# psychopa4/PFNL

Hardware: AMD Instinct MI355X
Metric: HR frames/sec at 4xSR, 7-frame 128x128->512x512 (higher is better)
Workload: dtype f32

## Files before the change

### pfnl_amd/csrc/capi.hip

```cpp
#include <dlfcn.h>

#include <atomic>
#include <cmath>
#include <condition_variable>
#include <cstdio>
#include <cstdlib>
#include <cstring>
#include <functional>
#include <map>
#include <memory>
#include <mutex>
#include <string>
#include <thread>
#include <vector>

#include "../../include/pfnl_hip.h"
#include "capi_internal.h"
#include "common.h"
#include "conv_bf16.h"
#include "conv_split16.h"
#include "conv_small.h"

namespace {

thread_local std::string g_err;

int fail(int code, const std::string& msg) {
    g_err = msg;
    return code;
}
}

int pfnl_internal_fail(int code, const std::string& msg) { return fail(code, msg); }

namespace {

static unsigned long long g_alloc_gen = 0;

struct DevBuf {
    float* p = nullptr;
    size_t n = 0;
    int ensure(size_t count) {
        if (count <= n) return 0;
        ++g_alloc_gen;
        if (p) hipFree(p);
        p = nullptr;
        n = 0;
        if (hipMalloc(&p, count * sizeof(float)) != hipSuccess) return -1;
        n = count;
        return 0;
    }
    void release() {
        if (p) hipFree(p);
        p = nullptr;
        n = 0;
    }
};

struct HostTensor {
    std::vector<int64_t> shape;
    std::vector<float> data;
};

struct PinBuf {
    unsigned char* p = nullptr;
    size_t n = 0;
    int ensure(size_t bytes) {
        if (bytes <= n) return 0;
        release();
        if (hipHostMalloc(reinterpret_cast<void**>(&p), bytes, hipHostMallocDefault) != hipSuccess) {
            p = nullptr;
            return -1;
        }
        n = bytes;
        return 0;
    }
    void release() {
        if (p) hipHostFree(p);
        p = nullptr;
        n = 0;
    }
};

struct HostPool {
    std::vector<std::thread> th;
    std::mutex m;
    std::condition_variable cv_work, cv_done;
    std::function<void(int)> fn;
    std::unique_ptr<std::atomic<int>[]> flag;
    int cap = 0, n = 0, next = 0, finished = 0, device = 0;
    bool stop = false;
    void start(int k, int dev) {
        if (!th.empty()) return;
        device = dev;
        for (int i = 0; i < k; ++i) th.emplace_back([this] { loop(); });
    }
    void loop() {
        hipSetDevice(device);
        for (;;) {
            int i;
            {
                std::unique_lock<std::mutex> lk(m);
                cv_work.wait(lk, [&] { return stop || next < n; });
                if (stop) return;
                i = next++;
            }
            fn(i);
            flag[i].store(1, std::memory_order_release);
            {
                std::lock_guard<std::mutex> lk(m);
                ++finished;
            }
            cv_done.notify_all();
        }
    }
    void run(int count, std::function<void(int)> f) {
        std::lock_guard<std::mutex> lk(m);
        if (count > cap) {
            flag.reset(new std::atomic<int>[count]);
            cap = count;
        }
        for (int i = 0; i < count; ++i) flag[i].store(0, std::memory_order_relaxed);
        fn = std::move(f);
        n = count;
        next = 0;
        finished = 0;
        cv_work.notify_all();
    }
    void wait_chunk(int i) {
        while (!flag[i].load(std::memory_order_acquire)) std::this_thread::yield();
    }
    void wait() {
        std::unique_lock<std::mutex> lk(m);
        cv_done.wait(lk, [&] { return finished >= n; });
    }
    void shutdown() {
        {
            std::lock_guard<std::mutex> lk(m);
            stop = true;
        }
        cv_work.notify_all();
        for (auto& t : th) t.join();
        th.clear();
    }
};

}

static constexpr int kSmallTiles256 = 200;
static constexpr int kMidChains256 = 136;
static int scaled_by_cus(int v256, int ncu) {
    return ncu > 0 && ncu != 256 ? std::max(1, (int)((long long)v256 * ncu / 256)) : v256;
}

struct BlockPacks {
    size_t c1_w = 0, c1_b = 0, c10_w = 0, c10_b = 0, c10_s = 0, c2a_w = 0, c2b_w = 0, c2_b = 0;
    size_t c1_u = 0, c2a_u = 0, c2b_u = 0;
    size_t bf_c1 = 0, bf_c10 = 0, bf_c2a = 0, bf_c2b = 0, bf_c1_m16 = 0, bf_c2b_m16 = 0;
    size_t s_c1 = 0, s_c2a = 0, s_c2b = 0, s_c10 = 0, s_c10f = 0, s_c2a_sf = 0, s_c2b_sf = 0, s_c2a_m16 = 0, s_c2b_m16 = 0, s_c1_m16 = 0;
    size_t sm_c1 = 0, sm_c10 = 0, sm_c2 = 0;
};

struct pfnl_handle {
    pfnl_config cfg;
    int ncu = 0;
    hipStream_t stream = nullptr;
    std::map<std::string, std::vector<int64_t>> expected;
    std::map<std::string, HostTensor> host;
    bool finalized = false;
    bool weights_external = false;
    size_t wdev_used = 0, wdev16_used = 0, wdev16s_used = 0;
    struct GraphEntry {
        int B, H, W, seen;
        hipGraph_t graph;
        hipGraphExec_t exec;
        unsigned long long alloc_gen, cfg_gen;
        unsigned long long seen_cfg_gen;
        int slot;
    };
    std::vector<GraphEntry> graphs;
    unsigned long long cfg_gen = 0;
    hipEvent_t gev = nullptr;
    int graph_mode = 0;
    bool conv2_grouped = true;
    int merge_cstride = 48;
    int conv1x1_algo = 2;
    bool bf16_fuse10 = true;
    bool bf16_m16 = true;
    bool bf16 = false;
    DevBuf wdev16;
    size_t off16_m1 = 0;
    size_t off16s_m1 = 0;
    int m1_algo = 0;
    int conv_algo = 5;
    int nl_algo = 2;
    DevBuf wdev16s;
    bool s16_m16 = true;
    size_t off16m_m1 = 0;
    unsigned* rflag_host = nullptr;
    unsigned* rflag_dev = nullptr;
    PinBuf pin_in, pin_out;
    HostPool pool;
    std::vector<hipEvent_t> d2h_ev;
    bool strict = false, strict_once = false, weights_f16_ok = true;
    long long range_reruns = 0;
    int small_mode = 0;
    bool small_c10 = true;
    DevBuf p10;
    bool sf_chain = true;
    bool sf_c10 = true;
    bool sf_mid = true;
    int sf_mid_chains = 0;
    bool sf0 = false;
    DevBuf inp0sf;
    bool split_chains = true;
    DevBuf c10part;
    bool sf_path = true;

    DevBuf wdev;
    size_t off_conv0_w = 0, off_conv0_b = 0;
    std::vector<BlockPacks> blocks;
    std::vector<size_t> off_m1_u;
    size_t off_m1_w = 0, off_m1_b = 0, off_m2_w = 0, off_m2_b = 0, off_nl_w = 0, off_nl_b = 0, off_zero = 0;

    std::map<std::string, std::vector<int64_t>> optional;
    bool nl_theta = false;
    size_t off_nl_m = 0, off_nl_c = 0;
    DevBuf Q;
    DevBuf Xs;
    int nl_type = -1;
    int nl_sub = 1;

    DevBuf nl16;
    DevBuf X, Xo, nlp, inp0, inp1, base, pb, merge, stage_in, stage_out, scratch;
    int lastB = 0, lastH = 0, lastW = 0;

    bool prof = false;
    int prof_mode = 0;
    bool prof_gate = true;
    bool chain_open = false;
    std::vector<hipEvent_t> evs;
    std::vector<int> ev_cls;
    std::vector<int> ev_cnt;
    int run_cls = -1, run_n = 0;
    size_t evs_used = 0;
    double prof_ms[PFNL_K_COUNT] = {0};
    int64_t prof_n[PFNL_K_COUNT] = {0};

    pfnl_stream* session = nullptr;
};

pfnl_handle_view pfnl_internal_view(pfnl_handle* h) {
    return {h->cfg.num_frames, h->cfg.scale, h->cfg.device_id, h->finalized, h->stream, &h->session};
}

namespace {

using namespace pfnl;

inline bool prof_sampled(int nb, int i) { return nb >= 10 ? (i % 10) == 3 : (i & 3) == 0; }

int prof_mark(pfnl_handle* h, hipStream_t s, int cls, int count = 1) {
    if (h->evs_used == h->evs.size()) {
        hipEvent_t e;
        if (hipEventCreate(&e) != hipSuccess) return -1;
        h->evs.push_back(e);
        h->ev_cls.push_back(-1);
        h->ev_cnt.push_back(1);
    }
    h->ev_cls[h->evs_used] = cls;
    h->ev_cnt[h->evs_used] = count;
    return hipEventRecord(h->evs[h->evs_used++], s) == hipSuccess ? 0 : -1;
}

void prof_flush_run(pfnl_handle* h, hipStream_t s) {
    if (h->prof && h->prof_mode == 4 && h->run_n > 0) prof_mark(h, s, h->run_cls, h->run_n);
    h->run_n = 0;
    h->run_cls = -1;
}

struct Roctx {
    int (*push)(const char*) = nullptr;
    int (*pop)() = nullptr;
};
const Roctx* roctx() {
    static const Roctx r = [] {
        Roctx x;
        const char* e = std::getenv("PFNL_ROCTX");
        if (!e || !*e || *e == '0') return x;
        for (const char* n : {"librocprofiler-sdk-roctx.so", "librocprofiler-sdk-roctx.so.1", "libroctx64.so", "libroctx64.so.4",
                              "/opt/rocm/lib/librocprofiler-sdk-roctx.so", "/opt/rocm/lib/libroctx64.so"}) {
            if (void* lib = dlopen(n, RTLD_NOW | RTLD_GLOBAL)) {
                x.push = reinterpret_cast<int (*)(const char*)>(dlsym(lib, "roctxRangePushA"));
                x.pop = reinterpret_cast<int (*)()>(dlsym(lib, "roctxRangePop"));
                if (x.push && x.pop) break;
                x.push = nullptr;
                x.pop = nullptr;
            }
        }
        return x;
    }();
    return &r;
}
const char* const kClassNames[PFNL_K_COUNT] = {"pfnl:nl_pack", "pfnl:nl_attn", "pfnl:conv0", "pfnl:conv3x3", "pfnl:conv1x1", "pfnl:merge1", "pfnl:tail"};

struct ProfScope {
    pfnl_handle* h;
    hipStream_t s;
    int cls;
    bool ranged = false;
    ProfScope(pfnl_handle* h_, hipStream_t s_, int cls_) : h(h_), s(s_), cls(cls_) {
        if (roctx()->push && cls >= 0 && cls < PFNL_K_COUNT) {
            roctx()->push(kClassNames[cls]);
            ranged = true;
        }
        if (h && h->prof && h->prof_mode == 4 && h->run_n > 0 && h->run_cls != cls) prof_flush_run(h, s);
        if (h && h->prof && h->prof_gate && !h->chain_open) {
            prof_mark(h, s, -1);
            h->chain_open = true;
        }
    }
    ~ProfScope() {
        if (h && h->prof && h->prof_mode == 4) {
            h->run_cls = cls;
            ++h->run_n;
        } else if (h && h->prof && h->prof_gate) {
            prof_mark(h, s, cls);
        }
        if (ranged) roctx()->pop();
    }
};

int prof_collect(pfnl_handle* h) {
    for (size_t i = 0; i < h->evs_used; ++i) {
        const int cls = h->ev_cls[i];
        if (cls < 0 || i == 0) continue;
        if (hipEventSynchronize(h->evs[i]) != hipSuccess) return -1;
        float ms = 0.f;
        if (hipEventElapsedTime(&ms, h->evs[i - 1], h->evs[i]) != hipSuccess) return -1;
        h->prof_ms[cls] += ms;
        h->prof_n[cls] += h->ev_cnt[i];
    }
    h->evs_used = 0;
    h->chain_open = false;
    return 0;
}

int check_geometry(const pfnl_config& c) {
    if (c.num_frames != 3 && c.num_frames != 5 && c.num_frames != 7)
        return fail(PFNL_ERR_INVALID, "num_frames must be 3, 5 or 7");
    if (c.scale != 2 && c.scale != 4) return fail(PFNL_ERR_INVALID, "scale must be 2 or 4");
    if (c.mf != 64) return fail(PFNL_ERR_INVALID, "mf must be 64");
    if (c.num_block < 0 || c.num_block > 1024) return fail(PFNL_ERR_INVALID, "bad num_block");
    for (int r : c.reserved)
        if (r != 0) return fail(PFNL_ERR_INVALID, "reserved config fields must be 0");
    return 0;
}

void add_expected(pfnl_handle* h, const std::string& layer, int k, int cin, int cout) {
    h->expected["nlvsr/" + layer + "/kernel"] = {k, k, cin, cout};
    h->expected["nlvsr/" + layer + "/bias"] = {cout};
}

size_t numel(const std::vector<int64_t>& s) {
    size_t n = 1;
    for (auto d : s) n *= (size_t)d;
    return n;
}

enum Merge1Kind {
    M1_SMALL,
    M1_BF16,
    M1_SPLIT16,
    M1_SPLIT16_CUT,
    M1_WINOGRAD,
    M1_DIRECT,
};
const char* const kMerge1Names[] = {"small", "bf16", "split16", "split16_cut", "winograd", "direct"};

struct TrunkPlan {
    bool bf16 = false;
    bool strict = false;
    int nltype = 1;
    int nl_family = 0;
    bool nl_fused_pack = false;
    bool bmid = false, fuse10 = false;
    int algo = 0, conv1x1_algo = 0;
    bool sf = false;
    bool small = false, small_c10 = false;
    bool mid = false;
    bool c10_fused = false;
    bool chain = false;
    bool sf0 = false;
    bool conv2_grouped = false;
    int n_full = 0, split_s = 0, split_q = 0;
    int c1x1_launches = 0;
    int launches_per_block = 0;
    int tiles8x32 = 0, chains = 0;
    int mfma = 32;
    int c1_mfma = 32;
    int merge1 = M1_DIRECT;
    int merge_stride = 48;
    size_t p10_floats = 0, inp0sf_floats = 0, c10part_floats = 0;
    const char* name = "";
};

void plan_bf16_trunk(const pfnl_handle* h, TrunkPlan& pl, int T, int grid, int mid_chains, bool fits32) {
    pl.bmid = h->sf_mid && h->bf16_fuse10 && pl.chains < mid_chains;
    pl.fuse10 = h->bf16_fuse10 && !pl.bmid;
    pl.launches_per_block = pl.fuse10 ? 3 : 4;
    pl.c1x1_launches = pl.fuse10 ? 0 : 1;
    if (pl.fuse10 && h->split_chains && fits32 && split_rule(pl.chains, T, grid, pl.n_full, pl.split_s, pl.split_q)) {
        pl.launches_per_block += 1;
        pl.c1x1_launches = 1;
    }
    pl.name = pl.bmid ? "bf16_mid4" : (pl.fuse10 ? (pl.split_s ? "bf16_3_split" : "bf16_3") : "bf16_4");
    pl.mfma = h->bf16_m16 ? 16 : 32;
    pl.merge1 = M1_BF16;
    pl.merge_stride = 64;
}

void plan_fp32_trunk(const pfnl_handle* h, TrunkPlan& pl, int B, int H, int W, int T, int grid, int mid_chains, bool fits32) {
    const int small_tiles = scaled_by_cus(kSmallTiles256, h->ncu);
    const int algo0 = h->conv_algo == 5 ? ((pl.tiles8x32 >= small_tiles && fits32) ? 4 : 3) : h->conv_algo;
    pl.algo = (pl.strict && algo0 == 4) ? 3 : algo0;
    pl.conv1x1_algo = (pl.strict && h->conv1x1_algo == 2) ? 1 : h->conv1x1_algo;
    pl.sf = pl.algo == 4 && pl.conv1x1_algo == 2 && h->sf_path;
    pl.small = !pl.strict && fits32 &&
               (h->small_mode == 1 || (h->small_mode == 0 && h->conv_algo == 5 && h->conv1x1_algo == 2 && pl.tiles8x32 < small_tiles));
    pl.small_c10 = pl.small && h->small_c10;
    if (pl.small) {
        pl.launches_per_block = pl.small_c10 ? 2 : 3;
        pl.c1x1_launches = pl.small_c10 ? 0 : 1;
        pl.name = pl.small_c10 ? "small2" : "small3";
        pl.merge1 = M1_SMALL;
        pl.merge_stride = 64;
        return;
    }
    pl.mid = pl.sf && h->sf_mid && h->conv_algo == 5 && h->sf_c10 && h->sf_chain && pl.chains < mid_chains;
    pl.c10_fused = pl.sf && h->sf_c10 && !pl.mid;
    pl.chain = pl.sf && h->sf_chain && !pl.mid;
    pl.sf0 = pl.c10_fused && pl.chain && h->sf0;
    const int wino_groups = B * ((W + 31) / 32) * ((H + 3) / 4);
    pl.conv2_grouped = pl.algo == 3 && h->conv2_grouped && wino_groups >= 224 && fits32;
    pl.launches_per_block = (pl.c10_fused ? 1 : 2) + ((pl.chain || pl.conv2_grouped) ? 1 : 2);
    pl.c1x1_launches = pl.c10_fused ? 0 : 1;
    if (pl.c10_fused && pl.chain && h->split_chains && split_rule(pl.chains, T, grid, pl.n_full, pl.split_s, pl.split_q)) {
        pl.launches_per_block += 1;
        pl.c1x1_launches = 1;
    }
    pl.mfma = (h->s16_m16 && pl.c10_fused && pl.chain && !pl.sf0 && !pl.split_s && pl.chains >= grid) ? 16 : 32;
    pl.c1_mfma = pl.mfma;
    pl.name = pl.mid ? "mid4" : (pl.c10_fused && pl.chain) ? (pl.sf0 ? "chain2_sf0" : (pl.split_s ? "chain2_split" : "chain2"))
            : pl.algo == 4 ? (pl.launches_per_block == 3 ? "split16_3" : "split16_4")
            : pl.algo == 3 ? (pl.conv2_grouped ? "winograd_ws3" : "winograd_ws4")
            : pl.algo == 1 ? "winograd_tile4" : "direct4";
    if (pl.algo == 4 && h->m1_algo != 2 && fits32) pl.merge1 = pl.split_s ? M1_SPLIT16_CUT : M1_SPLIT16;
    else if ((pl.algo == 3 || pl.algo == 4) && wino_groups >= 224 && fits32) pl.merge1 = M1_WINOGRAD;
    pl.merge_stride = pl.merge1 == M1_DIRECT ? 48 : 64;
}

TrunkPlan trunk_plan(const pfnl_handle* h, int B, int H, int W, int Hfull) {
    TrunkPlan pl;
    const int T = h->cfg.num_frames;
    pl.bf16 = h->bf16;
    pl.strict = !h->bf16 && (h->strict || h->strict_once || !h->weights_f16_ok);
    pl.tiles8x32 = B * T * ((W + 31) / 32) * ((H + 7) / 8);
    pl.chains = pl.tiles8x32 / T;
    const int grid = persistent_grid(h->ncu);
    const int mid_chains = h->sf_mid_chains > 0 ? h->sf_mid_chains : scaled_by_cus(kMidChains256, h->ncu);
    const bool fits32 = (long long)H * W * 256 < 0x7fffffffLL;
    if (h->bf16) plan_bf16_trunk(h, pl, T, grid, mid_chains, fits32);
    else plan_fp32_trunk(h, pl, B, H, W, T, grid, mid_chains, fits32);

    const int N = (Hfull / 2) * (W / 2);
    pl.nltype = h->nl_type < 0 ? (h->nl_theta ? 0 : 1) : h->nl_type;
    pl.nl_family = (pl.nltype != 1 || h->nl_sub > 1) ? 0
                 : h->bf16 ? 2
                 : (!pl.strict && (h->nl_algo == 1 || (h->nl_algo == 2 && N >= 1024))) ? 1 : 3;
    pl.nl_fused_pack = (pl.nl_family == 1 || pl.nl_family == 2) && nl_f16_fits_one_launch(B, N);

    const size_t frame_floats = (size_t)B * T * H * W * 64;
    pl.p10_floats = pl.small_c10 ? frame_floats : 0;
    pl.inp0sf_floats = pl.sf0 ? frame_floats : 0;
    pl.c10part_floats = pl.split_s ? (size_t)(pl.chains - pl.n_full) * pl.split_s * 8 * 32 * 64 : 0;
    return pl;
}

struct Fwd {
    pfnl_handle* h;
    const TrunkPlan& pl;
    hipStream_t s;
    int B, T, F, H, W;
    const float* wd;
    const uint16_t* w16;
    const uint16_t* w16s;
};

template <class P>
void set_split_chains(P& q, const TrunkPlan& pl, float* partial) {
    q.n_full = pl.n_full;
    q.split_s = pl.split_s;
    q.split_q = pl.split_q;
    q.partial = pl.split_s ? partial : nullptr;
}

template <class P>
P split_finalize_params(const Fwd& f) {
    P q{};
    q.H = f.H;
    q.W = f.W;
    q.items = f.F;
    q.add_div = f.T;
    set_split_chains(q, f.pl, f.h->c10part.p);
    return q;
}

ConvParams direct_params(const Fwd& f, const float* in, const float* wpack, const float* bias, float* out, int cout, int frames, int act) {
    ConvParams p{};
    p.in = in;
    p.wpack = wpack;
    p.bias = bias;
    p.out = out;
    p.H = f.H;
    p.W = f.W;
    p.in_cstride = 64;
    p.out_cstride = cout;
    p.cout = cout;
    p.chunks_per_frame = 64 / CONV_CK;
    p.frames_per_item = frames;
    p.nchunks = frames * p.chunks_per_frame;
    p.add_div = 1;
    p.act = act;
    return p;
}

int ensure_workspace(pfnl_handle* h, const TrunkPlan& pl, int B, int H, int W, int N) {
    const int T = h->cfg.num_frames, C = 12 * T, CP = nl_padded_ch(C);
    const size_t P = (size_t)H * W;
    if (h->X.ensure((size_t)B * N * CP) || h->Xo.ensure((size_t)B * N * CP) ||
        h->nlp.ensure(nl_partial_floats(B, N, C)) ||
        h->inp0.ensure((size_t)B * T * P * 64) || h->inp1.ensure((size_t)B * T * P * 64) ||
        h->base.ensure((size_t)B * P * 64) || h->pb.ensure((size_t)B * P * 64) ||
        h->merge.ensure((size_t)B * P * 64))
        return fail(PFNL_ERR_NOMEM, "workspace allocation failed");
    h->lastB = B;
    h->lastH = H;
    h->lastW = W;
    if (h->p10.ensure(h->cfg.num_block > 0 ? pl.p10_floats : 0) || h->inp0sf.ensure(pl.inp0sf_floats) || h->c10part.ensure(pl.c10part_floats))
        return fail(PFNL_ERR_NOMEM, "workspace allocation failed");
    return 0;
}

int nonlocal_block(const Fwd& f, const float* in, int Hfull, int q0, int q1) {
    pfnl_handle* const h = f.h;
    const TrunkPlan& pl = f.pl;
    const int B = f.B, T = f.T, W = f.W, N = (Hfull / 2) * (W / 2), C = 12 * T, CP = nl_padded_ch(C), nlt = pl.nltype;
    const float* const wd = f.wd;
    const hipStream_t s = f.s;
    if ((pl.nl_family == 1 || pl.nl_family == 2) && h->nl16.ensure((nl_f16_scratch_halfs(B, N) + 1) / 2))
        return fail(PFNL_ERR_NOMEM, "workspace allocation failed");
    {
        ProfScope ps(h, s, PFNL_K_NL_PACK);
        if (pl.nl_fused_pack) HIPCHK(launch_nl_pack_fused(in, h->X.p, reinterpret_cast<uint16_t*>(h->nl16.p), B, T, Hfull, W, s));
        else HIPCHK(launch_nl_pack(in, h->X.p, B, T, Hfull, W, s));
    }
    ProfScope ps(h, s, PFNL_K_NL_ATTN);
    if ((nlt == 0 || nlt == 2) && !h->nl_theta)
        return fail(PFNL_ERR_STATE, "nl_type 0 / 2 need the nlblock_0 theta / phi variables (reference utils.py:31-42)");
    if (pl.nl_family == 0) {
        const float* Kx = h->X.p;
        int Nk = N;
        if (h->nl_sub > 1) {
            const int h2 = Hfull / 2, w2 = W / 2;
            if (h2 / h->nl_sub < 1 || w2 / h->nl_sub < 1) return fail(PFNL_ERR_INVALID, "nl_sub_sample larger than the space_to_depth grid");
            Nk = (h2 / h->nl_sub) * (w2 / h->nl_sub);
            if (h->Xs.ensure((size_t)B * Nk * CP)) return fail(PFNL_ERR_NOMEM, "workspace allocation failed");
            HIPCHK(launch_nl_pool(h->X.p, h->Xs.p, B, h2, w2, h->nl_sub, C, s));
            Kx = h->Xs.p;
        }
        const float* Qp = nullptr;
        if (nlt != 1) {
            if (h->Q.ensure((size_t)B * N * CP)) return fail(PFNL_ERR_NOMEM, "workspace allocation failed");
            HIPCHK(launch_nl_qproj(h->X.p, wd + h->off_nl_m, wd + h->off_nl_c, h->Q.p, B, N, C, s, nlt == 2));
            Qp = h->Q.p;
        }
        HIPCHK(launch_nl_attn_general(h->X.p, Kx, Nk, h->Xo.p, wd + h->off_nl_w, wd + h->off_nl_b, h->nlp.p, B, N, C, s, Qp, q0, q1, nlt == 2));
    } else if (pl.nl_family == 1 || pl.nl_family == 2) {
        HIPCHK(launch_nl_attn_f16(h->X.p, h->Xo.p, wd + h->off_nl_w, wd + h->off_nl_b, h->nlp.p, reinterpret_cast<uint16_t*>(h->nl16.p), B, N, C, s,
                                  q0, q1, pl.nl_family == 1, pl.nl_fused_pack));
    } else {
        HIPCHK(launch_nl_attn(h->X.p, h->Xo.p, wd + h->off_nl_w, wd + h->off_nl_b, h->nlp.p, B, N, C, s, nullptr, q0, q1));
    }
    return 0;
}


int block_bf16(const Fwd& f, const BlockPacks& k) {
    pfnl_handle* const h = f.h;
    const TrunkPlan& pl = f.pl;
    const hipStream_t s = f.s;
    const float* const wd = f.wd;
    uint16_t* const a0 = reinterpret_cast<uint16_t*>(h->inp0.p);
    uint16_t* const a1 = reinterpret_cast<uint16_t*>(h->inp1.p);
    uint16_t* const ab = reinterpret_cast<uint16_t*>(h->base.p);
    uint16_t* const ap = reinterpret_cast<uint16_t*>(h->pb.p);
    {
        ProfScope ps(h, s, PFNL_K_CONV3X3);
        ConvBf16Params q{a0, f.w16 + k.bf_c1, wd + k.c1_b, nullptr, nullptr, a1, f.H, f.W, f.F, 1, 1};
        if (pl.fuse10) {
            q.add_div = f.T;
            q.x_w = f.w16 + k.bf_c10;
            q.x_bias = wd + k.c10_b;
            q.x_out = ab;
            set_split_chains(q, pl, h->c10part.p);
        }
        if (pl.mfma == 16) q.wpack16 = f.w16 + k.bf_c1_m16;
        HIPCHK(launch_conv3x3_bf16(q, s));
    }
    if (pl.fuse10 && pl.split_s) {
        ProfScope ps(h, s, PFNL_K_CONV1X1);
        ConvBf16Params q = split_finalize_params<ConvBf16Params>(f);
        q.x_bias = wd + k.c10_b;
        q.x_out = ab;
        HIPCHK(launch_c10_finalize_bf16(q, s));
    }
    if (!pl.fuse10) {
        ProfScope ps(h, s, PFNL_K_CONV1X1);
        HIPCHK(launch_conv1x1_bf16(a1, f.w16 + k.bf_c10, wd + k.c10_b, ab, f.B, f.T, f.H * f.W, 1, s));
    }
    {
        ProfScope ps(h, s, PFNL_K_CONV3X3);
        ConvBf16Params q{ab, f.w16 + k.bf_c2a, wd + h->off_zero, nullptr, nullptr, ap, f.H, f.W, f.B, 1, 0};
        HIPCHK(launch_conv3x3_bf16(q, s));
    }
    {
        ProfScope ps(h, s, PFNL_K_CONV3X3);
        ConvBf16Params q{a1, f.w16 + k.bf_c2b, wd + k.c2_b, ap, a0, a0, f.H, f.W, f.F, f.T, 1};
        q.flat = pl.bmid ? 1 : 0;
        set_split_chains(q, pl, nullptr);
        if (pl.mfma == 16) q.wpack16 = f.w16 + k.bf_c2b_m16;
        HIPCHK(launch_conv3x3_bf16(q, s));
    }
    return 0;
}

int block_small(const Fwd& f, const BlockPacks& k) {
    pfnl_handle* const h = f.h;
    const hipStream_t s = f.s;
    const float* const wd = f.wd;
    const int H = f.H, W = f.W, F = f.F, T = f.T;
    {
        ProfScope ps(h, s, PFNL_K_CONV3X3);
        ConvSmallParams q{nullptr, h->inp0.p, 0, 1, 1, 1, f.w16s + k.sm_c1, wd + k.c1_b, nullptr, h->inp1.p, H, W, F, 1, 3};
        if (f.pl.small_c10) {
            q.x_wpack = f.w16s + k.sm_c10;
            q.x_out = h->p10.p;
            q.x_T = T;
        }
        HIPCHK(launch_conv_small(q, s));
    }
    if (!f.pl.small_c10) {
        ProfScope ps(h, s, PFNL_K_CONV1X1);
        ConvSmallParams q{nullptr, h->inp1.p, 0, 1, T, T, f.w16s + k.sm_c10, wd + k.c10_b, nullptr, h->base.p, H, W, f.B, 1, 1};
        HIPCHK(launch_conv_small(q, s));
    }
    {
        ProfScope ps(h, s, PFNL_K_CONV3X3);
        ConvSmallParams q{f.pl.small_c10 ? h->p10.p : h->base.p, h->inp1.p, 1, T, 1, 2, f.w16s + k.sm_c2, wd + k.c2_b, h->inp0.p, h->inp0.p, H, W, F, 1, 3};
        if (f.pl.small_c10) {
            q.a_nsum = T;
            q.a_bias = wd + k.c10_b;
        }
        HIPCHK(launch_conv_small(q, s));
    }
    return 0;
}

int block_fp32(const Fwd& f, const BlockPacks& k, bool first, bool last) {
    pfnl_handle* const h = f.h;
    const TrunkPlan& pl = f.pl;
    const hipStream_t s = f.s;
    const float* const wd = f.wd;
    const int H = f.H, W = f.W, F = f.F, T = f.T, B = f.B, algo = pl.algo;
    const bool sf = pl.sf;
    const bool in_sf0 = pl.sf0 && !first, out_sf0 = pl.sf0 && !last;
    if (pl.c10_fused) {
        {
            ProfScope ps(h, s, PFNL_K_CONV3X3);
            ConvSplitParams q{in_sf0 ? h->inp0sf.p : h->inp0.p, f.w16s + k.s_c1, wd + k.c1_b, nullptr, nullptr, h->inp1.p, H, W, F, T, 1};
            q.in_sf = in_sf0 ? 1 : 0;
            q.wpack2 = f.w16s + k.s_c10f;
            q.bias2 = wd + k.c10_b;
            q.out2 = h->base.p;
            set_split_chains(q, pl, h->c10part.p);
            if (pl.c1_mfma == 16) q.wpack_m16 = f.w16s + k.s_c1_m16;
            HIPCHK(launch_conv3x3_c1c10(q, s));
        }
        if (pl.split_s) {
            ProfScope ps(h, s, PFNL_K_CONV1X1);
            ConvSplitParams q = split_finalize_params<ConvSplitParams>(f);
            q.act = 1;
            q.out2 = h->base.p;
            HIPCHK(launch_c10_finalize(q, s));
        }
    } else {
        {
            ProfScope ps(h, s, PFNL_K_CONV3X3);
            if (algo == 4) {
                ConvSplitParams q{h->inp0.p, f.w16s + k.s_c1, wd + k.c1_b, nullptr, nullptr, h->inp1.p, H, W, F, 1, 1};
                q.out_sf = sf ? 1 : 0;
                HIPCHK(launch_conv3x3_split16(q, s));
            } else if (algo == 1 || algo == 3) {
                WinoParams wp{h->inp0.p, wd + k.c1_u, wd + k.c1_b, nullptr, nullptr, h->inp1.p, H, W, 1, 1, F};
                HIPCHK(algo == 3 ? launch_conv_wino_ws(wp, s) : launch_conv_wino(wp, s));
            } else {
                HIPCHK(launch_conv_mfma(direct_params(f, h->inp0.p, wd + k.c1_w, wd + k.c1_b, h->inp1.p, 64, 1, 1), 3, F, s));
            }
        }
        {
            ProfScope ps(h, s, PFNL_K_CONV1X1);
            if (pl.conv1x1_algo == 2)
                HIPCHK(launch_conv1x1_split16(h->inp1.p, f.w16s + k.s_c10, wd + k.c10_b, h->base.p, B, T, H * W, 1, s, sf, sf));
            else if (pl.conv1x1_algo == 1)
                HIPCHK(launch_conv1x1_stream(h->inp1.p, wd + k.c10_s, wd + k.c10_b, h->base.p, B, T, H * W, 1, s));
            else
                HIPCHK(launch_conv_mfma(direct_params(f, h->inp1.p, wd + k.c10_w, wd + k.c10_b, h->base.p, 64, T, 1), 1, B, s));
        }
    }
    if (pl.conv2_grouped) {
        ProfScope ps(h, s, PFNL_K_CONV3X3);
        WinoParams wp{h->inp1.p, wd + k.c2b_u, wd + k.c2_b, nullptr, h->inp0.p, h->inp0.p, H, W, T, 1, F};
        wp.in2 = h->base.p;
        wp.upack2 = wd + k.c2a_u;
        HIPCHK(launch_conv_wino_ws(wp, s));
        return 0;
    }
    if (pl.chain) {
        ProfScope ps(h, s, PFNL_K_CONV3X3);
        ConvSplitParams q{h->inp1.p, f.w16s + k.s_c2b_sf, wd + k.c2_b, nullptr, h->inp0.p, h->inp0.p, H, W, F, T, 1};
        q.in2 = h->base.p;
        q.wpack2 = f.w16s + k.s_c2a_sf;
        q.out2 = out_sf0 ? h->inp0sf.p : nullptr;
        set_split_chains(q, pl, nullptr);
        if (pl.mfma == 16) {
            q.wpack_m16 = f.w16s + k.s_c2b_m16;
            q.wpack2_m16 = f.w16s + k.s_c2a_m16;
        }
        HIPCHK(launch_conv3x3_sf_chain(q, s));
        return 0;
    }
    {
        ProfScope ps(h, s, PFNL_K_CONV3X3);
        if (algo == 4) {
            ConvSplitParams q{h->base.p, f.w16s + (sf ? k.s_c2a_sf : k.s_c2a), wd + h->off_zero, nullptr, nullptr, h->pb.p, H, W, B, 1, 0};
            HIPCHK(sf ? launch_conv3x3_sf(q, s) : launch_conv3x3_split16(q, s));
        } else if (algo == 1 || algo == 3) {
            WinoParams wp{h->base.p, wd + k.c2a_u, wd + h->off_zero, nullptr, nullptr, h->pb.p, H, W, 1, 0, B};
            HIPCHK(algo == 3 ? launch_conv_wino_ws(wp, s) : launch_conv_wino(wp, s));
        } else {
            HIPCHK(launch_conv_mfma(direct_params(f, h->base.p, wd + k.c2a_w, wd + h->off_zero, h->pb.p, 64, 1, 0), 3, B, s));
        }
    }
    {
        ProfScope ps(h, s, PFNL_K_CONV3X3);
        if (algo == 4) {
            ConvSplitParams q{h->inp1.p, f.w16s + (sf ? k.s_c2b_sf : k.s_c2b), wd + k.c2_b, h->pb.p, h->inp0.p, h->inp0.p, H, W, F, T, 1};
            q.flat = pl.mid ? 1 : 0;
            HIPCHK(sf ? launch_conv3x3_sf(q, s) : launch_conv3x3_split16(q, s));
        } else if (algo == 1 || algo == 3) {
            WinoParams wp{h->inp1.p, wd + k.c2b_u, wd + k.c2_b, h->pb.p, h->inp0.p, h->inp0.p, H, W, T, 1, F};
            HIPCHK(algo == 3 ? launch_conv_wino_ws(wp, s) : launch_conv_wino(wp, s));
        } else {
            ConvParams p = direct_params(f, h->inp1.p, wd + k.c2b_w, wd + k.c2_b, h->inp0.p, 64, 1, 1);
            p.addend = h->pb.p;
            p.add_div = T;
            p.resid = h->inp0.p;
            HIPCHK(launch_conv_mfma(p, 3, F, s));
        }
    }
    return 0;
}

int convmerge1(const Fwd& f) {
    pfnl_handle* const h = f.h;
    const TrunkPlan& pl = f.pl;
    const hipStream_t s = f.s;
    const float* const wd = f.wd;
    const int H = f.H, W = f.W, F = f.F, T = f.T;
    h->merge_cstride = pl.merge_stride;
    if (pl.merge1 == M1_SPLIT16 || pl.merge1 == M1_SPLIT16_CUT) {
        {
            ProfScope ps(h, s, PFNL_K_MERGE1);
            ConvSplitParams q{h->inp0.p, f.w16s + h->off16s_m1, wd + h->off_m1_b, nullptr, nullptr, h->merge.p, H, W, F, T, 1, 1};
            set_split_chains(q, pl, h->c10part.p);
            HIPCHK(launch_conv3x3_split16(q, s));
        }
        if (pl.merge1 == M1_SPLIT16_CUT) {
            ProfScope ps(h, s, PFNL_K_MERGE1);
            ConvSplitParams q = split_finalize_params<ConvSplitParams>(f);
            q.act = 1;
            q.bias = wd + h->off_m1_b;
            q.out = h->merge.p;
            HIPCHK(launch_c10_finalize(q, s));
        }
        return 0;
    }
    ProfScope ps(h, s, PFNL_K_MERGE1);
    switch (pl.merge1) {
    case M1_SMALL: {
        ConvSmallParams q{nullptr, h->inp0.p, 0, 1, T, T, f.w16s + h->off16m_m1, wd + h->off_m1_b, nullptr, h->merge.p, H, W, f.B, 1, 3};
        HIPCHK(launch_conv_small(q, s));
        return 0;
    }
    case M1_BF16: {
        ConvBf16Params q{reinterpret_cast<const uint16_t*>(h->inp0.p), f.w16 + h->off16_m1, wd + h->off_m1_b, nullptr, nullptr, nullptr, H, W, F, T, 1};
        q.out_f32 = h->merge.p;
        HIPCHK(launch_conv3x3_bf16(q, s));
        return 0;
    }
    case M1_WINOGRAD: {
        WinoParams wp{h->inp0.p, wd + h->off_m1_u[0], wd + h->off_m1_b, nullptr, nullptr, h->merge.p, H, W, T, 1, F};
        wp.upack_stride = T > 1 ? (long long)(h->off_m1_u[1] - h->off_m1_u[0]) : 0;
        wp.accum = 1;
        HIPCHK(launch_conv_wino_ws(wp, s));
        return 0;
    }
    default:
        HIPCHK(launch_conv_mfma(direct_params(f, h->inp0.p, wd + h->off_m1_w, wd + h->off_m1_b, h->merge.p, 48, T, 1), 3, f.B, s));
        return 0;
    }
}

int forward_device(pfnl_handle* h, const float* in, float* out, int B, int Hfull, int W, hipStream_t s,
                   const StripGeom* strip = nullptr, int q0 = 0, int q1 = -1, int flag_slot = 1 ) {
    const pfnl_config& c = h->cfg;
    const int T = c.num_frames;
    const int H = strip ? strip->Hs : Hfull;
    const TrunkPlan pl = trunk_plan(h, B, H, W, Hfull);
    if (pl.bf16 && (long long)T * H * W * 128 >= 0x7fffffffLL) return fail(PFNL_ERR_INVALID, "frame too large for the bf16 trunk");
    if (int e = ensure_workspace(h, pl, B, H, W, (Hfull / 2) * (W / 2))) return e;
    const Fwd f{h, pl, s, B, T, B * T, H, W, h->wdev.p, reinterpret_cast<const uint16_t*>(h->wdev16.p), reinterpret_cast<const uint16_t*>(h->wdev16s.p)};
    const float* const wd = h->wdev.p;

    if (int e = nonlocal_block(f, in, Hfull, q0, q1)) return e;
    {
        ProfScope ps(h, s, PFNL_K_CONV0);
        if (pl.bf16)
            HIPCHK(launch_conv0_bf16(h->Xo.p, wd + h->off_conv0_w, wd + h->off_conv0_b, reinterpret_cast<uint16_t*>(h->inp0.p), B, T, Hfull, W, s, strip));
        else
            HIPCHK(launch_conv0(h->Xo.p, wd + h->off_conv0_w, wd + h->off_conv0_b, h->inp0.p, B, T, Hfull, W, s, strip, pl.strict));
    }
    for (int i = 0; i < c.num_block; ++i) {
        if (h->prof_mode == 2) {
            h->prof_gate = prof_sampled(c.num_block, i);
            h->chain_open = false;
        } else if (h->prof_mode == 3) {
            h->prof_gate = i == c.num_block / 2;
            h->chain_open = false;
        }
        const BlockPacks& k = h->blocks[i];
        const int e = pl.bf16 ? block_bf16(f, k) : pl.small ? block_small(f, k) : block_fp32(f, k, i == 0, i + 1 == c.num_block);
        if (e) return e;
    }
    h->prof_gate = h->prof_mode != 3;
    if (h->prof_mode == 2 || h->prof_mode == 3) h->chain_open = false;
    if (int e = convmerge1(f)) return e;
    {
        unsigned* const rflag = (pl.strict || pl.nltype == 2) ? nullptr : h->rflag_dev + flag_slot;
        ProfScope ps(h, s, PFNL_K_TAIL);
        HIPCHK(launch_tail(h->merge.p, in, wd + h->off_m2_w, wd + h->off_m2_b, out, B, T, Hfull, W, c.scale, pl.merge_stride, s, strip, rflag));
    }
    prof_flush_run(h, s);
    h->chain_open = false;
    return 0;
}

struct OptionField {
    int pfnl_handle::*i = nullptr;
    bool pfnl_handle::*b = nullptr;
    constexpr OptionField(int pfnl_handle::*f) : i(f) {}
    constexpr OptionField(bool pfnl_handle::*f) : b(f) {}
    int get(const pfnl_handle* h) const { return i ? h->*i : (int)(h->*b); }
    void set(pfnl_handle* h, int v) const {
        if (i) h->*i = v;
        else h->*b = v != 0;
    }
};

struct OptionName {
    const char* name;
    int value;
};

struct OptionSpec {
    const char* key;
    OptionField field;
    OptionName names[8];
    const char* refusal;
};

const OptionSpec kOptions[] = {
    {"graph", &pfnl_handle::graph_mode, {{"auto", 1}, {"on", 2}, {"off", 0}}, "graph must be auto, on or off"},
    {"conv3x3", &pfnl_handle::conv_algo, {{"winograd", 3}, {"winograd_ws", 3}, {"winograd_tile", 1}, {"direct", 0}, {"split16", 4}, {"auto", 5}},
     "conv3x3 must be auto, split16, winograd, winograd_tile or direct"},
    {"strict_fp32", &pfnl_handle::strict, {{"on", 1}, {"off", 0}}, "strict_fp32 must be on or off"},
    {"small", &pfnl_handle::small_mode, {{"auto", 0}, {"on", 1}, {"off", 2}}, "small must be auto, on or off"},
    {"split16_chain", &pfnl_handle::sf_chain, {{"on", 1}, {"off", 0}}, "split16_chain must be on or off"},
    {"split16_c10", &pfnl_handle::sf_c10, {{"on", 1}, {"off", 0}}, "split16_c10 must be on or off"},
    {"split16_mid", &pfnl_handle::sf_mid, {{"auto", 1}, {"off", 0}}, "split16_mid must be auto or off"},
    {"split16_sf0", &pfnl_handle::sf0, {{"on", 1}, {"off", 0}}, "split16_sf0 must be on or off"},
    {"split16_splitchains", &pfnl_handle::split_chains, {{"auto", 1}, {"off", 0}}, "split16_splitchains must be auto or off"},
    {"split16_sf", &pfnl_handle::sf_path, {{"on", 1}, {"off", 0}}, "split16_sf must be on or off"},
    {"conv2", &pfnl_handle::conv2_grouped, {{"grouped", 1}, {"split", 0}}, "conv2 must be grouped or split"},
    {"split16_mfma", &pfnl_handle::s16_m16, {{"16", 1}, {"32", 0}}, "split16_mfma must be 16 or 32"},
    {"bf16_mfma", &pfnl_handle::bf16_m16, {{"16", 1}, {"32", 0}}, "bf16_mfma must be 16 or 32"},
    {"bf16_conv10", &pfnl_handle::bf16_fuse10, {{"fused", 1}, {"separate", 0}}, "bf16_conv10 must be fused or separate"},
    {"precision", &pfnl_handle::bf16, {{"bf16", 1}, {"fp32", 0}}, "precision must be fp32 or bf16"},
    {"merge1", &pfnl_handle::m1_algo, {{"auto", 0}, {"split16", 1}, {"winograd", 2}}, "merge1 must be auto, split16 or winograd"},
    {"nl_type", &pfnl_handle::nl_type,
     {{"auto", -1}, {"0", 0}, {"embedded_gaussian", 0}, {"1", 1}, {"gaussian", 1}, {"2", 2}, {"dot_product", 2}},
     "nl_type: auto | 0 | 1 | 2 (nltype 3, 'concat', builds no graph in the reference either: utils.py:23)"},
    {"small_c10", &pfnl_handle::small_c10, {{"on", 1}, {"off", 0}}, "small_c10 must be on or off"},
    {"nonlocal", &pfnl_handle::nl_algo, {{"f32", 0}, {"split16", 1}, {"auto", 2}}, "nonlocal must be auto, f32 or split16"},
    {"conv1x1", &pfnl_handle::conv1x1_algo, {{"stream", 1}, {"tiled", 0}, {"split16", 2}}, "conv1x1 must be split16, stream or tiled"},
};

const OptionSpec* find_option(const std::string& key) {
    for (const OptionSpec& o : kOptions)
        if (key == o.key) return &o;
    return nullptr;
}

}

void pfnl_nl_fold_gw(const float* wg, const float* bg, const float* ww, const float* bw, int C, int CP, float* Wf, float* bf) {
    for (int ci = 0; ci < C; ++ci)
        for (int co = 0; co < C; ++co) {
            double acc = 0.0;
            for (int cm = 0; cm < C; ++cm) acc += (double)wg[(size_t)ci * C + cm] * (double)ww[(size_t)cm * C + co];
            Wf[(size_t)ci * CP + co] = (float)acc;
        }
    for (int co = 0; co < C; ++co) {
        double acc = bw[co];
        for (int cm = 0; cm < C; ++cm) acc += (double)bg[cm] * (double)ww[(size_t)cm * C + co];
        bf[co] = (float)acc;
    }
}

void pfnl_nl_fold_theta_phi(const float* wt, const float* bt, const float* wp, const float* bp, int C, int CP, float* Mf, float* cf) {
    for (int ci = 0; ci < C; ++ci)
        for (int cj = 0; cj < C; ++cj) {
            double acc = 0.0;
            for (int cm = 0; cm < C; ++cm) acc += (double)wt[(size_t)ci * C + cm] * (double)wp[(size_t)cj * C + cm];
            Mf[(size_t)ci * CP + cj] = (float)acc;
        }
    for (int cj = 0; cj < C; ++cj) {
        double acc = 0.0;
        for (int cm = 0; cm < C; ++cm) acc += (double)bt[cm] * (double)wp[(size_t)cj * C + cm];
        cf[cj] = (float)acc;
    }
    if (!bp) return;
    double d0 = 0.0;
    for (int cm = 0; cm < C; ++cm) d0 += (double)bt[cm] * (double)bp[cm];
    cf[C] = (float)d0;
    for (int ci = 0; ci < C; ++ci) {
        double acc = 0.0;
        for (int cm = 0; cm < C; ++cm) acc += (double)wt[(size_t)ci * C + cm] * (double)bp[cm];
        Mf[(size_t)ci * CP + C] = (float)acc;
    }
}

extern "C" {

const char* pfnl_last_error(void) { return g_err.c_str(); }
int pfnl_version(void) { return 4; }

int pfnl_device_count(int* count) {
    if (!count) return fail(PFNL_ERR_INVALID, "count is NULL");
    int n = 0;
    if (hipGetDeviceCount(&n) != hipSuccess) n = 0;
    *count = n;
    return 0;
}

int pfnl_create(const pfnl_config* cfg, pfnl_handle** out) {
    if (!cfg || !out) return fail(PFNL_ERR_INVALID, "NULL argument");
    if (int e = check_geometry(*cfg)) return e;
    int ndev = 0;
    if (hipGetDeviceCount(&ndev) != hipSuccess || ndev == 0)
        return fail(PFNL_ERR_NODEVICE, "no HIP device visible: libpfnl_hip has no CPU fallback");
    if (cfg->device_id < 0 || cfg->device_id >= ndev) return fail(PFNL_ERR_INVALID, "bad device_id");
    HIPCHK(hipSetDevice(cfg->device_id));
    pfnl_handle* h = new pfnl_handle();
    h->cfg = *cfg;
    h->ncu = pfnl::device_cu_count();
    if (const char* e = std::getenv("PFNL_SF_MID_CHAINS")) h->sf_mid_chains = std::atoi(e);
    if (const char* e = std::getenv("PFNL_CONV3X3")) {
        const std::string v(e);
        h->conv_algo = v == "direct" ? 0 : (v == "winograd_tile" ? 1 : (v == "split16" ? 4 : (v == "winograd" ? 3 : 5)));
    }
    if (hipStreamCreateWithFlags(&h->stream, hipStreamDefault) != hipSuccess) {
        delete h;
        return fail(PFNL_ERR_HIP, "hipStreamCreate failed");
    }
    if (hipHostMalloc(reinterpret_cast<void**>(&h->rflag_host), 64, hipHostMallocMapped) != hipSuccess ||
        hipHostGetDevicePointer(reinterpret_cast<void**>(&h->rflag_dev), h->rflag_host, 0) != hipSuccess) {
        if (h->rflag_host) hipHostFree(h->rflag_host);
        hipStreamDestroy(h->stream);
        delete h;
        return fail(PFNL_ERR_NOMEM, "allocation failed");
    }
    std::memset(h->rflag_host, 0, 64);
    if (const char* e = std::getenv("PFNL_STRICT_FP32")) h->strict = std::string(e) != "0" && std::string(e) != "off";
    const int T = cfg->num_frames, C = 12 * T;
    add_expected(h, "conv0", 5, 3, 64);
    for (int i = 0; i < cfg->num_block; ++i) {
        add_expected(h, "conv1_" + std::to_string(i), 3, 64, 64);
        add_expected(h, "conv10_" + std::to_string(i), 1, 64 * T, 64);
        add_expected(h, "conv2_" + std::to_string(i), 3, 128, 64);
    }
    add_expected(h, "convmerge1", 3, 64 * T, 48);
    add_expected(h, "convmerge2", 3, 12, cfg->scale == 4 ? 12 : 3);
    add_expected(h, "nlblock_0/g/g", 1, C, C);
    add_expected(h, "nlblock_0/w/w", 1, C, C);
    for (const char* n : {"theta/theta", "phi/phi"}) {
        h->optional[std::string("nlvsr/nlblock_0/") + n + "/kernel"] = {1, 1, C, C};
        h->optional[std::string("nlvsr/nlblock_0/") + n + "/bias"] = {C};
    }
    *out = h;
    return 0;
}

int pfnl_destroy(pfnl_handle* h) {
    if (!h) return 0;
    if (h->session) pfnl_stream_close(h->session);
    hipSetDevice(h->cfg.device_id);
    if (h->stream) {
        hipStreamSynchronize(h->stream);
        hipStreamDestroy(h->stream);
    }
    for (auto& e : h->evs) hipEventDestroy(e);
    if (h->gev) hipEventDestroy(h->gev);
    for (auto& g : h->graphs) {
        if (g.exec) hipGraphExecDestroy(g.exec);
        if (g.graph) hipGraphDestroy(g.graph);
    }
    h->pool.shutdown();
    for (auto& e : h->d2h_ev) hipEventDestroy(e);
    h->pin_in.release();
    h->pin_out.release();
    if (h->rflag_host) hipHostFree(h->rflag_host);
    for (DevBuf* b : {&h->p10, &h->Xs, &h->Q, &h->wdev16s, &h->wdev, &h->wdev16, &h->nl16, &h->X, &h->Xo, &h->nlp, &h->inp0, &h->inp0sf, &h->c10part, &h->inp1, &h->base, &h->pb, &h->merge,
                      &h->stage_in, &h->stage_out, &h->scratch})
        b->release();
    delete h;
    return 0;
}

int pfnl_set_weight(pfnl_handle* h, const char* tf_name, const float* host, const int64_t* shape,
                    int rank) {
    if (!h || !tf_name || !host || !shape) return fail(PFNL_ERR_INVALID, "NULL argument");
    std::string name(tf_name);
    if (name.size() > 2 && name.compare(name.size() - 2, 2, ":0") == 0) name.resize(name.size() - 2);
    auto it = h->expected.find(name);
    if (it == h->expected.end()) it = h->expected.find("nlvsr/" + name);
    if (it == h->expected.end()) {
        it = h->optional.find(name);
        if (it == h->optional.end()) it = h->optional.find("nlvsr/" + name);
        if (it == h->optional.end()) return fail(PFNL_ERR_INVALID, "unknown tensor name: " + name);
    }
    if ((int)it->second.size() != rank) return fail(PFNL_ERR_INVALID, "rank mismatch for " + name);
    for (int i = 0; i < rank; ++i)
        if (shape[i] != it->second[i]) return fail(PFNL_ERR_INVALID, "shape mismatch for " + name);
    if (h->weights_external) {
        h->host.clear();
        h->weights_external = false;
    }
    HostTensor t;
    t.shape = it->second;
    t.data.assign(host, host + numel(t.shape));
    h->host[it->first] = std::move(t);
    h->finalized = false;
    return 0;
}

int pfnl_set_option(pfnl_handle* h, const char* key, const char* value) {
    if (!h || !key || !value) return fail(PFNL_ERR_INVALID, "NULL argument");
    const std::string k(key), v(value);
    ++h->cfg_gen;
    if (k == "nl_sub_sample") {
        const int n = atoi(v.c_str());
        if (n < 1 || n > 64) return fail(PFNL_ERR_INVALID, "nl_sub_sample: an integer >= 1");
        h->nl_sub = n;
        return 0;
    }
    if (k == "bf16_nonlocal") {
        if (v != "f16") return fail(PFNL_ERR_INVALID, "bf16_nonlocal must be f16");
        return 0;
    }
    const OptionSpec* o = find_option(k);
    if (!o) return fail(PFNL_ERR_INVALID, "unknown option " + k);
    for (const OptionName& n : o->names)
        if (n.name && v == n.name) {
            o->field.set(h, n.value);
            return 0;
        }
    return fail(PFNL_ERR_INVALID, o->refusal);
}

int pfnl_get_option(pfnl_handle* h, const char* key, char* buf, size_t buflen) {
    if (!h || !key || !buf || buflen < 1) return fail(PFNL_ERR_INVALID, "NULL argument");
    const std::string k(key);
    std::string v;
    if (k == "nl_sub_sample") v = std::to_string(h->nl_sub);
    else if (k == "bf16_nonlocal") v = "f16";
    else if (const OptionSpec* o = find_option(k)) {
        const int cur = o->field.get(h);
        for (const OptionName& n : o->names)
            if (n.name && n.value == cur) {
                v = n.name;
                break;
            }
    } else return fail(PFNL_ERR_INVALID, "unknown option " + k);
    if (v.size() + 1 > buflen) return fail(PFNL_ERR_INVALID, "buffer too small");
    std::memcpy(buf, v.c_str(), v.size() + 1);
    return 0;
}

int pfnl_missing_weights(pfnl_handle* h, int* count) {
    if (!h || !count) return fail(PFNL_ERR_INVALID, "NULL argument");
    int n = 0;
    for (auto& kv : h->expected)
        if (!h->host.count(kv.first)) ++n;
    *count = n;
    return 0;
}

int pfnl_finalize_weights(pfnl_handle* h) {
    if (!h) return fail(PFNL_ERR_INVALID, "NULL handle");
    for (auto& kv : h->expected)
        if (!h->host.count(kv.first)) return fail(PFNL_ERR_STATE, "missing tensor " + kv.first);
    HIPCHK(hipSetDevice(h->cfg.device_id));
    const int T = h->cfg.num_frames, nb = h->cfg.num_block, C = 12 * T, CP = pfnl::nl_padded_ch(C);
    std::vector<float> blob;
    auto W = [&](const std::string& l) -> const std::vector<float>& { return h->host["nlvsr/" + l + "/kernel"].data; };
    auto Bv = [&](const std::string& l) -> const std::vector<float>& { return h->host["nlvsr/" + l + "/bias"].data; };
    auto reserve = [&](size_t n) {
        size_t off = (blob.size() + 63) / 64 * 64;
        blob.resize(off + n, 0.f);
        return off;
    };
    auto put_bias = [&](const std::vector<float>& b) {
        size_t off = reserve(64);
        std::memcpy(&blob[off], b.data(), b.size() * sizeof(float));
        return off;
    };
    auto put_wino = [&](const std::vector<float>& k, int cin_total, int cin_begin) {
        size_t off = reserve(pfnl::wino_pack_floats());
        pfnl::wino_pack_weights(k.data(), cin_total, cin_begin, &blob[off]);
        return off;
    };
    auto put_pack = [&](const std::vector<float>& k, int ks, int cin_total, int cin_begin, int cin, int cout) {
        size_t off = reserve(pfnl::conv_pack_floats(ks, cin));
        pfnl::conv_pack_weights(k.data(), ks, cin_total, cin_begin, cin, cout, &blob[off]);
        return off;
    };

    h->off_zero = reserve(64);
    h->off_conv0_w = reserve(75 * 64);
    std::memcpy(&blob[h->off_conv0_w], W("conv0").data(), 75 * 64 * sizeof(float));
    h->off_conv0_b = put_bias(Bv("conv0"));
    h->blocks.assign(nb, BlockPacks{});
    for (int i = 0; i < nb; ++i) {
        const std::string s = std::to_string(i);
        BlockPacks& k = h->blocks[i];
        k.c1_w = put_pack(W("conv1_" + s), 3, 64, 0, 64, 64);
        k.c1_b = put_bias(Bv("conv1_" + s));
        k.c10_w = put_pack(W("conv10_" + s), 1, 64 * T, 0, 64 * T, 64);
        k.c10_b = put_bias(Bv("conv10_" + s));
        k.c10_s = reserve(pfnl::conv1x1_pack_floats(T));
        pfnl::conv1x1_pack_weights(W("conv10_" + s).data(), T, &blob[k.c10_s]);
        k.c2a_w = put_pack(W("conv2_" + s), 3, 128, 0, 64, 64);
        k.c2b_w = put_pack(W("conv2_" + s), 3, 128, 64, 64, 64);
        k.c2_b = put_bias(Bv("conv2_" + s));
        k.c1_u = put_wino(W("conv1_" + s), 64, 0);
        k.c2a_u = put_wino(W("conv2_" + s), 128, 0);
        k.c2b_u = put_wino(W("conv2_" + s), 128, 64);
    }
    h->off_m1_w = put_pack(W("convmerge1"), 3, 64 * T, 0, 64 * T, 48);
    h->off_m1_b = put_bias(Bv("convmerge1"));
    h->off_m1_u.assign(T, 0);
    for (int f = 0; f < T; ++f) {
        h->off_m1_u[f] = reserve(pfnl::wino_pack_floats());
        pfnl::wino_pack_weights(W("convmerge1").data(), 64 * T, 64 * f, &blob[h->off_m1_u[f]], 48);
    }
    {
        const auto& k = W("convmerge2");
        h->off_m2_w = reserve(k.size());
        std::memcpy(&blob[h->off_m2_w], k.data(), k.size() * sizeof(float));
        h->off_m2_b = put_bias(Bv("convmerge2"));
    }
    {
        h->off_nl_w = reserve((size_t)CP * CP);
        h->off_nl_b = reserve(CP);
        pfnl_nl_fold_gw(W("nlblock_0/g/g").data(), Bv("nlblock_0/g/g").data(), W("nlblock_0/w/w").data(), Bv("nlblock_0/w/w").data(), C, CP,
                        &blob[h->off_nl_w], &blob[h->off_nl_b]);
    }
    {
        int have = 0;
        for (auto& kv : h->optional) have += (int)h->host.count(kv.first);
        if (have != 0 && have != (int)h->optional.size())
            return fail(PFNL_ERR_STATE, "nlblock_0 theta/phi: all four tensors (two kernels, two biases) or none");
        h->nl_theta = have != 0;
        if (h->nl_theta) {
            h->off_nl_m = reserve((size_t)CP * CP);
            h->off_nl_c = reserve(CP);
            pfnl_nl_fold_theta_phi(W("nlblock_0/theta/theta").data(), Bv("nlblock_0/theta/theta").data(), W("nlblock_0/phi/phi").data(),
                                   Bv("nlblock_0/phi/phi").data(), C, CP, &blob[h->off_nl_m], &blob[h->off_nl_c]);
        }
    }
    {
        std::vector<uint16_t> b16;
        auto reserve16 = [&](size_t n) {
            size_t off = (b16.size() + 127) / 128 * 128;
            b16.resize(off + n, 0);
            return off;
        };
        for (int i = 0; i < nb; ++i) {
            const std::string s = std::to_string(i);
            BlockPacks& k = h->blocks[i];
            k.bf_c1 = reserve16(pfnl::conv3x3_bf16_pack_halfs());
            pfnl::conv3x3_bf16_pack_weights(W("conv1_" + s).data(), 64, 0, &b16[k.bf_c1]);
            k.bf_c10 = reserve16(pfnl::conv1x1_bf16_pack_halfs(T));
            pfnl::conv1x1_bf16_pack_weights(W("conv10_" + s).data(), T, &b16[k.bf_c10]);
            k.bf_c2a = reserve16(pfnl::conv3x3_bf16_pack_halfs());
            pfnl::conv3x3_bf16_pack_weights(W("conv2_" + s).data(), 128, 0, &b16[k.bf_c2a]);
            k.bf_c2b = reserve16(pfnl::conv3x3_bf16_pack_halfs());
            pfnl::conv3x3_bf16_pack_weights(W("conv2_" + s).data(), 128, 64, &b16[k.bf_c2b]);
            k.bf_c1_m16 = reserve16(pfnl::conv3x3_bf16_pack_halfs());
            pfnl::conv3x3_bf16_pack_weights16(W("conv1_" + s).data(), 64, 0, &b16[k.bf_c1_m16]);
            k.bf_c2b_m16 = reserve16(pfnl::conv3x3_bf16_pack_halfs());
            pfnl::conv3x3_bf16_pack_weights16(W("conv2_" + s).data(), 128, 64, &b16[k.bf_c2b_m16]);
        }
        h->off16_m1 = reserve16((size_t)T * pfnl::conv3x3_bf16_pack_halfs());
        for (int f = 0; f < T; ++f)
            pfnl::conv3x3_bf16_pack_weights(W("convmerge1").data(), 64 * T, 64 * f, &b16[h->off16_m1 + (size_t)f * pfnl::conv3x3_bf16_pack_halfs()], 48);
        b16.resize((b16.size() + 1) / 2 * 2 + 2, 0);
        h->wdev16_used = b16.size() / 2;
        if (h->wdev16.ensure(b16.size() / 2)) return fail(PFNL_ERR_NOMEM, "weight allocation failed");
        HIPCHK(hipMemcpy(h->wdev16.p, b16.data(), b16.size() * sizeof(uint16_t), hipMemcpyHostToDevice));
    }
    {
        std::vector<uint16_t> b16;
        const size_t n3 = pfnl::conv3x3_split16_pack_halfs(), n1 = pfnl::conv1x1_split16_pack_halfs(T);
        const size_t blk = 8 * n3 + n1 + pfnl::conv1x1_c10_pack_halfs(T);
        h->off16s_m1 = (size_t)nb * blk;
        const size_t m3 = pfnl::conv_small_pack_halfs(3, 1), m10 = pfnl::conv_small_pack_halfs(1, T);
        const size_t small_base = (size_t)nb * blk + (size_t)T * n3;
        h->off16m_m1 = small_base + (size_t)nb * (3 * m3 + m10);
        b16.resize(h->off16m_m1 + (size_t)T * m3 + 2, 0);
        pfnl::conv_small_pack_weights(W("convmerge1").data(), 3, T, 48, &b16[h->off16m_m1]);
        for (int f = 0; f < T; ++f)
            pfnl::conv3x3_split16_pack_weights(W("convmerge1").data(), 64 * T, 64 * f, &b16[h->off16s_m1 + (size_t)f * n3], 48);
        for (int i = 0; i < nb; ++i) {
            const std::string s = std::to_string(i);
            BlockPacks& k = h->blocks[i];
            k.s_c1 = (size_t)i * blk;
            k.s_c2a = k.s_c1 + n3;
            k.s_c2b = k.s_c1 + 2 * n3;
            k.s_c10 = k.s_c1 + 3 * n3;
            k.s_c2a_sf = k.s_c10 + n1;
            k.s_c2b_sf = k.s_c2a_sf + n3;
            k.s_c10f = k.s_c2b_sf + n3;
            k.s_c2a_m16 = k.s_c10f + pfnl::conv1x1_c10_pack_halfs(T);
            k.s_c2b_m16 = k.s_c2a_m16 + n3;
            k.s_c1_m16 = k.s_c2b_m16 + n3;
            pfnl::conv3x3_split16_pack_weights16(W("conv1_" + s).data(), 64, 0, &b16[k.s_c1_m16], true);
            pfnl::conv3x3_split16_pack_weights16(W("conv2_" + s).data(), 128, 0, &b16[k.s_c2a_m16]);
            pfnl::conv3x3_split16_pack_weights16(W("conv2_" + s).data(), 128, 64, &b16[k.s_c2b_m16]);
            pfnl::conv1x1_c10_pack_weights(W("conv10_" + s).data(), T, &b16[k.s_c10f]);
            pfnl::conv3x3_split16_pack_weights(W("conv2_" + s).data(), 128, 0, &b16[k.s_c2a_sf], 64, true);
            pfnl::conv3x3_split16_pack_weights(W("conv2_" + s).data(), 128, 64, &b16[k.s_c2b_sf], 64, true);
            k.sm_c1 = small_base + (size_t)i * (3 * m3 + m10);
            k.sm_c2 = k.sm_c1 + m3;
            k.sm_c10 = k.sm_c1 + 3 * m3;
            pfnl::conv_small_pack_weights(W("conv1_" + s).data(), 3, 1, 64, &b16[k.sm_c1]);
            pfnl::conv_small_pack_weights(W("conv2_" + s).data(), 3, 2, 64, &b16[k.sm_c2]);
            pfnl::conv_small_pack_weights(W("conv10_" + s).data(), 1, T, 64, &b16[k.sm_c10]);
            pfnl::conv1x1_split16_pack_weights(W("conv10_" + s).data(), T, &b16[k.s_c10]);
            pfnl::conv3x3_split16_pack_weights(W("conv1_" + s).data(), 64, 0, &b16[k.s_c1]);
            pfnl::conv3x3_split16_pack_weights(W("conv2_" + s).data(), 128, 0, &b16[k.s_c2a]);
            pfnl::conv3x3_split16_pack_weights(W("conv2_" + s).data(), 128, 64, &b16[k.s_c2b]);
        }
        h->wdev16s_used = b16.size() / 2;
        if (h->wdev16s.ensure(b16.size() / 2)) return fail(PFNL_ERR_NOMEM, "weight allocation failed");
        HIPCHK(hipMemcpy(h->wdev16s.p, b16.data(), b16.size() / 2 * 2 * sizeof(uint16_t), hipMemcpyHostToDevice));
    }
    {
        float wmax = 0.f;
        for (const auto& kv : h->host)
            for (float v : kv.second.data) wmax = std::fmax(wmax, std::fabs(v));
        h->weights_f16_ok = wmax < 65504.0f;
    }
    h->wdev_used = blob.size();
    if (h->wdev.ensure(blob.size())) return fail(PFNL_ERR_NOMEM, "weight allocation failed");
    HIPCHK(hipMemcpy(h->wdev.p, blob.data(), blob.size() * sizeof(float), hipMemcpyHostToDevice));
    h->finalized = true;
    ++h->cfg_gen;
    return 0;
}

int pfnl_workspace_bytes(pfnl_handle* h, int B, int H, int W, size_t* bytes) {
    if (!h || !bytes) return fail(PFNL_ERR_INVALID, "NULL argument");
    if (B <= 0 || H <= 0 || W <= 0 || (H & 1) || (W & 1)) return fail(PFNL_ERR_INVALID, "bad shape");
    const size_t T = h->cfg.num_frames, P = (size_t)H * W, N = P / 4, sc = h->cfg.scale;
    const int C = 12 * (int)T;
    const size_t CP = pfnl::nl_padded_ch(C);
    size_t f = 2 * B * N * CP
             + pfnl::nl_partial_floats(B, (int)N, C)
             + 2 * B * T * P * 64
             + 3 * B * P * 64
             + (size_t)B * T * P * 3 + (size_t)B * P * sc * sc * 3;
    if (h->bf16 || h->nl_algo != 0) f += (pfnl::nl_f16_scratch_halfs(B, (int)N) + 1) / 2;
    if (h->nl_theta) f += (size_t)B * N * CP;
    if (h->nl_sub > 1) f += (size_t)B * ((H / 2) / h->nl_sub) * ((W / 2) / h->nl_sub) * CP;
    const TrunkPlan pl = trunk_plan(h, B, H, W, H);
    f += pl.p10_floats + pl.inp0sf_floats + pl.c10part_floats;
    *bytes = f * sizeof(float);
    return 0;
}

int pfnl_plan(pfnl_handle* h, int B, int H, int W, char* buf, size_t buflen) {
    if (!h || !buf || buflen < 1) return fail(PFNL_ERR_INVALID, "NULL argument");
    if (B <= 0 || H <= 0 || W <= 0 || (H & 1) || (W & 1)) return fail(PFNL_ERR_INVALID, "bad shape");
    const TrunkPlan pl = trunk_plan(h, B, H, W, H);
    static const char* const nln[] = {"general_f32", "split16", "f16", "f32"};
    static const char* const a3[] = {"direct", "winograd_tile", "?", "winograd", "split16"};
    static const char* const a1[] = {"tiled", "stream", "split16"};
    char tmp[384];
    if (pl.bf16)
        std::snprintf(tmp, sizeof tmp, "%s launches_per_block=%d c1x1=%d precision=bf16 tiles=%d chains=%d whole_chains=%d split_parts=%d part_frames=%d nl=%s nl_pack_fused=%d mfma=%d merge1=%s",
                      pl.name, pl.launches_per_block, pl.c1x1_launches, pl.tiles8x32, pl.chains, pl.split_s ? pl.n_full : pl.chains, pl.split_s, pl.split_q,
                      nln[pl.nl_family], pl.nl_fused_pack ? 1 : 0, pl.mfma, kMerge1Names[pl.merge1]);
    else
        std::snprintf(tmp, sizeof tmp, "%s launches_per_block=%d c1x1=%d precision=fp32 conv3x3=%s conv1x1=%s c10_fused=%d chain=%d sf0=%d strict=%d tiles=%d chains=%d "
                      "whole_chains=%d split_parts=%d part_frames=%d nl=%s nl_pack_fused=%d mfma=%d c1_mfma=%d merge1=%s",
                      pl.name, pl.launches_per_block, pl.c1x1_launches, pl.small ? "small" : a3[pl.algo < 0 || pl.algo > 4 ? 2 : pl.algo],
                      a1[pl.conv1x1_algo < 0 || pl.conv1x1_algo > 2 ? 0 : pl.conv1x1_algo], pl.c10_fused ? 1 : 0, pl.chain ? 1 : 0, pl.sf0 ? 1 : 0,
                      pl.strict ? 1 : 0, pl.tiles8x32, pl.chains, pl.split_s ? pl.n_full : pl.chains, pl.split_s, pl.split_q, nln[pl.nl_family],
                      pl.nl_fused_pack ? 1 : 0, pl.mfma, pl.c1_mfma, kMerge1Names[pl.merge1]);
    if (std::strlen(tmp) + 1 > buflen) return fail(PFNL_ERR_INVALID, "buffer too small");
    std::strcpy(buf, tmp);
    return 0;
}

static int range_flag_take(pfnl_handle* h, int slot, int* flagged) {
    unsigned* const f = h->rflag_host + slot;
    *flagged = __atomic_exchange_n(f, 0u, __ATOMIC_ACQ_REL) != 0;
    return 0;
}

int pfnl_range_reruns(pfnl_handle* h, long long* count) {
    if (!h || !count) return fail(PFNL_ERR_INVALID, "NULL argument");
    *count = h->range_reruns;
    return 0;
}

namespace {
constexpr size_t STAGE_POOL_MIN = 512u << 10;
constexpr int STAGE_MAX_CHUNKS = 32;

bool host_is_pinned(const void* p) {
    hipPointerAttribute_t a;
    if (hipPointerGetAttributes(&a, p) != hipSuccess) {
        (void)hipGetLastError();
        return false;
    }
    return a.type == hipMemoryTypeHost;
}

void ensure_pool(pfnl_handle* h) {
    if (!h->pool.th.empty()) return;
    int k = 4;
    if (const char* e = std::getenv("PFNL_HOST_THREADS")) k = std::atoi(e);
    const int hw = (int)std::thread::hardware_concurrency();
    if (hw > 1 && k > hw - 1) k = hw - 1;
    k = k < 1 ? 1 : (k > 16 ? 16 : k);
    h->pool.start(k, h->cfg.device_id);
}

size_t stage_chunk_bytes(size_t bytes) {
    size_t c = (bytes + STAGE_MAX_CHUNKS - 1) / STAGE_MAX_CHUNKS;
    if (c < (1u << 20)) c = 1u << 20;
    return (c + 4095) & ~(size_t)4095;
}

int stage_h2d(pfnl_handle* h, float* dst, const void* src, size_t bytes, hipStream_t s) {
    if (host_is_pinned(src)) {
        HIPCHK(hipMemcpyAsync(dst, src, bytes, hipMemcpyHostToDevice, s));
        return 0;
    }
    if (h->pin_in.ensure(bytes)) return fail(PFNL_ERR_NOMEM, "pinned staging allocation failed");
    unsigned char* const pin = h->pin_in.p;
    if (bytes < STAGE_POOL_MIN) {
        std::memcpy(pin, src, bytes);
        HIPCHK(hipMemcpyAsync(dst, pin, bytes, hipMemcpyHostToDevice, s));
        return 0;
    }
    ensure_pool(h);
    const size_t csz = stage_chunk_bytes(bytes);
    const int n = (int)((bytes + csz - 1) / csz);
    const unsigned char* const sp = static_cast<const unsigned char*>(src);
    h->pool.run(n, [=](int i) {
        const size_t off = (size_t)i * csz;
        std::memcpy(pin + off, sp + off, std::min(csz, bytes - off));
    });
    hipError_t err = hipSuccess;
    for (int i = 0; i < n; ++i) {
        h->pool.wait_chunk(i);
        const size_t off = (size_t)i * csz;
        if (err == hipSuccess)
            err = hipMemcpyAsync(reinterpret_cast<unsigned char*>(dst) + off, pin + off, std::min(csz, bytes - off), hipMemcpyHostToDevice, s);
    }
    h->pool.wait();
    if (err != hipSuccess) return fail(PFNL_ERR_HIP, std::string("H2D staging: ") + hipGetErrorString(err));
    return 0;
}

int stage_d2h(pfnl_handle* h, void* dst, const float* src, size_t bytes, hipStream_t s) {
    if (host_is_pinned(dst)) {
        HIPCHK(hipMemcpyAsync(dst, src, bytes, hipMemcpyDeviceToHost, s));
        HIPCHK(hipStreamSynchronize(s));
        return 0;
    }
    if (h->pin_out.ensure(bytes)) return fail(PFNL_ERR_NOMEM, "pinned staging allocation failed");
    unsigned char* const pin = h->pin_out.p;
    if (bytes < STAGE_POOL_MIN) {
        HIPCHK(hipMemcpyAsync(pin, src, bytes, hipMemcpyDeviceToHost, s));
        HIPCHK(hipStreamSynchronize(s));
        std::memcpy(dst, pin, bytes);
        return 0;
    }
    ensure_pool(h);
    const size_t csz = stage_chunk_bytes(bytes);
    const int n = (int)((bytes + csz - 1) / csz);
    while ((int)h->d2h_ev.size() < n) {
        hipEvent_t e = nullptr;
        HIPCHK(hipEventCreateWithFlags(&e, hipEventDisableTiming));
        h->d2h_ev.push_back(e);
    }
    for (int i = 0; i < n; ++i) {
        const size_t off = (size_t)i * csz;
        HIPCHK(hipMemcpyAsync(pin + off, reinterpret_cast<const unsigned char*>(src) + off, std::min(csz, bytes - off), hipMemcpyDeviceToHost, s));
        HIPCHK(hipEventRecord(h->d2h_ev[i], s));
    }
    HIPCHK(hipEventSynchronize(h->d2h_ev[0]));
    unsigned char* const dp = static_cast<unsigned char*>(dst);
    hipEvent_t* const ev = h->d2h_ev.data();
    h->pool.run(n, [=](int i) {
        const size_t off = (size_t)i * csz;
        (void)hipEventSynchronize(ev[i]);
        std::memcpy(dp + off, pin + off, std::min(csz, bytes - off));
    });
    h->pool.wait();
    HIPCHK(hipStreamSynchronize(s));
    return 0;
}

const char* const RANGE_MSG_FP32 =
    "a device-pointer forward since the last check produced non-finite values: an operand left the range of the f16-pipe kernels "
    "(|x| < 65504; the non-local block: inputs on a [0,1] scale) or the input was not finite. Re-run with "
    "pfnl_set_option(h, \"strict_fp32\", \"on\") (f32-MFMA kernels: the reference's range), or use host pointers";
const char* const RANGE_MSG_BF16 =
    "a precision=bf16 forward produced non-finite values: the input was not finite, or it left the range of the binary16 operands of "
    "this precision's non-local block and conv0 (inputs on a [0,1] scale, |x| < ~350). precision=fp32 covers the whole fp32 range";
}

int pfnl_forward(pfnl_handle* h, const void* in, int in_is_device, void* out, int out_is_device, int B,
                 int H, int W, void* stream) {
    if (!h || !in || !out) return fail(PFNL_ERR_INVALID, "NULL argument");
    if (!h->finalized) return fail(PFNL_ERR_STATE, "pfnl_finalize_weights has not been called");
    if (B <= 0 || H <= 0 || W <= 0) return fail(PFNL_ERR_INVALID, "B, H, W must be positive");
    if ((H & 1) || (W & 1))
        return fail(PFNL_ERR_INVALID, "H and W must be even (space_to_depth(2), reference model/pfnl.py:57)");
    HIPCHK(hipSetDevice(h->cfg.device_id));
    const int T = h->cfg.num_frames, sc = h->cfg.scale;
    const size_t n_in = (size_t)B * T * H * W * 3, n_out = (size_t)B * H * W * sc * sc * 3;
    const float* din = (const float*)in;
    float* dout = (float*)out;
    const bool sync_call = !in_is_device || !out_is_device;
    const int slot = sync_call ? 0 : 1;
    const bool can_rerun = !h->bf16 && !(h->strict || !h->weights_f16_ok);
    const bool want_graph = !h->prof && (h->graph_mode == 2 || (h->graph_mode == 1 && (size_t)B * T * H * W <= 65536));
    hipStream_t s = stream ? (hipStream_t)stream : ((in_is_device && out_is_device && !want_graph) ? (hipStream_t) nullptr : h->stream);
    if (want_graph) {
        if (h->stage_in.ensure(n_in) || h->stage_out.ensure(n_out)) return fail(PFNL_ERR_NOMEM, "staging allocation failed");
        pfnl_handle::GraphEntry* ge = nullptr;
        for (auto& g : h->graphs)
            if (g.B == B && g.H == H && g.W == W && g.slot == slot) ge = &g;
        if (!ge) {
            h->graphs.push_back({B, H, W, 0, nullptr, nullptr, 0, 0, h->cfg_gen, slot});
            ge = &h->graphs.back();
        }
        if (ge->exec && (ge->alloc_gen != g_alloc_gen || ge->cfg_gen != h->cfg_gen)) {
            HIPCHK(hipStreamSynchronize(s));
            hipGraphExecDestroy(ge->exec);
            hipGraphDestroy(ge->graph);
            ge->exec = nullptr;
            ge->graph = nullptr;
            ge->seen = 0;
        }
        if (!ge->exec && ge->seen_cfg_gen != h->cfg_gen) {
            ge->seen = 0;
            ge->seen_cfg_gen = h->cfg_gen;
        }
        if (!ge->exec && ge->seen >= 1) {
            HIPCHK(hipStreamBeginCapture(s, hipStreamCaptureModeThreadLocal));
            const int fe = forward_device(h, h->stage_in.p, h->stage_out.p, B, H, W, s, nullptr, 0, -1, slot);
            hipGraph_t g = nullptr;
            const hipError_t ce = hipStreamEndCapture(s, &g);
            if (fe) return fe;
            if (ce != hipSuccess || !g) return fail(PFNL_ERR_HIP, std::string("graph capture: ") + hipGetErrorString(ce));
            hipGraphExec_t ex = nullptr;
            const hipError_t ie = hipGraphInstantiate(&ex, g, nullptr, nullptr, 0);
            if (ie != hipSuccess) {
                hipGraphDestroy(g);
                return fail(PFNL_ERR_HIP, std::string("graph instantiate: ") + hipGetErrorString(ie));
            }
            ge->graph = g;
            ge->exec = ex;
            ge->alloc_gen = g_alloc_gen;
            ge->cfg_gen = h->cfg_gen;
        }
        if (ge->exec) {
            if (!stream) {
                if (!h->gev && hipEventCreateWithFlags(&h->gev, hipEventDisableTiming) != hipSuccess)
                    return fail(PFNL_ERR_HIP, "event creation failed");
                HIPCHK(hipEventRecord(h->gev, nullptr));
                HIPCHK(hipStreamWaitEvent(s, h->gev, 0));
            }
            if (in_is_device)
                HIPCHK(hipMemcpyAsync(h->stage_in.p, in, n_in * sizeof(float), hipMemcpyDeviceToDevice, s));
            else if (int e = stage_h2d(h, h->stage_in.p, in, n_in * sizeof(float), s))
                return e;
            HIPCHK(hipGraphLaunch(ge->exec, s));
            if (out_is_device)
                HIPCHK(hipMemcpyAsync(out, h->stage_out.p, n_out * sizeof(float), hipMemcpyDeviceToDevice, s));
            if (sync_call) {
                if (!out_is_device) {
                    if (int e = stage_d2h(h, out, h->stage_out.p, n_out * sizeof(float), s)) return e;
                } else {
                    HIPCHK(hipStreamSynchronize(s));
                }
                int flagged = 0;
                if (int e = range_flag_take(h, 0, &flagged)) return e;
                if (flagged && can_rerun) {
                    h->strict_once = true;
                    const int e = forward_device(h, h->stage_in.p, h->stage_out.p, B, H, W, s, nullptr, 0, -1, 0);
                    h->strict_once = false;
                    if (e) return e;
                    ++h->range_reruns;
                    if (out_is_device) {
                        HIPCHK(hipMemcpyAsync(out, h->stage_out.p, n_out * sizeof(float), hipMemcpyDeviceToDevice, s));
                        HIPCHK(hipStreamSynchronize(s));
                    } else if (int e2 = stage_d2h(h, out, h->stage_out.p, n_out * sizeof(float), s)) {
                        return e2;
                    }
                } else if (flagged && h->bf16) {
                    return fail(PFNL_ERR_RANGE, RANGE_MSG_BF16);
                }
            } else if (!stream) {
                HIPCHK(hipEventRecord(h->gev, s));
                HIPCHK(hipStreamWaitEvent(nullptr, h->gev, 0));
            }
            h->lastB = B;
            h->lastH = H;
            h->lastW = W;
            return 0;
        }
        ge->seen++;
    }
    if (!in_is_device) {
        if (h->stage_in.ensure(n_in)) return fail(PFNL_ERR_NOMEM, "staging allocation failed");
        if (int e = stage_h2d(h, h->stage_in.p, in, n_in * sizeof(float), s)) return e;
        din = h->stage_in.p;
    }
    if (!out_is_device) {
        if (h->stage_out.ensure(n_out)) return fail(PFNL_ERR_NOMEM, "staging allocation failed");
        dout = h->stage_out.p;
    }
    if (int e = forward_device(h, din, dout, B, H, W, s, nullptr, 0, -1, slot)) return e;
    if (!out_is_device) {
        if (int e = stage_d2h(h, out, dout, n_out * sizeof(float), s)) return e;
    } else if (!in_is_device) {
        HIPCHK(hipStreamSynchronize(s));
    }
    if (sync_call) {
        int flagged = 0;
        if (int e = range_flag_take(h, 0, &flagged)) return e;
        if (flagged && can_rerun) {
            h->strict_once = true;
            const int e = forward_device(h, din, dout, B, H, W, s, nullptr, 0, -1, 0);
            h->strict_once = false;
            if (e) return e;
            ++h->range_reruns;
            if (!out_is_device) {
                if (int e2 = stage_d2h(h, out, dout, n_out * sizeof(float), s)) return e2;
            } else {
                HIPCHK(hipStreamSynchronize(s));
            }
        } else if (flagged && h->bf16) {
            return fail(PFNL_ERR_RANGE, RANGE_MSG_BF16);
        }
    }
    return 0;
}

int pfnl_forward_strip(pfnl_handle* h, const void* in, void* out, int B, int H, int W, int row0, int nrows, void* stream) {
    if (!h || !in || !out) return fail(PFNL_ERR_INVALID, "NULL argument");
    if (!h->finalized) return fail(PFNL_ERR_STATE, "pfnl_finalize_weights has not been called");
    if (B <= 0 || H <= 0 || W <= 0 || (H & 1) || (W & 1)) return fail(PFNL_ERR_INVALID, "B, H, W must be positive, H and W even");
    if (row0 < 0 || nrows < 1 || row0 + nrows > H) return fail(PFNL_ERR_INVALID, "strip rows out of range");
    HIPCHK(hipSetDevice(h->cfg.device_id));
    const int halo = 4 + 2 * h->cfg.num_block;
    int a = row0 - halo, b = row0 + nrows + halo;
    a = a < 0 ? 0 : (a & ~1);
    b = b > H ? H : ((b + 1) & ~1);
    const StripGeom g{a, b - a, row0 - a, row0 - a + nrows};
    const int W2 = W / 2, H2 = H / 2;
    int qa = (a - 2) >> 1, qb = (b + 2 + 1) >> 1;
    qa = qa < 0 ? 0 : qa;
    qb = qb > H2 ? H2 : qb;
    hipStream_t s = stream ? (hipStream_t)stream : (hipStream_t) nullptr;
    return forward_device(h, (const float*)in, (float*)out, B, H, W, s, &g, qa * W2, qb * W2);
}

int pfnl_sync(pfnl_handle* h) {
    if (!h) return fail(PFNL_ERR_INVALID, "NULL handle");
    HIPCHK(hipSetDevice(h->cfg.device_id));
    HIPCHK(hipStreamSynchronize(h->stream));
    HIPCHK(hipStreamSynchronize(nullptr));
    int flagged = 0;
    if (int e = range_flag_take(h, 1, &flagged)) return e;
    if (flagged) return fail(PFNL_ERR_RANGE, h->bf16 ? RANGE_MSG_BF16 : RANGE_MSG_FP32);
    return 0;
}

int pfnl_host_alloc(size_t bytes, void** out) {
    if (!out || !bytes) return fail(PFNL_ERR_INVALID, "bad host allocation");
    void* p = nullptr;
    if (hipHostMalloc(&p, bytes, hipHostMallocDefault) != hipSuccess || !p) {
        (void)hipGetLastError();
        return fail(PFNL_ERR_NOMEM, "hipHostMalloc failed");
    }
    *out = p;
    return 0;
}

int pfnl_host_free(void* p) {
    if (p && hipHostFree(p) != hipSuccess) {
        (void)hipGetLastError();
        return fail(PFNL_ERR_HIP, "hipHostFree failed");
    }
    return 0;
}

int pfnl_range_flag(pfnl_handle* h, int* flagged) {
    if (!h || !flagged) return fail(PFNL_ERR_INVALID, "NULL argument");
    return range_flag_take(h, 1, flagged);
}

static int prepare_to_receive_weights(pfnl_handle* h) {
    if (h->finalized) return 0;
    for (auto& kv : h->expected)
        if (!h->host.count(kv.first)) {
            HostTensor t;
            t.shape = kv.second;
            t.data.assign(numel(t.shape), 0.f);
            h->host[kv.first] = std::move(t);
        }
    const int e = pfnl_finalize_weights(h);
    if (!e) h->weights_external = true;
    return e;
}

int pfnl_copy_weights(pfnl_handle* dst, pfnl_handle* src) {
    if (!dst || !src) return fail(PFNL_ERR_INVALID, "NULL handle");
    if (dst == src) return 0;
    if (!src->finalized) return fail(PFNL_ERR_STATE, "the source handle has no finalized weights");
    if (src->nl_theta) return fail(PFNL_ERR_INVALID, "theta/phi handles carry host-side state: load them through pfnl_set_weight");
    if (int e = prepare_to_receive_weights(dst)) return e;
    if (dst->wdev_used != src->wdev_used || dst->wdev16_used != src->wdev16_used || dst->wdev16s_used != src->wdev16s_used)
        return fail(PFNL_ERR_STATE, "the handles differ in geometry (weight blob sizes)");
    HIPCHK(hipSetDevice(dst->cfg.device_id));
    HIPCHK(hipMemcpy(dst->wdev.p, src->wdev.p, src->wdev_used * sizeof(float), hipMemcpyDefault));
    HIPCHK(hipMemcpy(dst->wdev16.p, src->wdev16.p, src->wdev16_used * sizeof(float), hipMemcpyDefault));
    HIPCHK(hipMemcpy(dst->wdev16s.p, src->wdev16s.p, src->wdev16s_used * sizeof(float), hipMemcpyDefault));
    dst->weights_f16_ok = src->weights_f16_ok;
    dst->weights_external = true;
    ++dst->cfg_gen;
    return 0;
}

int pfnl_comm_bcast_weights(pfnl_comm* c, pfnl_handle* h, int root) {
    if (!c || !h) return fail(PFNL_ERR_INVALID, "NULL argument");
    int rank = 0, nranks = 0;
    if (int e = pfnl_comm_rank(c, &rank, &nranks)) return e;
    if (root < 0 || root >= nranks) return fail(PFNL_ERR_INVALID, "bad root");
    if (rank == root && !h->finalized) return fail(PFNL_ERR_STATE, "root has no finalized weights");
    const int prep = rank != root ? prepare_to_receive_weights(h) : 0;
    const std::string prep_msg = prep ? std::string(pfnl_last_error()) : std::string();
    double v[8] = {(double)h->wdev_used, -(double)h->wdev_used, (double)h->wdev16_used, -(double)h->wdev16_used,
                   (double)h->wdev16s_used, -(double)h->wdev16s_used, prep ? 1.0 : 0.0, (rank == root && !h->weights_f16_ok) ? 1.0 : 0.0};
    if (int e = pfnl_comm_allreduce_f64(c, v, 8, PFNL_COMM_MAX)) return e;
    if (v[6] != 0.0) return prep ? fail(prep, prep_msg) : fail(PFNL_ERR_STATE, "another rank could not prepare to receive the weights");
    if (v[0] != -v[1] || v[2] != -v[3] || v[4] != -v[5]) return fail(PFNL_ERR_STATE, "ranks disagree on the weight blob size (geometry / theta-phi option)");
    if (int e = pfnl_comm_bcast(c, h->wdev.p, h->wdev_used * sizeof(float), root)) return e;
    if (int e = pfnl_comm_bcast(c, h->wdev16.p, h->wdev16_used * sizeof(float), root)) return e;
    if (int e = pfnl_comm_bcast(c, h->wdev16s.p, h->wdev16s_used * sizeof(float), root)) return e;
    if (rank != root) {
        h->weights_f16_ok = v[7] == 0.0;
        h->weights_external = true;
    }
    ++h->cfg_gen;
    return 0;
}

int pfnl_profile_enable(pfnl_handle* h, int enable) {
    if (!h) return fail(PFNL_ERR_INVALID, "NULL handle");
    if (!enable && h->prof) {
        if (prof_collect(h)) return fail(PFNL_ERR_HIP, "event collection failed");
    }
    h->prof = enable != 0;
    h->prof_mode = enable == 2 ? 2 : enable == 3 ? 3 : enable == 4 ? 4 : (enable ? 1 : 0);
    h->prof_gate = h->prof_mode != 3;
    h->run_n = 0;
    h->run_cls = -1;
    return 0;
}

int pfnl_profile_reset(pfnl_handle* h) {
    if (!h) return fail(PFNL_ERR_INVALID, "NULL handle");
    if (prof_collect(h)) return fail(PFNL_ERR_HIP, "event collection failed");
    for (int i = 0; i < PFNL_K_COUNT; ++i) {
        h->prof_ms[i] = 0;
        h->prof_n[i] = 0;
    }
    return 0;
}

int pfnl_profile_read(pfnl_handle* h, double* ms, int64_t* launches) {
    if (!h || !ms || !launches) return fail(PFNL_ERR_INVALID, "NULL argument");
    if (prof_collect(h)) return fail(PFNL_ERR_HIP, "event collection failed");
    for (int i = 0; i < PFNL_K_COUNT; ++i) {
        ms[i] = h->prof_ms[i];
        launches[i] = h->prof_n[i];
    }
    return 0;
}

int pfnl_debug_tap(pfnl_handle* h, const char* name, float* host_dst, size_t count) {
    if (!h || !name || !host_dst) return fail(PFNL_ERR_INVALID, "NULL argument");
    if (!h->lastB) return fail(PFNL_ERR_STATE, "no forward has run");
    HIPCHK(hipSetDevice(h->cfg.device_id));
    HIPCHK(hipDeviceSynchronize());
    const int B = h->lastB, H = h->lastH, W = h->lastW, T = h->cfg.num_frames;
    const std::string n(name);
    const float* src = nullptr;
    size_t need = 0;
    if (n == "nl_out") {
        need = (size_t)B * H * W * 3 * T;
        if (h->scratch.ensure(need)) return fail(PFNL_ERR_NOMEM, "scratch allocation failed");
        HIPCHK(pfnl::launch_nl_unpack(h->Xo.p, h->scratch.p, B, T, H, W, h->stream));
        HIPCHK(hipStreamSynchronize(h->stream));
        src = h->scratch.p;
    } else if (n == "trunk") {
        need = (size_t)B * T * H * W * 64;
        src = h->inp0.p;
        if (h->bf16) {
            if (h->scratch.ensure(need)) return fail(PFNL_ERR_NOMEM, "scratch allocation failed");
            HIPCHK(pfnl::launch_cast_bf16_f32(reinterpret_cast<const uint16_t*>(h->inp0.p), h->scratch.p, need, h->stream));
            HIPCHK(hipStreamSynchronize(h->stream));
            src = h->scratch.p;
        }
    } else if (n == "merge1") {
        need = (size_t)B * H * W * 48;
        if (count != need) return fail(PFNL_ERR_INVALID, "tap size mismatch");
        HIPCHK(hipMemcpy2D(host_dst, 48 * sizeof(float), h->merge.p, h->merge_cstride * sizeof(float), 48 * sizeof(float),
                           (size_t)B * H * W, hipMemcpyDeviceToHost));
        return 0;
    } else {
        return fail(PFNL_ERR_INVALID, "unknown tap " + n);
    }
    if (count != need) return fail(PFNL_ERR_INVALID, "tap size mismatch");
    HIPCHK(hipMemcpy(host_dst, src, need * sizeof(float), hipMemcpyDeviceToHost));
    return 0;
}

}
```

### pfnl_amd/csrc/common.h

```cpp
#pragma once
#include <hip/hip_runtime.h>
#include <stddef.h>
#include <stdint.h>

#include <atomic>

namespace pfnl {

typedef float f32x16 __attribute__((ext_vector_type(16)));
typedef float f32x4 __attribute__((ext_vector_type(4)));

__device__ __forceinline__ f32x16 mfma32(float a, float b, f32x16 c) {
    return __builtin_amdgcn_mfma_f32_32x32x2f32(a, b, c, 0, 0, 0);
}
__device__ __forceinline__ int drow(int r, int lane) { return (r & 3) + 8 * (r >> 2) + 4 * (lane >> 5); }

typedef unsigned pfnl_u32x4 __attribute__((ext_vector_type(4)));
template <int AUX = 0>
__device__ __forceinline__ void buffer_store_b128_guarded(pfnl_u32x4 v, __amdgpu_buffer_rsrc_t rs, int voffset, int soffset) {
    __builtin_amdgcn_raw_buffer_store_b128(v, rs, voffset, soffset, AUX);
    asm volatile("s_nop 1" ::"v"(v));
}

inline int device_cu_count() {
    static std::atomic<int> ncu[64];
    int dev = 0;
    if (hipGetDevice(&dev) != hipSuccess || dev < 0 || dev >= 64) return 0;
    int n = ncu[dev].load(std::memory_order_relaxed);
    if (!n) {
        hipDeviceProp_t prop;
        if (hipGetDeviceProperties(&prop, dev) != hipSuccess) return 0;
        n = prop.multiProcessorCount > 0 ? prop.multiProcessorCount : 0;
        ncu[dev].store(n, std::memory_order_relaxed);
    }
    return n;
}

inline int persistent_grid(int ncu) { return ncu >= 8 ? ncu / 8 * 8 : 8; }

__device__ __forceinline__ float lrelu(float v) { return fmaxf(v, 0.2f * v); }

constexpr int CONV_TW = 32;
constexpr int CONV_TH = 8;
constexpr int CONV_CK = 16;
constexpr int CONV_NPAD = 64;

struct ConvParams {
    const float* in;
    const float* wpack;
    const float* bias;
    const float* addend;
    const float* resid;
    float* out;
    int H, W;
    int in_cstride;
    int out_cstride;
    int cout;
    int chunks_per_frame;
    int frames_per_item;
    int nchunks;
    int add_div;
    int act;
};

hipError_t launch_conv_mfma(const ConvParams& p, int ksize, int items, hipStream_t s);
int conv_ck(int ksize);
size_t conv_pack_floats(int ksize, int cin);
void conv_pack_weights(const float* hwio, int ksize, int cin_total, int cin_begin, int cin,
                       int cout, float* dst);

hipError_t launch_conv1x1_stream(const float* in, const float* wpack, const float* bias, float* out, int items, int T,
                                 int HW, int act, hipStream_t s);
hipError_t launch_conv1x1_split16(const float* in, const uint16_t* wpack, const float* bias, float* out, int items, int T,
                                  int HW, int act, hipStream_t s,
                                  bool in_sf = false, bool out_sf = false);
size_t conv1x1_split16_pack_halfs(int T);
void conv1x1_split16_pack_weights(const float* hwio, int T, uint16_t* dst);
size_t conv1x1_pack_floats(int T);
void conv1x1_pack_weights(const float* hwio, int T, float* dst);

struct WinoParams {
    const float* in;
    const float* upack;
    const float* bias;
    const float* addend;
    const float* resid;
    float* out;
    int H, W;
    int add_div;
    int act;
    int items;
    long long in_item_stride;
    const float* in2;
    const float* upack2;
    int accum;
    long long upack_stride;
};
hipError_t launch_conv_wino(const WinoParams& p, hipStream_t s);
hipError_t launch_conv_wino_ws(const WinoParams& p, hipStream_t s);
size_t wino_pack_floats();
void wino_pack_weights(const float* hwio, int cin_total, int cin_begin, float* dst, int cout = 64);

int nl_padded_ch(int C);
hipError_t launch_nl_pack(const float* x, float* X, int B, int T, int H, int W, hipStream_t s);
size_t nl_partial_floats(int B, int N, int C);
hipError_t launch_nl_attn(const float* X, float* Xo, const float* Wp, const float* bp, float* partial, int B,
                          int N, int C, hipStream_t s, const float* Q = nullptr,
                          int q0 = 0, int q1 = -1);
hipError_t launch_nl_qproj(const float* X, const float* M, const float* c, float* Q, int B, int N, int C, hipStream_t s,
                           bool dot_column = false);
hipError_t launch_nl_attn_general(const float* X, const float* Kx, int Nk, float* Xo, const float* Wp, const float* bp,
                                  float* partial, int B, int N, int C, hipStream_t s, const float* Q, int q0, int q1, bool dot);
hipError_t launch_nl_pool(const float* X, float* Xs, int B, int h2, int w2, int sub, int C, hipStream_t s);
int nl_key_splits(int B, int N);
hipError_t launch_nl_merge(const float* X, const float* Zp, const float* ML, const float* bp, float* Xo, int B, int N, int C, int ks,
                           hipStream_t s, int q0 = 0, int q1 = -1);
hipError_t launch_nl_unpack(const float* Xo, float* out, int B, int T, int H, int W, hipStream_t s);

struct StripGeom {
    int yoff, Hs, core0, core1;
};
hipError_t launch_conv0(const float* Xo, const float* w75x64, const float* bias, float* out, int B,
                        int T, int H, int W, hipStream_t s, const StripGeom* strip = nullptr, bool force_f32 = false);
hipError_t launch_tail(const float* merge, const float* x, const float* w2, const float* b2,
                       float* out, int B, int T, int H, int W, int scale, int merge_cstride, hipStream_t s,
                       const StripGeom* strip = nullptr, unsigned* nonfinite = nullptr);
hipError_t launch_blur_decimate(const float* hr, float* lr, int F, int H, int W, int scale, hipStream_t s);
hipError_t launch_bicubic(const float* x, float* out, int B, int H, int W, int scale, hipStream_t s);
hipError_t run_mfma_selftest(int* mismatches);
hipError_t launch_gather_windows(const float* frames, float* win, int F, int first, int count, int T, size_t frame_floats,
                                 hipStream_t s);
hipError_t launch_quantise_u8(const float* sr, uint8_t* out, size_t n, hipStream_t s);
hipError_t launch_gather_windows_u8(const uint8_t* ring, float* win, int cap, long long last, long long first, int count, int T,
                                    size_t frame_bytes, hipStream_t s);

size_t score_scratch_bytes(int F, int H, int W);
hipError_t launch_score_y(const uint8_t* pred, const uint8_t* truth, int F, int H, int W, int sp_border, double* out, double* partial,
                          hipStream_t s);

}
```

### pfnl_amd/csrc/conv_bf16.h

```cpp
#pragma once
#include <hip/hip_runtime.h>
#include <stddef.h>
#include <stdint.h>

namespace pfnl {

struct ConvBf16Params {
    const uint16_t* in;
    const uint16_t* wpack;
    const float* bias;
    const uint16_t* addend;
    const uint16_t* resid;
    uint16_t* out;
    int H, W, items, add_div, act;
    const uint16_t* x_w;
    const float* x_bias;
    uint16_t* x_out;
    float* out_f32;
    int n_full, split_s, split_q;
    float* partial;
    int flat;
    const uint16_t* wpack16;
};
hipError_t launch_conv3x3_bf16(const ConvBf16Params& p, hipStream_t s);
hipError_t launch_conv3x3_bf16_v2(const ConvBf16Params& p, int mode, hipStream_t s);
hipError_t launch_conv3x3_bf16_v3(const ConvBf16Params& p, int mode, hipStream_t s);
hipError_t launch_c10_finalize_bf16(const ConvBf16Params& p, hipStream_t s);
hipError_t launch_conv1x1_bf16(const uint16_t* in, const uint16_t* wpack, const float* bias, uint16_t* out, int items, int T,
                               int HW, int act, hipStream_t s);
hipError_t launch_cast_bf16_f32(const uint16_t* in, float* out, size_t n, hipStream_t s);
hipError_t launch_cast_f32_bf16(const float* in, uint16_t* out, size_t n, hipStream_t s);
uint16_t bf16_rne(float f);
size_t conv3x3_bf16_pack_halfs();
void conv3x3_bf16_pack_weights(const float* hwio, int cin_total, int cin_begin, uint16_t* dst, int cout = 64);
void conv3x3_bf16_pack_weights16(const float* hwio, int cin_total, int cin_begin, uint16_t* dst);
size_t conv1x1_bf16_pack_halfs(int T);
void conv1x1_bf16_pack_weights(const float* hwio, int T, uint16_t* dst);
struct StripGeom;
hipError_t launch_conv0_bf16(const float* Xo, const float* w75x64, const float* bias, uint16_t* out, int B, int T, int H,
                             int W, hipStream_t s, const StripGeom* strip = nullptr);

}
```

### pfnl_amd/csrc/conv_split16.h

```cpp
#pragma once
#include <hip/hip_runtime.h>
#include <stddef.h>
#include <stdint.h>

#include "chain_order.h"

namespace pfnl {

struct ConvSplitParams {
    const float* in;
    const uint16_t* wpack;
    const float* bias;
    const float* addend;
    const float* resid;
    float* out;
    int H, W, items, add_div, act;
    int accum;
    int out_sf;
    const float* in2;
    const uint16_t* wpack2;
    const float* bias2;
    float* out2;
    int n_full, split_s, split_q;
    float* partial;
    int in_sf;
    int flat;
    const uint16_t* wpack_m16;
    const uint16_t* wpack2_m16;
};

hipError_t launch_conv3x3_split16(const ConvSplitParams& p, hipStream_t s);
size_t conv3x3_split16_pack_halfs();
void conv3x3_split16_pack_weights16(const float* hwio, int cin_total, int cin_begin, uint16_t* dst,
                                    bool perm_rows = false);
void conv3x3_split16_pack_weights(const float* hwio, int cin_total, int cin_begin, uint16_t* dst, int cout = 64,
                                  bool identity_rows = false);

hipError_t launch_conv3x3_c1c10(const ConvSplitParams& p, hipStream_t s);
hipError_t launch_c10_finalize(const ConvSplitParams& p, hipStream_t s);
size_t conv1x1_c10_pack_halfs(int T);
void conv1x1_c10_pack_weights(const float* hwio, int T, uint16_t* dst);

hipError_t launch_conv3x3_sf(const ConvSplitParams& p, hipStream_t s);
hipError_t launch_conv3x3_sf_chain(const ConvSplitParams& p, hipStream_t s);
hipError_t launch_sf_from_f32(const float* in, uint16_t* out, size_t npix, hipStream_t s);
hipError_t launch_sf_to_f32(const uint16_t* in, float* out, size_t npix, hipStream_t s);

size_t nl_f16_scratch_halfs(int B, int N);
hipError_t launch_nl_attn_f16(const float* X, float* Xo, const float* Wp, const float* bp, float* partial, uint16_t* scratch16,
                              int B, int N, int C, hipStream_t s, int q0 = 0, int q1 = -1, bool split = true,
                              bool prepacked = false);
bool nl_f16_fits_one_launch(int B, int N);
hipError_t launch_nl_pack_fused(const float* x, float* X, uint16_t* scratch16, int B, int T, int H, int W, hipStream_t s);

}
```

### pfnl_amd/csrc/misc_kernels.hip

```cpp
#include <cstdlib>

#include "common.h"
#include "conv_bf16.h"

namespace pfnl {

constexpr int C0_T = 16;
constexpr int C0_IN = C0_T + 4;

template <bool BF16OUT>
__global__ __launch_bounds__(256) void conv0_kernel(const float* __restrict__ Xo,
                                                    const float* __restrict__ w,
                                                    const float* __restrict__ bias,
                                                    float* __restrict__ out, int T, int H, int W,
                                                    int CP, int yoff, int Hs) {
    __shared__ __attribute__((aligned(16))) float smem0[256 * 36];
    float* const sw = smem0;
    float* const s_in = smem0 + 75 * 64;
    const int tid = threadIdx.x;
    const int f = blockIdx.z;
    const int b = f / T, t = f % T;
    const int x0 = blockIdx.x * C0_T, y0 = blockIdx.y * C0_T;
    const int W2 = W / 2, C3 = 3 * T;
    const float* Xb = Xo + (size_t)b * (H / 2) * W2 * CP;

    for (int i = tid; i < 75 * 64; i += 256) sw[i] = w[i];
    for (int i = tid; i < C0_IN * C0_IN * 3; i += 256) {
        const int c = i % 3, pix = i / 3;
        const int py = pix / C0_IN, px = pix % C0_IN;
        const int gy = yoff + y0 + py - 2, gx = x0 + px - 2;
        float v = 0.f;
        if (gy >= 0 && gy < H && gx >= 0 && gx < W)
            v = Xb[((size_t)(gy >> 1) * W2 + (gx >> 1)) * CP + ((gy & 1) * 2 + (gx & 1)) * C3 + 3 * t + c];
        s_in[i] = v;
    }
    __syncthreads();

    const int ty = tid / C0_T, tx = tid % C0_T;
    typedef float f32x2 __attribute__((ext_vector_type(2)));
    f32x2 acc[32];
#pragma unroll
    for (int o = 0; o < 32; ++o) acc[o] = f32x2{bias[2 * o], bias[2 * o + 1]};
    for (int ky = 0; ky < 5; ++ky) {
        for (int kx = 0; kx < 5; ++kx) {
            const float* ip = s_in + ((ty + ky) * C0_IN + tx + kx) * 3;
            const float* wp = sw + (ky * 5 + kx) * 3 * 64;
#pragma unroll
            for (int c = 0; c < 3; ++c) {
                const float a = ip[c];
                const f32x2 a2 = {a, a};
#pragma unroll
                for (int o4 = 0; o4 < 16; ++o4) {
                    const f32x4 wv = *reinterpret_cast<const f32x4*>(wp + c * 64 + o4 * 4);
                    acc[o4 * 2 + 0] = __builtin_elementwise_fma(a2, f32x2{wv.x, wv.y}, acc[o4 * 2 + 0]);
                    acc[o4 * 2 + 1] = __builtin_elementwise_fma(a2, f32x2{wv.z, wv.w}, acc[o4 * 2 + 1]);
                }
            }
        }
    }
    constexpr int SS = 36;
    float* slab = smem0;
    static_assert(75 * 64 + C0_IN * C0_IN * 3 <= 256 * SS, "weights + input tile must fit the slab they share LDS with");
#pragma unroll
    for (int hp = 0; hp < 2; ++hp) {
        __syncthreads();
#pragma unroll
        for (int o4 = 0; o4 < 8; ++o4) {
            const int o = hp * 16 + o4 * 2;
            *reinterpret_cast<f32x4*>(slab + tid * SS + o4 * 4) =
                f32x4{lrelu(acc[o].x), lrelu(acc[o].y), lrelu(acc[o + 1].x), lrelu(acc[o + 1].y)};
        }
        __syncthreads();
#pragma unroll
        for (int it = 0; it < 8; ++it) {
            const int id = it * 256 + tid;
            const int pix = id >> 3, q = id & 7;
            const int y = y0 + pix / C0_T, x = x0 + pix % C0_T;
            if (y < Hs && x < W) {
                const f32x4 v = *reinterpret_cast<const f32x4*>(slab + pix * SS + q * 4);
                if (BF16OUT) {
                    typedef __bf16 bf16x4 __attribute__((ext_vector_type(4)));
                    *reinterpret_cast<bf16x4*>(reinterpret_cast<uint16_t*>(out) + (((size_t)f * Hs + y) * W + x) * 64 + hp * 32 + q * 4) =
                        __builtin_convertvector(v, bf16x4);
                } else {
                    *reinterpret_cast<f32x4*>(out + (((size_t)f * Hs + y) * W + x) * 64 + hp * 32 + q * 4) = v;
                }
            }
        }
    }
}

constexpr int C0M_TW = 32, C0M_TH = 16, C0M_IW = C0M_TW + 4, C0M_IH = C0M_TH + 4;
constexpr int C0M_IN_DW = C0M_IH * C0M_IW * 3 + 4;
constexpr int C0M_W_BYTES = 5 * 2 * 2 * 1024;

template <bool BF16OUT>
__global__ __launch_bounds__(256) void conv0_mfma_kernel(const float* __restrict__ Xo, const float* __restrict__ w,
                                                         const float* __restrict__ bias, float* __restrict__ out, int T, int H,
                                                         int W, int CP, int yoff, int Hs) {
    typedef _Float16 h8 __attribute__((ext_vector_type(8)));
    typedef unsigned u32x4 __attribute__((ext_vector_type(4)));
    __shared__ __attribute__((aligned(16))) unsigned char sw[C0M_W_BYTES];
    __shared__ __attribute__((aligned(16))) unsigned s_in[C0M_IN_DW];
    const int tid = threadIdx.x, lane = tid & 63, wave = tid >> 6;
    const int f = blockIdx.z;
    const int b = f / T, t = f % T;
    const int x0 = blockIdx.x * C0M_TW, y0 = blockIdx.y * C0M_TH;
    const int W2 = W / 2, C3 = 3 * T;
    const float* Xb = Xo + (size_t)b * (H / 2) * W2 * CP;

    auto split1 = [](float v, unsigned short& hb, unsigned short& lb) {
        const _Float16 hi = (_Float16)v;
        const _Float16 lo = (_Float16)((v - (float)hi) * 2048.0f);
        hb = __builtin_bit_cast(unsigned short, hi);
        lb = __builtin_bit_cast(unsigned short, lo);
    };
    constexpr int C0M_WIT = (5 * 2 * 64 + 255) / 256, C0M_XIT = (C0M_IN_DW + 255) / 256;
    float wreg[C0M_WIT][8], xreg[C0M_XIT];
#pragma unroll
    for (int k = 0; k < C0M_WIT; ++k) {
        const int ent = min(tid + k * 256, 5 * 2 * 64 - 1);
        const int l = ent & 63, g = (ent >> 6) & 1, ky = ent >> 7;
#pragma unroll
        for (int e = 0; e < 8; ++e) {
            const int kp = 8 * (l >> 5) + e;
            const float wv = w[(size_t)(ky * 15 + min(kp, 14)) * 64 + 32 * g + (l & 31)];
            wreg[k][e] = kp < 15 ? wv : 0.f;
        }
    }
#pragma unroll
    for (int k = 0; k < C0M_XIT; ++k) {
        const int i = min(tid + k * 256, C0M_IN_DW - 1);
        const int c = i % 3, pix = i / 3;
        const int py = pix / C0M_IW, px = pix - py * C0M_IW;
        const int gy = yoff + y0 + py - 2, gx = x0 + px - 2;
        const bool in = py < C0M_IH && gy >= 0 && gy < H && gx >= 0 && gx < W;
        const int cy = in ? gy : 0, cx = in ? gx : 0;
        const float v = Xb[((size_t)(cy >> 1) * W2 + (cx >> 1)) * CP + ((cy & 1) * 2 + (cx & 1)) * C3 + 3 * t + c];
        xreg[k] = in ? v : 0.f;
    }
#pragma unroll
    for (int k = 0; k < C0M_WIT; ++k) {
        const int ent = tid + k * 256;
        if (ent >= 5 * 2 * 64) break;
        const int l = ent & 63, g = (ent >> 6) & 1, ky = ent >> 7;
        unsigned short hv[8], lv[8];
#pragma unroll
        for (int e = 0; e < 8; ++e) split1(wreg[k][e], hv[e], lv[e]);
        u32x4 hq, lq;
#pragma unroll
        for (int e = 0; e < 4; ++e) {
            hq[e] = hv[2 * e] | ((unsigned)hv[2 * e + 1] << 16);
            lq[e] = lv[2 * e] | ((unsigned)lv[2 * e + 1] << 16);
        }
        *reinterpret_cast<u32x4*>(sw + ((ky * 2 + 0) * 2 + g) * 1024 + l * 16) = hq;
        *reinterpret_cast<u32x4*>(sw + ((ky * 2 + 1) * 2 + g) * 1024 + l * 16) = lq;
    }
#pragma unroll
    for (int k = 0; k < C0M_XIT; ++k) {
        const int i = tid + k * 256;
        if (i >= C0M_IN_DW) break;
        unsigned short hb, lb;
        split1(xreg[k], hb, lb);
        s_in[i] = hb | ((unsigned)lb << 16);
    }
    __syncthreads();

    const int xl = lane & 31, kh = lane >> 5;
    const float bias0 = bias[xl], bias1 = bias[32 + xl];
    const unsigned char* const wl = sw + lane * 16;
#pragma unroll 1
    for (int rr = 0; rr < 4; ++rr) {
        const int row = wave * 4 + rr;
        if (y0 + row >= Hs) break;
        f32x16 am0, am1, ac0, ac1;
#pragma unroll
        for (int r = 0; r < 16; ++r) {
            am0[r] = bias0;
            am1[r] = bias1;
            ac0[r] = 0.f;
            ac1[r] = 0.f;
        }
#pragma unroll
        for (int ky = 0; ky < 5; ++ky) {
            const unsigned* ap = s_in + ((row + ky) * C0M_IW + xl) * 3 + 8 * kh;
            unsigned d[8];
#pragma unroll
            for (int e = 0; e < 8; ++e) d[e] = ap[e];
            u32x4 ahq, alq;
#pragma unroll
            for (int e = 0; e < 4; ++e) {
                ahq[e] = __builtin_amdgcn_perm(d[2 * e + 1], d[2 * e], 0x05040100u);
                alq[e] = __builtin_amdgcn_perm(d[2 * e + 1], d[2 * e], 0x07060302u);
            }
            const h8 ah = __builtin_bit_cast(h8, ahq), al = __builtin_bit_cast(h8, alq);
            const h8 w0h = *reinterpret_cast<const h8*>(wl + ((ky * 2 + 0) * 2 + 0) * 1024);
            const h8 w1h = *reinterpret_cast<const h8*>(wl + ((ky * 2 + 0) * 2 + 1) * 1024);
            const h8 w0l = *reinterpret_cast<const h8*>(wl + ((ky * 2 + 1) * 2 + 0) * 1024);
            const h8 w1l = *reinterpret_cast<const h8*>(wl + ((ky * 2 + 1) * 2 + 1) * 1024);
            am0 = __builtin_amdgcn_mfma_f32_32x32x16_f16(ah, w0h, am0, 0, 0, 0);
            am1 = __builtin_amdgcn_mfma_f32_32x32x16_f16(ah, w1h, am1, 0, 0, 0);
            ac0 = __builtin_amdgcn_mfma_f32_32x32x16_f16(ah, w0l, ac0, 0, 0, 0);
            ac1 = __builtin_amdgcn_mfma_f32_32x32x16_f16(ah, w1l, ac1, 0, 0, 0);
            ac0 = __builtin_amdgcn_mfma_f32_32x32x16_f16(al, w0h, ac0, 0, 0, 0);
            ac1 = __builtin_amdgcn_mfma_f32_32x32x16_f16(al, w1h, ac1, 0, 0, 0);
        }
        const size_t rowbase = (((size_t)f * Hs + y0 + row) * W + x0) * 64;
#pragma unroll
        for (int r = 0; r < 16; ++r) {
            const int px = drow(r, lane);
            const float v0 = lrelu(am0[r] + ac0[r] * (1.0f / 2048.0f)), v1 = lrelu(am1[r] + ac1[r] * (1.0f / 2048.0f));
            if (x0 + px < W) {
                if (BF16OUT) {
                    uint16_t* o16 = reinterpret_cast<uint16_t*>(out) + rowbase + (size_t)px * 64 + xl;
                    o16[0] = __builtin_bit_cast(unsigned short, (__bf16)v0);
                    o16[32] = __builtin_bit_cast(unsigned short, (__bf16)v1);
                } else {
                    float* o = out + rowbase + (size_t)px * 64 + xl;
                    o[0] = v0;
                    o[32] = v1;
                }
            }
        }
    }
}

static bool conv0_use_valu() {
    static const int v = [] {
        const char* e = getenv("PFNL_CONV0");
        return (e && e[0] == 'v') ? 1 : 0;
    }();
    return v != 0;
}

hipError_t launch_conv0(const float* Xo, const float* w75x64, const float* bias, float* out, int B,
                        int T, int H, int W, hipStream_t s, const StripGeom* strip, bool force_f32) {
    const int yoff = strip ? strip->yoff : 0, Hs = strip ? strip->Hs : H;
    if (!conv0_use_valu() && !force_f32) {
        dim3 grid((W + C0M_TW - 1) / C0M_TW, (Hs + C0M_TH - 1) / C0M_TH, B * T);
        hipLaunchKernelGGL(conv0_mfma_kernel<false>, grid, dim3(256), 0, s, Xo, w75x64, bias, out, T, H, W, nl_padded_ch(12 * T), yoff, Hs);
        return hipGetLastError();
    }
    dim3 grid((W + C0_T - 1) / C0_T, (Hs + C0_T - 1) / C0_T, B * T);
    hipLaunchKernelGGL(conv0_kernel<false>, grid, dim3(256), 0, s, Xo, w75x64, bias, out, T, H, W,
                       nl_padded_ch(12 * T), yoff, Hs);
    return hipGetLastError();
}

hipError_t launch_conv0_bf16(const float* Xo, const float* w75x64, const float* bias, uint16_t* out, int B, int T, int H,
                             int W, hipStream_t s, const StripGeom* strip) {
    const int yoff = strip ? strip->yoff : 0, Hs = strip ? strip->Hs : H;
    if (!conv0_use_valu()) {
        dim3 grid((W + C0M_TW - 1) / C0M_TW, (Hs + C0M_TH - 1) / C0M_TH, B * T);
        hipLaunchKernelGGL(conv0_mfma_kernel<true>, grid, dim3(256), 0, s, Xo, w75x64, bias, reinterpret_cast<float*>(out), T, H, W,
                           nl_padded_ch(12 * T), yoff, Hs);
        return hipGetLastError();
    }
    dim3 grid((W + C0_T - 1) / C0_T, (Hs + C0_T - 1) / C0_T, B * T);
    hipLaunchKernelGGL(conv0_kernel<true>, grid, dim3(256), 0, s, Xo, w75x64, bias, reinterpret_cast<float*>(out), T, H, W,
                       nl_padded_ch(12 * T), yoff, Hs);
    return hipGetLastError();
}

__device__ __forceinline__ void cubic_taps(float t, float w[4]) {
    const float A = -0.75f;
    const float d0 = 1.f + t, d1 = t, d2 = 1.f - t, d3 = 2.f - t;
    w[0] = ((A * d0 - 5.f * A) * d0 + 8.f * A) * d0 - 4.f * A;
    w[1] = ((A + 2.f) * d1 - (A + 3.f)) * d1 * d1 + 1.f;
    w[2] = ((A + 2.f) * d2 - (A + 3.f)) * d2 * d2 + 1.f;
    w[3] = ((A * d3 - 5.f * A) * d3 + 8.f * A) * d3 - 4.f * A;
}

__device__ __forceinline__ void bicubic_px(const float* __restrict__ src, int H, int W, size_t pitch,
                                           int scale, int oy, int ox, float res[3]) {
    const int iy = oy / scale, ix = ox / scale;
    float wy[4], wx[4];
    cubic_taps((float)(oy % scale) / (float)scale, wy);
    cubic_taps((float)(ox % scale) / (float)scale, wx);
    res[0] = res[1] = res[2] = 0.f;
#pragma unroll
    for (int a = 0; a < 4; ++a) {
        const int yy = min(max(iy - 1 + a, 0), H - 1);
        float row[3] = {0.f, 0.f, 0.f};
#pragma unroll
        for (int bb = 0; bb < 4; ++bb) {
            const int xx = min(max(ix - 1 + bb, 0), W - 1);
            const float* p = src + (size_t)yy * pitch + (size_t)xx * 3;
            row[0] = fmaf(wx[bb], p[0], row[0]);
            row[1] = fmaf(wx[bb], p[1], row[1]);
            row[2] = fmaf(wx[bb], p[2], row[2]);
        }
        res[0] = fmaf(wy[a], row[0], res[0]);
        res[1] = fmaf(wy[a], row[1], res[1]);
        res[2] = fmaf(wy[a], row[2], res[2]);
    }
}

__global__ void bicubic_kernel(const float* __restrict__ x, float* __restrict__ out, int B, int H,
                               int W, int scale) {
    const int OH = H * scale, OW = W * scale;
    const size_t total = (size_t)B * OH * OW;
    for (size_t i = (size_t)blockIdx.x * blockDim.x + threadIdx.x; i < total;
         i += (size_t)gridDim.x * blockDim.x) {
        const int ox = (int)(i % OW);
        const int oy = (int)((i / OW) % OH);
        const int b = (int)(i / ((size_t)OW * OH));
        float r[3];
        bicubic_px(x + (size_t)b * H * W * 3, H, W, (size_t)W * 3, scale, oy, ox, r);
        out[i * 3 + 0] = r[0];
        out[i * 3 + 1] = r[1];
        out[i * 3 + 2] = r[2];
    }
}

hipError_t launch_bicubic(const float* x, float* out, int B, int H, int W, int scale, hipStream_t s) {
    const size_t total = (size_t)B * H * W * scale * scale;
    const int blocks = (int)((total + 255) / 256 < 8192 ? (total + 255) / 256 : 8192);
    hipLaunchKernelGGL(bicubic_kernel, dim3(blocks), dim3(256), 0, s, x, out, B, H, W, scale);
    return hipGetLastError();
}

template <int CO>
__global__ __launch_bounds__(256) void tail_kernel(const float* __restrict__ merge,
                                                   const float* __restrict__ x,
                                                   const float* __restrict__ w2,
                                                   const float* __restrict__ b2,
                                                   float* __restrict__ out, int B, int T, int H, int W, int MS,
                                                   int yoff, int Hs, int core0, int core1,
                                                   unsigned* __restrict__ nonfinite) {
    constexpr int SCALE = (CO == 12) ? 4 : 2;
    const int H2 = 2 * Hs, W2 = 2 * W;
    const int X = blockIdx.x * 32 + (threadIdx.x & 31);
    const int Y = blockIdx.y * 8 + (threadIdx.x >> 5);
    const int b = blockIdx.z;
    if (X >= W2 || Y >= H2 || (Y >> 1) < core0 || (Y >> 1) >= core1) return;
    const float* mb = merge + (size_t)b * Hs * W * MS;

    float acc[CO];
#pragma unroll
    for (int o = 0; o < CO; ++o) acc[o] = b2[o];
#pragma unroll
    for (int dy = 0; dy < 3; ++dy) {
        const int yy = Y + dy - 1;
        if (yy < 0 || yy >= H2) continue;
#pragma unroll
        for (int dx = 0; dx < 3; ++dx) {
            const int xx = X + dx - 1;
            if (xx < 0 || xx >= W2) continue;
            const float4* src = reinterpret_cast<const float4*>(
                mb + ((size_t)(yy >> 1) * W + (xx >> 1)) * MS + ((yy & 1) * 2 + (xx & 1)) * 12);
            const float4 v0 = src[0], v1 = src[1], v2 = src[2];
            const float v[12] = {v0.x, v0.y, v0.z, v0.w, v1.x, v1.y, v1.z, v1.w, v2.x, v2.y, v2.z, v2.w};
            const float* wp = w2 + (dy * 3 + dx) * 12 * CO;
#pragma unroll
            for (int k = 0; k < 12; ++k)
#pragma unroll
                for (int o = 0; o < CO; ++o) acc[o] = fmaf(v[k], wp[k * CO + o], acc[o]);
        }
    }

    const float* xc = x + (((size_t)b * T + T / 2) * H) * W * 3;
    const int OH = SCALE * H, OW = SCALE * W;
    float* ob = out + (size_t)b * OH * OW * 3;
    bool bad = false;
    if (CO == 12) {
        const int Yf = Y + 2 * yoff;
        const int iy = Yf >> 1, ix = X >> 1;
        float wy[2][4], wx[2][4];
#pragma unroll
        for (int i = 0; i < 2; ++i) {
            cubic_taps((float)(2 * (Yf & 1) + i) / 4.0f, wy[i]);
            cubic_taps((float)(2 * (X & 1) + i) / 4.0f, wx[i]);
        }
        float res[2][2][3];
#pragma unroll
        for (int i = 0; i < 2; ++i)
#pragma unroll
            for (int j = 0; j < 2; ++j) res[i][j][0] = res[i][j][1] = res[i][j][2] = 0.f;
#pragma unroll
        for (int a = 0; a < 4; ++a) {
            const int yy = min(max(iy - 1 + a, 0), H - 1);
            float px[4][3];
#pragma unroll
            for (int bb = 0; bb < 4; ++bb) {
                const int xx = min(max(ix - 1 + bb, 0), W - 1);
                const float* p = xc + ((size_t)yy * W + xx) * 3;
                px[bb][0] = p[0];
                px[bb][1] = p[1];
                px[bb][2] = p[2];
            }
#pragma unroll
            for (int j = 0; j < 2; ++j) {
                float row[3] = {0.f, 0.f, 0.f};
#pragma unroll
                for (int bb = 0; bb < 4; ++bb) {
                    row[0] = fmaf(wx[j][bb], px[bb][0], row[0]);
                    row[1] = fmaf(wx[j][bb], px[bb][1], row[1]);
                    row[2] = fmaf(wx[j][bb], px[bb][2], row[2]);
                }
#pragma unroll
                for (int i = 0; i < 2; ++i) {
                    res[i][j][0] = fmaf(wy[i][a], row[0], res[i][j][0]);
                    res[i][j][1] = fmaf(wy[i][a], row[1], res[i][j][1]);
                    res[i][j][2] = fmaf(wy[i][a], row[2], res[i][j][2]);
                }
            }
        }
#pragma unroll
        for (int i = 0; i < 2; ++i) {
            const int oy = 2 * Yf + i;
            float v[6];
#pragma unroll
            for (int j = 0; j < 2; ++j)
#pragma unroll
                for (int c = 0; c < 3; ++c) {
                    v[3 * j + c] = acc[(2 * i + j) * 3 + c] + res[i][j][c];
                    bad |= !(fabsf(v[3 * j + c]) <= 3.4028234e38f);
                }
            float* dstf = ob + ((size_t)oy * OW + 2 * X) * 3;
            if ((reinterpret_cast<uintptr_t>(out) & 7) == 0) {
                float2* dst = reinterpret_cast<float2*>(dstf);
                dst[0] = make_float2(v[0], v[1]);
                dst[1] = make_float2(v[2], v[3]);
                dst[2] = make_float2(v[4], v[5]);
            } else {
#pragma unroll
                for (int k = 0; k < 6; ++k) dstf[k] = v[k];
            }
        }
    } else {
        float bic[3];
        bicubic_px(xc, H, W, (size_t)W * 3, SCALE, Y + 2 * yoff, X, bic);
        float* dst = ob + ((size_t)(Y + 2 * yoff) * OW + X) * 3;
#pragma unroll
        for (int c = 0; c < 3; ++c) {
            const float v = acc[c] + bic[c];
            bad |= !(fabsf(v) <= 3.4028234e38f);
            dst[c] = v;
        }
    }
    if (bad && nonfinite) __hip_atomic_store(nonfinite, 1u, __ATOMIC_RELAXED, __HIP_MEMORY_SCOPE_SYSTEM);
}

hipError_t launch_tail(const float* merge, const float* x, const float* w2, const float* b2, float* out,
                       int B, int T, int H, int W, int scale, int merge_cstride, hipStream_t s, const StripGeom* strip, unsigned* nonfinite) {
    if (merge_cstride != 48 && merge_cstride != 64) return hipErrorInvalidValue;
    const StripGeom g = strip ? *strip : StripGeom{0, H, 0, H};
    dim3 grid((2 * W + 31) / 32, (2 * g.Hs + 7) / 8, B);
    if (scale == 4)
        hipLaunchKernelGGL(tail_kernel<12>, grid, dim3(256), 0, s, merge, x, w2, b2, out, B, T, H, W, merge_cstride, g.yoff, g.Hs, g.core0, g.core1, nonfinite);
    else if (scale == 2)
        hipLaunchKernelGGL(tail_kernel<3>, grid, dim3(256), 0, s, merge, x, w2, b2, out, B, T, H, W, merge_cstride, g.yoff, g.Hs, g.core0, g.core1, nonfinite);
    else
        return hipErrorInvalidValue;
    return hipGetLastError();
}

__constant__ float c_blur[13 * 13];

__global__ void blur_decimate_kernel(const float* __restrict__ hr, float* __restrict__ lr, int F, int H, int W,
                                     int oh, int ow, int scale) {
    const size_t total = (size_t)F * oh * ow;
    for (size_t i = (size_t)blockIdx.x * blockDim.x + threadIdx.x; i < total; i += (size_t)gridDim.x * blockDim.x) {
        const int ox = (int)(i % ow);
        const int oy = (int)((i / ow) % oh);
        const int f = (int)(i / ((size_t)ow * oh));
        const float* src = hr + (size_t)f * H * W * 3;
        float a0 = 0.f, a1 = 0.f, a2 = 0.f;
        for (int ky = 0; ky < 13; ++ky) {
            int y = oy * scale + ky - 6;
            y = y < 0 ? -y : (y >= H ? 2 * H - 2 - y : y);
            for (int kx = 0; kx < 13; ++kx) {
                int x = ox * scale + kx - 6;
                x = x < 0 ? -x : (x >= W ? 2 * W - 2 - x : x);
                const float w = c_blur[ky * 13 + kx];
                const float* p = src + ((size_t)y * W + x) * 3;
                a0 = fmaf(w, p[0], a0);
                a1 = fmaf(w, p[1], a1);
                a2 = fmaf(w, p[2], a2);
            }
        }
        lr[i * 3 + 0] = a0;
        lr[i * 3 + 1] = a1;
        lr[i * 3 + 2] = a2;
    }
}

hipError_t launch_blur_decimate(const float* hr, float* lr, int F, int H, int W, int scale, hipStream_t s) {
    static std::atomic<int> init[64];
    int dev = 0;
    hipError_t e = hipGetDevice(&dev);
    if (e != hipSuccess) return e;
    if (dev >= 0 && dev < 64 && !init[dev]) {
        double k[13], sum = 0.0;
        for (int i = 0; i < 13; ++i) {
            const double d = (i - 6) / 1.6;
            k[i] = exp(-0.5 * d * d);
            sum += k[i];
        }
        float w[169];
        for (int a = 0; a < 13; ++a)
            for (int b = 0; b < 13; ++b) w[a * 13 + b] = (float)((k[a] / sum) * (k[b] / sum));
        e = hipMemcpyToSymbol(HIP_SYMBOL(c_blur), w, sizeof(w));
        if (e != hipSuccess) return e;
        init[dev] = 1;
    }
    const int oh = (H + scale - 1) / scale, ow = (W + scale - 1) / scale;
    const size_t total = (size_t)F * oh * ow;
    const int blocks = (int)((total + 255) / 256 < 8192 ? (total + 255) / 256 : 8192);
    hipLaunchKernelGGL(blur_decimate_kernel, dim3(blocks), dim3(256), 0, s, hr, lr, F, H, W, oh, ow, scale);
    return hipGetLastError();
}

__global__ void mfma_selftest_kernel(int* mismatches) {
    const int lane = threadIdx.x & 63;
    const int i = lane & 31, k = lane >> 5;
    const float a = (float)(3 * i + 7 * k + 1);
    const float bv = (float)(5 * (lane & 31) - 11 * k + 2);
    f32x16 d;
    for (int r = 0; r < 16; ++r) d[r] = 0.f;
    d = mfma32(a, bv, d);
    int bad = 0;
    for (int r = 0; r < 16; ++r) {
        const int row = drow(r, lane), col = lane & 31;
        float ref = 0.f;
        for (int kk = 0; kk < 2; ++kk)
            ref += (float)(3 * row + 7 * kk + 1) * (float)(5 * col - 11 * kk + 2);
        if (d[r] != ref) ++bad;
    }
    if (bad) atomicAdd(mismatches, bad);
}

hipError_t run_mfma_selftest(int* mismatches) {
    int* d = nullptr;
    hipError_t e = hipMalloc(&d, sizeof(int));
    if (e != hipSuccess) return e;
    hipMemset(d, 0, sizeof(int));
    hipLaunchKernelGGL(mfma_selftest_kernel, dim3(1), dim3(64), 0, 0, d);
    e = hipMemcpy(mismatches, d, sizeof(int), hipMemcpyDeviceToHost);
    hipFree(d);
    return e;
}

}

namespace pfnl {

__global__ __launch_bounds__(256) void gather_windows_kernel(const f32x4* __restrict__ frames, f32x4* __restrict__ win, int F,
                                                             int first, int count, int T, size_t frame_f4) {
    const size_t total = (size_t)count * T * frame_f4;
    for (size_t i = (size_t)blockIdx.x * 256 + threadIdx.x; i < total; i += (size_t)gridDim.x * 256) {
        const size_t e = i % frame_f4;
        const int wt = (int)(i / frame_f4);
        const int w = wt / T, t = wt - w * T;
        int f = first + w + t - T / 2;
        f = f < 0 ? 0 : (f > F - 1 ? F - 1 : f);
        win[i] = frames[(size_t)f * frame_f4 + e];
    }
}

hipError_t launch_gather_windows(const float* frames, float* win, int F, int first, int count, int T, size_t frame_floats,
                                 hipStream_t s) {
    if (frame_floats % 4) return hipErrorInvalidValue;
    const size_t total = (size_t)count * T * (frame_floats / 4);
    const int blocks = (int)((total + 255) / 256 < 8192 ? (total + 255) / 256 : 8192);
    hipLaunchKernelGGL(gather_windows_kernel, dim3(blocks ? blocks : 1), dim3(256), 0, s, reinterpret_cast<const f32x4*>(frames),
                       reinterpret_cast<f32x4*>(win), F, first, count, T, frame_floats / 4);
    return hipGetLastError();
}

__global__ __launch_bounds__(256) void quantise_u8_kernel(const f32x4* __restrict__ sr, uint32_t* __restrict__ out, size_t n4) {
    for (size_t i = (size_t)blockIdx.x * 256 + threadIdx.x; i < n4; i += (size_t)gridDim.x * 256) {
        const f32x4 v = sr[i];
        const uint32_t a = (uint32_t)rintf(fminf(fmaxf(v.x * 255.0f, 0.f), 255.f));
        const uint32_t b = (uint32_t)rintf(fminf(fmaxf(v.y * 255.0f, 0.f), 255.f));
        const uint32_t c = (uint32_t)rintf(fminf(fmaxf(v.z * 255.0f, 0.f), 255.f));
        const uint32_t d = (uint32_t)rintf(fminf(fmaxf(v.w * 255.0f, 0.f), 255.f));
        out[i] = a | (b << 8) | (c << 16) | (d << 24);
    }
}

hipError_t launch_quantise_u8(const float* sr, uint8_t* out, size_t n, hipStream_t s) {
    if (n % 4) return hipErrorInvalidValue;
    const size_t n4 = n / 4;
    const int blocks = (int)((n4 + 255) / 256 < 8192 ? (n4 + 255) / 256 : 8192);
    hipLaunchKernelGGL(quantise_u8_kernel, dim3(blocks ? blocks : 1), dim3(256), 0, s, reinterpret_cast<const f32x4*>(sr),
                       reinterpret_cast<uint32_t*>(out), n4);
    return hipGetLastError();
}

}
```

### pfnl_amd/csrc/nonlocal_f16.hip

```cpp
#include <algorithm>
#include <cstdlib>
#include <type_traits>

#include "common.h"
#include "conv_bf16.h"
#include "conv_split16.h"

namespace pfnl {

typedef _Float16 bf16x8 __attribute__((ext_vector_type(8)));
typedef unsigned u32x4 __attribute__((ext_vector_type(4)));

constexpr int NF_KT = 64;
constexpr int NF_KROW = 208;
constexpr int NF_VROW = 144;
constexpr int NF_CP = 96;
constexpr int NF_THREADS = 512;
constexpr int NF_QB = NF_THREADS / 2;

constexpr float NF_XSCALE = 128.0f;
constexpr float NF_SINV = 1.0f / (128.0f * 128.0f);
constexpr float NF_PSHIFT = 14.0f;
__device__ __forceinline__ unsigned short bf16_bits(float f) {
    const _Float16 b = (_Float16)f;
    return __builtin_bit_cast(unsigned short, b);
}
__device__ __forceinline__ float bf16_float(unsigned short u) { return (float)__builtin_bit_cast(_Float16, u); }

template <bool FROMX>
__global__ __launch_bounds__(256) void nl_pack_f16_kernel(const float* __restrict__ X, uint16_t* __restrict__ Khi, uint16_t* __restrict__ Klo,
                                                          uint16_t* __restrict__ Vthi, uint16_t* __restrict__ Vtlo, int B, int N, int Npad, int C,
                                                          int CPin, const float* __restrict__ xraw, float* __restrict__ Xout, int H, int W) {
    __shared__ uint16_t vth[NF_CP][34], vtl[NF_CP][34];
    const int nblk = Npad / 32;
    const int b = blockIdx.x / nblk, n0 = (blockIdx.x - b * nblk) * 32;
    const int tid = threadIdx.x;
    [[maybe_unused]] const int C3 = C / 4, T = C / 12, W2 = W / 2;
#pragma unroll
    for (int j = 0; j < 32 * NF_CP / 256; ++j) {
        const int i = tid + 256 * j;
        const int kk = i / NF_CP, c = i - kk * NF_CP;
        const int n = n0 + kk;
        float raw = 0.f;
        if constexpr (FROMX) {
            if (n < N && c < C) {
                const int sub = c / C3, k = c - sub * C3;
                const int t = k / 3, cc = k - 3 * t;
                const int y = 2 * (n / W2) + (sub >> 1), xx = 2 * (n % W2) + (sub & 1);
                raw = xraw[((((size_t)b * T + t) * H + y) * W + xx) * 3 + cc];
            }
            if (n < N && c < CPin) Xout[((size_t)b * N + n) * CPin + c] = raw;
        } else {
            raw = (n < N && c < C) ? X[((size_t)b * N + n) * CPin + c] : 0.f;
        }
        const float v = raw * NF_XSCALE;
        const unsigned short hi = bf16_bits(v);
        const unsigned short lo = bf16_bits(v - bf16_float(hi));
        Khi[((size_t)b * Npad + n) * NF_CP + c] = (n >= N && c == C) ? (unsigned short)0xfbff : (c == C + 1 ? (unsigned short)0x3c00 : hi);
        Klo[((size_t)b * Npad + n) * NF_CP + c] = lo;
        const int e = (kk & 3) | (((kk >> 3) & 1) << 2), kh = (kk >> 2) & 1, t = kk >> 4;
        const int pos = 16 * t + 8 * kh + e;
        vth[c][pos] = c == C ? (unsigned short)0x3c00 : hi;
        vtl[c][pos] = c == C ? (unsigned short)0 : lo;
    }
    __syncthreads();
#pragma unroll
    for (int j = 0; j < 16 * NF_CP / 256; ++j) {
        const int i = tid + 256 * j;
        const int c = i >> 4, pp = (i & 15) * 2;
        const size_t vp = ((size_t)b * NF_CP + c) * Npad + n0 + pp;
        *reinterpret_cast<unsigned*>(Vthi + vp) = (unsigned)vth[c][pp] | ((unsigned)vth[c][pp + 1] << 16);
        *reinterpret_cast<unsigned*>(Vtlo + vp) = (unsigned)vtl[c][pp] | ((unsigned)vtl[c][pp + 1] << 16);
    }
}



template <bool SPLIT>
struct NfSW {
    static constexpr int KLO_OFF = NF_KT * NF_KROW;
    static constexpr int VHI_OFF = SPLIT ? 2 * NF_KT * NF_KROW : NF_KT * NF_KROW;
    static constexpr int VLO_OFF = VHI_OFF + NF_CP * NF_VROW;
    static constexpr int TILE_BYTES = SPLIT ? VLO_OFF + NF_CP * NF_VROW : VLO_OFF;
    static constexpr int NSLOT = SPLIT ? 3 : 5;
    static constexpr int PIECES = SPLIT ? 53 : 32;
    static constexpr int SLOT_BYTES = PIECES * 1024;
    static constexpr int PW = (PIECES + 7) / 8;
    static constexpr int LDS_BYTES = NSLOT * SLOT_BYTES;
    static_assert(TILE_BYTES <= SLOT_BYTES && LDS_BYTES <= 160 * 1024, "LDS budget");
    static_assert(SPLIT || PIECES % 8 == 0, "the vmcnt wait of a ring deeper than 3 counts on equal shares");
};

__device__ __forceinline__ void nf_dma16(__amdgpu_buffer_rsrc_t rs, unsigned lds_dst, int voff) {
    unsigned keep;
    asm volatile("s_mov_b32 %0, m0\n\ts_mov_b32 m0, %2\n\ts_nop 0\n\tbuffer_load_dwordx4 %1, %3, 0 offen lds\n\ts_mov_b32 m0, %0"
                 : "=&s"(keep) : "v"(voff), "s"(lds_dst), "s"(rs) : "memory");
}
#define NF_BARRIER() asm volatile("s_waitcnt lgkmcnt(0)\n\ts_barrier" ::: "memory")

template <int C, bool SPLIT>
__global__ __launch_bounds__(NF_THREADS, 2) void nl_attn_f16_sw_kernel(const float* __restrict__ X, const uint16_t* __restrict__ K16,
                                                                 unsigned rel_klo, unsigned rel_vhi, unsigned rel_vlo, unsigned scratch_bytes,
                                                                 float* __restrict__ Xo, const float* __restrict__ Wp,
                                                                 const float* __restrict__ bp, float* __restrict__ Zp,
                                                                 float* __restrict__ ML, int N, int Npad, int q0, int q1) {
    using G = NfSW<SPLIT>;
    constexpr int CT = 3;
    constexpr int CP = (C + 31) / 32 * 32;
    static_assert(C + 1 < NF_CP && C % 2 == 0, "needs two pad channels inside 96");
    extern __shared__ __attribute__((aligned(16))) unsigned char sm[];

    const int tid = threadIdx.x;
    const int lane = tid & 63;
    const int wave = __builtin_amdgcn_readfirstlane(tid >> 6);
    const int xl = lane & 31;
    const int kh = lane >> 5;
    const int b = blockIdx.y;
    const float* Xb = X + (size_t)b * N * CP;
    float* Xob = Xo + (size_t)b * N * CP;
    const int q = q0 + blockIdx.x * NF_QB + (tid >> 6) * 32 + xl;
    const int qc = q < q1 ? q : q1 - 1;

    constexpr float LOG2E = 1.4426950408889634f;
    bf16x8 qh[6];
    [[maybe_unused]] bf16x8 ql[6];
#pragma unroll
    for (int ks = 0; ks < 6; ++ks)
#pragma unroll
        for (int e = 0; e < 8; ++e) {
            const int c = 16 * ks + 8 * kh + e;
            const float v = c < C ? Xb[(size_t)qc * CP + c] * (LOG2E * NF_XSCALE) : (c == C ? 1024.f : 0.f);
            const _Float16 h = (_Float16)v;
            qh[ks][e] = h;
            if constexpr (SPLIT) ql[ks][e] = (_Float16)(v - (float)h);
        }
    constexpr int CS = C;
    constexpr int LCT = CS / 32, LI = CS % 32;
    constexpr int LKH = (LI % 8) >= 4 ? 1 : 0, LR = (LI / 8) * 4 + (LI % 8) % 4;

    f32x16 o[CT];
#pragma unroll
    for (int ct = 0; ct < CT; ++ct)
#pragma unroll
        for (int r = 0; r < 16; ++r) o[ct][r] = 0.f;
    float m = -INFINITY;

    int srel[G::PW];
#pragma unroll
    for (int k = 0; k < G::PW; ++k) {
        const int p = (wave + 8 * k) * 1024 + 16 * lane;
        int sr = 0x7fffffff;
        if (p < NF_KT * NF_KROW || (SPLIT && p < 2 * NF_KT * NF_KROW)) {
            const bool lo = p >= NF_KT * NF_KROW;
            const int r = p - (lo ? NF_KT * NF_KROW : 0);
            const int row = r / NF_KROW, col = r - row * NF_KROW;
            if (col < NF_CP * 2) {
                sr = (int)((lo ? rel_klo : 0u) + (unsigned)(((size_t)b * Npad + row) * (NF_CP * 2)) + col);
            }
        } else if (p < G::TILE_BYTES) {
            const bool lo = SPLIT && p >= G::VLO_OFF;
            const int r = p - (lo ? G::VLO_OFF : G::VHI_OFF);
            const int ch = r / NF_VROW, col = r - ch * NF_VROW;
            if (col < NF_KT * 2) {
                sr = (int)((lo ? rel_vlo : rel_vhi) + (unsigned)(((size_t)b * NF_CP + ch) * Npad * 2) + col);
            }
        }
        srel[k] = sr;
    }
    const unsigned lds0 = (unsigned)(uintptr_t)sm;
    auto tile_piece = [&](int k, int kt, int slot, bool live) __attribute__((always_inline)) {
        const int i = wave + 8 * k;
        if (G::PIECES % 8 == 0 || 8 * k + 7 < G::PIECES || i < G::PIECES) {
            const __amdgpu_buffer_rsrc_t rs = __builtin_amdgcn_make_buffer_rsrc(const_cast<uint16_t*>(K16), 0, live ? scratch_bytes : 0, 0x00020000);
            const int k0 = kt * NF_KT;
            const bool isk = i * 1024 < (SPLIT ? 2 : 1) * NF_KT * NF_KROW;
            const int off = (int)((unsigned)srel[k] + (unsigned)(k0 * (isk ? NF_CP * 2 : 2)));
            nf_dma16(rs, lds0 + slot * G::SLOT_BYTES + i * 1024, off);
        }
    };

    const int ntiles = (N + NF_KT - 1) / NF_KT;
    const int ksp = gridDim.z, sp = blockIdx.z;
    const int kt0 = (int)((long long)ntiles * sp / ksp), kt1 = (int)((long long)ntiles * (sp + 1) / ksp);
#pragma unroll
    for (int j = 0; j < G::NSLOT - 1; ++j)
#pragma unroll
        for (int k = 0; k < G::PW; ++k) tile_piece(k, kt0 + j, j, kt0 + j < kt1);
#pragma unroll
    for (int k = 0; k < G::PW; ++k) tile_piece(k, 0, G::NSLOT - 1, false);
    asm volatile("s_waitcnt vmcnt(0)" ::: "memory");
    __syncthreads();

    bf16x8 pt[2][2];
    [[maybe_unused]] bf16x8 pl[2][2];
#pragma unroll
    for (int i = 0; i < 2; ++i)
#pragma unroll
        for (int j = 0; j < 2; ++j)
#pragma unroll
            for (int e = 0; e < 8; ++e) {
                pt[i][j][e] = (_Float16)0.f;
                if constexpr (SPLIT) pl[i][j][e] = (_Float16)0.f;
            }
#define NP_MFMA(a_, b_, c_) __builtin_amdgcn_mfma_f32_32x32x16_f16(a_, b_, c_, 0, 0, 0)
    f32x16 st[2];
    constexpr int NQ = SPLIT ? 18 : 6, NR = SPLIT ? 24 : 12;
#define NP_PIN(v_) asm volatile("" : "+v"(v_))
    constexpr int AHEAD = 4;
    constexpr int RING = AHEAD + 2;
    bf16x8 rb[RING];
    auto half_body = [&](auto hc, const unsigned char* qbuf, const unsigned char* vbuf, int kt_fill, int s_fill) __attribute__((always_inline)) {
        constexpr int H = decltype(hc)::value;
        f32x16& stc = st[H];
        f32x16& stn = st[H ^ 1];
        const unsigned char* const kah = qbuf + ((1 - H) * 32 + xl) * NF_KROW + kh * 16;
        const unsigned char* const vah = vbuf + G::VHI_OFF + xl * NF_VROW + kh * 16 + (1 - H) * 64;
        auto read = [&](auto qc) __attribute__((always_inline)) {
            constexpr int q = decltype(qc)::value;
            if constexpr (q < NR) {
                constexpr int d = q % RING;
                if constexpr (!SPLIT) {
                    if constexpr (q < 6) rb[d] = *reinterpret_cast<const bf16x8*>(kah + q * 32);
                    else rb[d] = *reinterpret_cast<const bf16x8*>(vah + ((q - 6) % 3) * 32 * NF_VROW + ((q - 6) / 3) * 32);
                } else {
                    if constexpr (q < 12) rb[d] = *reinterpret_cast<const bf16x8*>(kah + (q & 1) * G::KLO_OFF + (q >> 1) * 32);
                    else {
                        constexpr int u = (q - 12) >> 1, lo = (q - 12) & 1;
                        rb[d] = *reinterpret_cast<const bf16x8*>(vah + lo * (G::VLO_OFF - G::VHI_OFF) + (u % 3) * 32 * NF_VROW + (u / 3) * 32);
                    }
                }
            }
        };
        auto mfma = [&](auto ic) __attribute__((always_inline)) {
            constexpr int i = decltype(ic)::value;
            constexpr int q = SPLIT ? 2 * (i / 3) + (i % 3 == 2) : i;
            const bf16x8 a = rb[q % RING];
            if constexpr (i < NQ) {
                constexpr int ks = SPLIT ? i / 3 : i;
                bf16x8 bq = qh[ks];
                if constexpr (SPLIT) {
                    if constexpr (i % 3 == 1) bq = ql[ks];
                }
                if constexpr (i == 0) {
                    f32x16 z;
#pragma unroll
                    for (int r = 0; r < 16; ++r) z[r] = 0.f;
                    stn = NP_MFMA(a, bq, z);
                } else {
                    stn = NP_MFMA(a, bq, stn);
                }
            } else {
                constexpr int j = i - NQ;
                constexpr int u = SPLIT ? j / 3 : j;
                constexpr int jj = u / 3, ct = u % 3;
                bf16x8 bp = pt[1 - H][jj];
                if constexpr (SPLIT) {
                    if constexpr (j % 3 == 1) bp = pl[1 - H][jj];
                }
                o[ct] = NP_MFMA(a, bp, o[ct]);
            }
        };
#pragma unroll
        for (int q0_ = 0; q0_ <= AHEAD; ++q0_) {
            if (q0_ == 0) read(std::integral_constant<int, 0>{});
            if (q0_ == 1) read(std::integral_constant<int, 1>{});
            if (q0_ == 2) read(std::integral_constant<int, 2>{});
            if (q0_ == 3) read(std::integral_constant<int, 3>{});
            if (q0_ == 4) read(std::integral_constant<int, 4>{});
            if (q0_ == 5) read(std::integral_constant<int, 5>{});
            if (q0_ == 6) read(std::integral_constant<int, 6>{});
        }
        __builtin_amdgcn_sched_barrier(0);
        float tmax = 0.f, tsw = 0.f, alpha = 1.f, shift = 0.f;
        [[maybe_unused]] float pv0 = 0.f, pv1 = 0.f;
        auto gap = [&](auto ic) __attribute__((always_inline)) {
            constexpr int i = decltype(ic)::value;
            mfma(ic);
            __builtin_amdgcn_sched_barrier(0);
            {
                constexpr int qn = (SPLIT ? 2 * (i / 3) + (i % 3 == 2) : i) + AHEAD + 1;
                constexpr int qp = i == 0 ? AHEAD + 1 : (SPLIT ? 2 * ((i - 1) / 3) + ((i - 1) % 3 == 2) : i - 1) + AHEAD + 1;
                if constexpr (qn > qp) read(std::integral_constant<int, qn - 1 < NR ? (qn - 1 >= qp ? qn - 1 : NR) : NR>{});
            }
            if constexpr (i == 0) {
                float ta, tb;
                asm("v_max3_f32 %0, %1, %2, %3" : "=v"(ta) : "v"(stc[0]), "v"(stc[1]), "v"(stc[2]));
                asm("v_max3_f32 %0, %1, %2, %3" : "=v"(tb) : "v"(stc[8]), "v"(stc[9]), "v"(stc[10]));
                asm("v_max3_f32 %0, %1, %2, %3" : "=v"(ta) : "v"(ta), "v"(stc[3]), "v"(stc[4]));
                asm("v_max3_f32 %0, %1, %2, %3" : "=v"(tb) : "v"(tb), "v"(stc[11]), "v"(stc[12]));
                asm("v_max3_f32 %0, %1, %2, %3" : "=v"(ta) : "v"(ta), "v"(stc[5]), "v"(stc[6]));
                asm("v_max3_f32 %0, %1, %2, %3" : "=v"(tb) : "v"(tb), "v"(stc[13]), "v"(stc[14]));
                asm("v_max3_f32 %0, %1, %2, %3" : "=v"(ta) : "v"(ta), "v"(stc[7]), "v"(stc[15]));
                asm("v_max_f32 %0, %1, %2" : "=v"(tmax) : "v"(ta), "v"(tb));
                NP_PIN(tmax);
            } else if constexpr (i == 1) {
                tsw = __shfl_xor(tmax, 32);
                NP_PIN(tsw);
            } else if constexpr (i == 3) {
                asm("v_max_f32 %0, %1, %2" : "=v"(tmax) : "v"(tmax), "v"(tsw));
                tmax *= NF_SINV;
                const float mn = fmaxf(m, tmax);
                alpha = __builtin_amdgcn_exp2f(m - mn);
                shift = NF_PSHIFT - mn;
                m = mn;
                NP_PIN(shift);
                NP_PIN(alpha);
            }
            if constexpr (!SPLIT) {
                if constexpr (i >= 4) {
                    constexpr int r = 2 * (i - 4);
                    const float a0 = __builtin_amdgcn_exp2f(__builtin_fmaf(stc[r], NF_SINV, shift));
                    const float a1 = __builtin_amdgcn_exp2f(__builtin_fmaf(stc[r + 1], NF_SINV, shift));
                    pt[H][r >> 3][r & 7] = (_Float16)a0;
                    pt[H][r >> 3][(r & 7) + 1] = (_Float16)a1;
                    NP_PIN(pt[H][r >> 3]);
                }
            } else {
                if constexpr (i >= 4 && i % 2 == 0) {
                    constexpr int r = 2 * ((i - 4) / 4);
                    if constexpr (((i - 4) / 2) % 2 == 0) {
                        pv0 = __builtin_amdgcn_exp2f(__builtin_fmaf(stc[r], NF_SINV, shift));
                        pv1 = __builtin_amdgcn_exp2f(__builtin_fmaf(stc[r + 1], NF_SINV, shift));
                        asm volatile("" : "+v"(pv0), "+v"(pv1));
                    } else {
                        const _Float16 h0 = (_Float16)pv0, h1 = (_Float16)pv1;
                        pt[H][r >> 3][r & 7] = h0;
                        pt[H][r >> 3][(r & 7) + 1] = h1;
                        pl[H][r >> 3][r & 7] = (_Float16)(pv0 - (float)h0);
                        pl[H][r >> 3][(r & 7) + 1] = (_Float16)(pv1 - (float)h1);
                        NP_PIN(pt[H][r >> 3]);
                        NP_PIN(pl[H][r >> 3]);
                    }
                }
            }
            if constexpr (H == 1) {
                constexpr int step = SPLIT ? 5 : 3;
                if constexpr (i % step == 2 && i / step < G::PW) tile_piece(i / step, kt_fill, s_fill, kt_fill < kt1);
            }
            __builtin_amdgcn_sched_barrier(0);
        };
        gap(std::integral_constant<int, 0>{});
        gap(std::integral_constant<int, 1>{});
        gap(std::integral_constant<int, 2>{});
        gap(std::integral_constant<int, 3>{});
        gap(std::integral_constant<int, 4>{});
        gap(std::integral_constant<int, 5>{});
        gap(std::integral_constant<int, 6>{});
        gap(std::integral_constant<int, 7>{});
        gap(std::integral_constant<int, 8>{});
        gap(std::integral_constant<int, 9>{});
        gap(std::integral_constant<int, 10>{});
        gap(std::integral_constant<int, 11>{});
        if constexpr (SPLIT) {
            gap(std::integral_constant<int, 12>{});
            gap(std::integral_constant<int, 13>{});
            gap(std::integral_constant<int, 14>{});
            gap(std::integral_constant<int, 15>{});
            gap(std::integral_constant<int, 16>{});
            gap(std::integral_constant<int, 17>{});
            gap(std::integral_constant<int, 18>{});
            gap(std::integral_constant<int, 19>{});
            gap(std::integral_constant<int, 20>{});
            gap(std::integral_constant<int, 21>{});
            gap(std::integral_constant<int, 22>{});
            gap(std::integral_constant<int, 23>{});
            gap(std::integral_constant<int, 24>{});
            gap(std::integral_constant<int, 25>{});
            gap(std::integral_constant<int, 26>{});
            gap(std::integral_constant<int, 27>{});
            gap(std::integral_constant<int, 28>{});
            gap(std::integral_constant<int, 29>{});
            gap(std::integral_constant<int, 30>{});
            gap(std::integral_constant<int, 31>{});
            gap(std::integral_constant<int, 32>{});
            gap(std::integral_constant<int, 33>{});
            gap(std::integral_constant<int, 34>{});
            gap(std::integral_constant<int, 35>{});
        }
        if (!__all(alpha == 1.0f)) {
#pragma unroll
            for (int ct = 0; ct < CT; ++ct)
#pragma unroll
                for (int r = 0; r < 16; ++r) o[ct][r] *= alpha;
        }
    };

    int s_cur = 0, s_prv = G::NSLOT - 1, s_nxt = 1;
    {
        const unsigned char* const kah = sm + xl * NF_KROW + kh * 16;
#pragma unroll
        for (int r = 0; r < 16; ++r) st[0][r] = 0.f;
#pragma unroll
        for (int ks = 0; ks < 6; ++ks) {
            const bf16x8 ah = *reinterpret_cast<const bf16x8*>(kah + ks * 32);
            st[0] = NP_MFMA(ah, qh[ks], st[0]);
            if constexpr (SPLIT) {
                const bf16x8 al = *reinterpret_cast<const bf16x8*>(kah + G::KLO_OFF + ks * 32);
                st[0] = NP_MFMA(ah, ql[ks], st[0]);
                st[0] = NP_MFMA(al, qh[ks], st[0]);
            }
        }
    }
    for (int kt = kt0; kt < kt1; ++kt) {
        const unsigned char* const cur = sm + s_cur * G::SLOT_BYTES;
        const unsigned char* const prv = sm + s_prv * G::SLOT_BYTES;
        const unsigned char* const nxt = sm + s_nxt * G::SLOT_BYTES;
        half_body(std::integral_constant<int, 0>{}, cur, prv, 0, 0);
        asm volatile("s_waitcnt vmcnt(%0)" ::"n"((G::NSLOT - 3) * G::PW) : "memory");
        NF_BARRIER();
        half_body(std::integral_constant<int, 1>{}, nxt, cur, kt + G::NSLOT - 1, s_prv);
        s_prv = s_cur;
        s_cur = s_nxt;
        s_nxt = s_nxt + 1 == G::NSLOT ? 0 : s_nxt + 1;
    }
    {
        const unsigned char* const vah = sm + s_prv * G::SLOT_BYTES + G::VHI_OFF + xl * NF_VROW + kh * 16 + 64;
#pragma unroll
        for (int jj = 0; jj < 2; ++jj)
#pragma unroll
            for (int ct = 0; ct < CT; ++ct) {
                const bf16x8 vh = *reinterpret_cast<const bf16x8*>(vah + ct * 32 * NF_VROW + jj * 32);
                o[ct] = NP_MFMA(vh, pt[1][jj], o[ct]);
                if constexpr (SPLIT) {
                    const bf16x8 vl = *reinterpret_cast<const bf16x8*>(vah + (G::VLO_OFF - G::VHI_OFF) + ct * 32 * NF_VROW + jj * 32);
                    o[ct] = NP_MFMA(vh, pl[1][jj], o[ct]);
                    o[ct] = NP_MFMA(vl, pt[1][jj], o[ct]);
                }
            }
    }

    float l = o[LCT][LR];
    {
        const float lo = __shfl_xor(l, 32);
        if (kh != LKH) l = lo;
    }
    const float inv = (1.0f / NF_XSCALE) / l;
#pragma unroll
    for (int ct = 0; ct < CT; ++ct)
#pragma unroll
        for (int r = 0; r < 16; ++r) o[ct][r] *= inv;

    constexpr int CTW = CP / 32;
    constexpr int NPAIR = CTW * CTW * 2;
    static_assert(NPAIR * 2048 <= G::SLOT_BYTES * G::NSLOT, "W' in operand form fits the ring");
    asm volatile("s_waitcnt vmcnt(0)" ::: "memory");
    __syncthreads();
    for (int pp = tid; pp < NPAIR * 64; pp += NF_THREADS) {
        const int ln = pp & 63, g = pp >> 6;
        const int t = g & 1, ctp = (g >> 1) % CTW, cotp = (g >> 1) / CTW;
        const float* w = Wp + (size_t)(ctp * 32 + 16 * t + 4 * (ln >> 5)) * CP + cotp * 32 + (ln & 31);
        bf16x8 h, l;
#pragma unroll
        for (int i = 0; i < 8; ++i) {
            const float v = w[((i & 3) + 8 * (i >> 2)) * CP];
            const _Float16 hh = (_Float16)v;
            h[i] = hh;
            l[i] = (_Float16)((v - (float)hh) * 2048.0f);
        }
        *reinterpret_cast<bf16x8*>(sm + g * 2048 + ln * 16) = h;
        *reinterpret_cast<bf16x8*>(sm + g * 2048 + 1024 + ln * 16) = l;
    }
    bf16x8 bh[CTW][2], bl[CTW][2];
#pragma unroll
    for (int ct = 0; ct < CTW; ++ct)
#pragma unroll
        for (int t = 0; t < 2; ++t)
#pragma unroll
            for (int i = 0; i < 8; ++i) {
                const float v = o[ct][8 * t + i];
                const _Float16 hh = (_Float16)v;
                bh[ct][t][i] = hh;
                bl[ct][t][i] = (_Float16)((v - (float)hh) * 2048.0f);
            }
    __syncthreads();
#pragma unroll
    for (int cot = 0; cot < CTW; ++cot) {
        f32x16 z, zc;
#pragma unroll
        for (int r = 0; r < 16; ++r) z[r] = zc[r] = 0.f;
#pragma unroll
        for (int ct = 0; ct < CTW; ++ct)
#pragma unroll
            for (int t = 0; t < 2; ++t) {
                const unsigned char* wa = sm + ((cot * CTW + ct) * 2 + t) * 2048 + lane * 16;
                const bf16x8 ah = *reinterpret_cast<const bf16x8*>(wa), al = *reinterpret_cast<const bf16x8*>(wa + 1024);
                z = NP_MFMA(ah, bh[ct][t], z);
                zc = NP_MFMA(ah, bl[ct][t], zc);
                zc = NP_MFMA(al, bh[ct][t], zc);
            }
#pragma unroll
        for (int r = 0; r < 16; ++r) z[r] = (z[r] + zc[r] * (1.0f / 2048.0f)) * (ksp == 1 ? 1.0f : l);
        if (q < q1) {
            if (ksp == 1) {
#pragma unroll
                for (int r = 0; r < 16; ++r) {
                    const int co = cot * 32 + drow(r, lane);
                    if (co < C) {
                        const size_t idx = (size_t)q * CP + co;
                        Xob[idx] = Xb[idx] + z[r] + bp[co];
                    }
                }
            } else {
                float* zp = Zp + (((size_t)b * ksp + sp) * N + q) * CP;
#pragma unroll
                for (int r = 0; r < 16; ++r) zp[cot * 32 + drow(r, lane)] = z[r];
            }
        }
    }
    if (ksp > 1 && q < q1 && kh == 0) {
        float* ml = ML + (((size_t)b * ksp + sp) * N + q) * 2;
        ml[0] = m;
        ml[1] = l;
    }
}

size_t nl_f16_scratch_halfs(int B, int N) {
    const size_t npad = (size_t)(N + 31) / 32 * 32 + 64;
    return 4 * (size_t)B * NF_CP * npad;
}

static size_t nl_f16_chunk_limit() {
    static const size_t lim = [] {
        const char* e = std::getenv("PFNL_NL_CHUNK_BYTES");
        const long long v = e ? std::atoll(e) : 0;
        return v > 0 ? (size_t)v : (size_t)0x7fff0000ull;
    }();
    return lim;
}

static hipError_t nl_attn_f16_run(const float* X, float* Xo, const float* Wp, const float* bp, float* partial, uint16_t* scratch16,
                                  int B, int N, int C, hipStream_t s, int q0, int q1, bool split, int ks_cap, bool prepacked = false);

bool nl_f16_fits_one_launch(int B, int N) { return 2 * nl_f16_scratch_halfs(1, N) * (size_t)B <= nl_f16_chunk_limit(); }

hipError_t launch_nl_pack_fused(const float* x, float* X, uint16_t* scratch16, int B, int T, int H, int W, hipStream_t s) {
    const int C = 12 * T, N = (H / 2) * (W / 2);
    if (!x || !X || !scratch16 || B < 1 || (C != 84 && C != 60 && C != 36) || (H & 1) || (W & 1) || !nl_f16_fits_one_launch(B, N)) return hipErrorInvalidValue;
    const int CP = nl_padded_ch(C);
    const int npad = (N + 31) / 32 * 32 + 64;
    uint16_t* Khi = scratch16;
    uint16_t* Klo = Khi + (size_t)B * npad * NF_CP;
    uint16_t* Vthi = Klo + (size_t)B * npad * NF_CP;
    uint16_t* Vtlo = Vthi + (size_t)B * NF_CP * npad;
    hipLaunchKernelGGL(nl_pack_f16_kernel<true>, dim3(B * (npad / 32)), dim3(256), 0, s, nullptr, Khi, Klo, Vthi, Vtlo, B, N, npad, C, CP, x, X, H, W);
    return hipGetLastError();
}

hipError_t launch_nl_attn_f16(const float* X, float* Xo, const float* Wp, const float* bp, float* partial, uint16_t* scratch16,
                               int B, int N, int C, hipStream_t s, int q0, int q1, bool split, bool prepacked) {
    if (B < 1 || N < 1) return hipErrorInvalidValue;
    if (prepacked) {
        if (!nl_f16_fits_one_launch(B, N)) return hipErrorInvalidValue;
        return nl_attn_f16_run(X, Xo, Wp, bp, partial, scratch16, B, N, C, s, q0, q1, split, nl_key_splits(B, N), true);
    }
    const size_t per_clip = 2 * nl_f16_scratch_halfs(1, N);
    const int ks_cap = nl_key_splits(B, N);
    int bc = (int)std::min<size_t>((size_t)B, std::max<size_t>(1, nl_f16_chunk_limit() / per_clip));
    const int CP = nl_padded_ch(C);
    for (int b0 = 0; b0 < B; b0 += bc) {
        const int nb = std::min(bc, B - b0);
        hipError_t e = nl_attn_f16_run(X + (size_t)b0 * N * CP, Xo + (size_t)b0 * N * CP, Wp, bp, partial, scratch16, nb, N, C, s, q0, q1, split, ks_cap);
        if (e != hipSuccess) return e;
    }
    return hipSuccess;
}

static hipError_t nl_attn_f16_run(const float* X, float* Xo, const float* Wp, const float* bp, float* partial, uint16_t* scratch16,
                                  int B, int N, int C, hipStream_t s, int q0, int q1, bool split, int ks_cap, bool prepacked) {
    if (C != 84 && C != 60 && C != 36) return hipErrorInvalidValue;
    if (q1 < 0) q1 = N;
    if (q0 < 0 || q0 >= q1 || q1 > N) return hipErrorInvalidValue;
    const int CP = nl_padded_ch(C);
    const int npad = (N + 31) / 32 * 32 + 64;
    uint16_t* Khi = scratch16;
    uint16_t* Klo = Khi + (size_t)B * npad * NF_CP;
    uint16_t* Vthi = Klo + (size_t)B * npad * NF_CP;
    uint16_t* Vtlo = Vthi + (size_t)B * NF_CP * npad;
    if (!prepacked) {
        hipLaunchKernelGGL(nl_pack_f16_kernel<false>, dim3(B * (npad / 32)), dim3(256), 0, s, X, Khi, Klo, Vthi, Vtlo, B, N, npad, C, CP, nullptr, nullptr, 0, 0);
        hipError_t e = hipGetLastError();
        if (e != hipSuccess) return e;
    }
    const int ks_max = std::min(nl_key_splits(B, N), ks_cap);
    int ks = 1;
    {
        const long long qb = (long long)((q1 - q0 + NF_QB - 1) / NF_QB) * B;
        double best = 1e30;
        for (int k = 1; k <= ks_max; ++k) {
            const double t = (double)((qb * k + 255) / 256) / k;
            if (t < best - 1e-9) {
                best = t;
                ks = k;
            }
        }
    }
    if (ks > 1 && !partial) return hipErrorInvalidValue;
    float* Zp = partial;
    float* ML = partial ? partial + (size_t)B * ks * N * CP : nullptr;
    dim3 grid((q1 - q0 + NF_QB - 1) / NF_QB, B, ks);
    dim3 block(NF_THREADS);
    int dev = 0;
    if (hipGetDevice(&dev) != hipSuccess || dev < 0 || dev >= 64) return hipErrorInvalidDevice;
    const size_t scratch_bytes = 2 * nl_f16_scratch_halfs(B, N);
    static std::atomic<int> attr_sw[64];
    if (!attr_sw[dev]) {
        const void* const fns[6] = {
            reinterpret_cast<const void*>(nl_attn_f16_sw_kernel<84, true>), reinterpret_cast<const void*>(nl_attn_f16_sw_kernel<60, true>),
            reinterpret_cast<const void*>(nl_attn_f16_sw_kernel<36, true>), reinterpret_cast<const void*>(nl_attn_f16_sw_kernel<84, false>),
            reinterpret_cast<const void*>(nl_attn_f16_sw_kernel<60, false>), reinterpret_cast<const void*>(nl_attn_f16_sw_kernel<36, false>),
        };
        const int lds[2] = {NfSW<true>::LDS_BYTES, NfSW<false>::LDS_BYTES};
        for (int i = 0; i < 6; ++i) {
            hipError_t e = hipFuncSetAttribute(fns[i], hipFuncAttributeMaxDynamicSharedMemorySize, lds[i / 3]);
            if (e != hipSuccess) return e;
        }
        attr_sw[dev] = 1;
    }
    const unsigned rel_klo = (unsigned)((Klo - Khi) * 2), rel_vhi = (unsigned)((Vthi - Khi) * 2), rel_vlo = (unsigned)((Vtlo - Khi) * 2);
#define NP_LAUNCH(C_, S_) hipLaunchKernelGGL((nl_attn_f16_sw_kernel<C_, S_>), grid, block, (NfSW<S_>::LDS_BYTES), s, X, Khi, rel_klo, rel_vhi, rel_vlo, \
                                             (unsigned)scratch_bytes, Xo, Wp, bp, Zp, ML, N, npad, q0, q1)
    switch (C) {
        case 84: if (split) NP_LAUNCH(84, true); else NP_LAUNCH(84, false); break;
        case 60: if (split) NP_LAUNCH(60, true); else NP_LAUNCH(60, false); break;
        case 36: if (split) NP_LAUNCH(36, true); else NP_LAUNCH(36, false); break;
    }
#undef NP_LAUNCH
    hipError_t e = hipGetLastError();
    if (e != hipSuccess || ks == 1) return e;
    return launch_nl_merge(X, Zp, ML, bp, Xo, B, N, C, ks, s, q0, q1);
}

}
```

### pfnl_amd/engine.py

```python
from __future__ import annotations

import ctypes as C
import os
from typing import Dict, Optional

import numpy as np

from . import _capi
from .spec import PFNLGeometry, check_weights


def _is_torch(x) -> bool:
    return type(x).__module__.startswith("torch")


class _PinnedPool:

    def __init__(self):
        import threading
        self._free = {}
        self._free_bytes = 0
        self._lock = threading.RLock()

    def _cap(self) -> int:
        return int(float(os.environ.get("PFNL_PINNED_POOL_MB", "256")) * (1 << 20))

    def array(self, shape, nbytes: int) -> Optional[np.ndarray]:
        import weakref
        lib = _capi.load_library()
        ptr = None
        with self._lock:
            lst = self._free.get(nbytes)
            if lst:
                ptr = lst.pop()
                self._free_bytes -= nbytes
        if ptr is None:
            p = C.c_void_p()
            if lib.pfnl_host_alloc(nbytes, C.byref(p)) != 0 or not p.value:
                return None
            ptr = p.value
        base = (C.c_float * (nbytes // 4)).from_address(ptr)
        fin = weakref.finalize(base, self._give, ptr, nbytes)
        fin.atexit = False
        return np.ctypeslib.as_array(base).reshape(shape)

    def _give(self, ptr: int, nbytes: int) -> None:
        keep = False
        with self._lock:
            if self._free_bytes + nbytes <= self._cap():
                self._free.setdefault(nbytes, []).append(ptr)
                self._free_bytes += nbytes
                keep = True
        if not keep:
            try:
                _capi.load_library().pfnl_host_free(C.c_void_p(ptr))
            except Exception:
                pass

    def free_bytes(self) -> int:
        return self._free_bytes


_pinned_pool = _PinnedPool()


class PFNLEngine:
    def __init__(self, geom: PFNLGeometry = PFNLGeometry(), device: int = 0):
        self.geom = geom
        self.device = int(device)
        self._lib = _capi.load_library()
        cfg = _capi.pfnl_config(geom.num_frames, geom.scale, geom.mf, geom.num_block, self.device,
                                (C.c_int32 * 3)(0, 0, 0))
        h = C.c_void_p()
        _capi.check(self._lib.pfnl_create(C.byref(cfg), C.byref(h)))
        self._h = h
        self._ready = False
        self._options: Dict[str, str] = {}

    def close(self) -> None:
        if getattr(self, "_h", None):
            self._lib.pfnl_destroy(self._h)
            self._h = None

    def __del__(self):
        try:
            self.close()
        except Exception:
            pass

    def load_weights(self, weights: Dict[str, np.ndarray]) -> None:
        check_weights(self.geom, weights)
        opt = [(n, s) for n, s in self.geom.optional_weight_shapes() if n in weights]
        for name, shape in list(self.geom.weight_shapes()) + opt:
            arr = np.ascontiguousarray(weights[name], dtype=np.float32)
            shp = (C.c_int64 * len(shape))(*shape)
            _capi.check(self._lib.pfnl_set_weight(self._h, name.encode(), arr.ctypes.data_as(C.c_void_p),
                                                  shp, len(shape)))
        _capi.check(self._lib.pfnl_finalize_weights(self._h))
        self._ready = True

    def copy_weights_from(self, other: "PFNLEngine") -> None:
        _capi.check(self._lib.pfnl_copy_weights(self._h, other._h))
        self._ready = True

    OPTION_KEYS = ("precision", "strict_fp32", "conv3x3", "conv1x1", "conv2", "merge1", "nonlocal", "nl_type", "nl_sub_sample", "small", "small_c10",
                   "split16_sf", "split16_chain", "split16_c10", "split16_mid", "split16_sf0", "split16_splitchains", "bf16_conv10", "bf16_mfma", "split16_mfma", "graph")

    def clone(self) -> "PFNLEngine":
        other = PFNLEngine(self.geom, device=self.device)
        for k in self.OPTION_KEYS:
            other.set_option(k, self.get_option(k))
        other.copy_weights_from(self)
        return other

    def set_option(self, key: str, value: str) -> None:
        _capi.check(self._lib.pfnl_set_option(self._h, key.encode(), value.encode()))
        self._options[key] = value

    def option(self, key: str, default: Optional[str] = None) -> Optional[str]:
        return self._options.get(key, default)

    def missing_weights(self) -> int:
        n = C.c_int(0)
        _capi.check(self._lib.pfnl_missing_weights(self._h, C.byref(n)))
        return n.value

    def _check_input(self, shape, dtype_ok: bool):
        if len(shape) != 5:
            raise ValueError(f"expected [B,T,H,W,3], got shape {tuple(shape)}")
        B, T, H, W, c = (int(s) for s in shape)
        if c != 3 or T != self.geom.num_frames:
            raise ValueError(f"expected [B,{self.geom.num_frames},H,W,3], got {tuple(shape)}")
        if B < 1 or H < 2 or W < 2:
            raise ValueError(f"empty or degenerate input {tuple(shape)}")
        if H % 2 or W % 2:
            raise ValueError("H and W must be even (tf.space_to_depth(2), reference model/pfnl.py:57)")
        if not dtype_ok:
            raise TypeError("input must be float32")
        if not self._ready:
            raise RuntimeError("weights have not been loaded")
        return B, T, H, W

    def out_shape(self, B: int, H: int, W: int):
        s = self.geom.scale
        return (B, 1, s * H, s * W, 3)

    def forward(self, x):
        if _is_torch(x):
            import torch
            if x.is_cuda:
                B, T, H, W = self._check_input(x.shape, x.dtype == torch.float32)
                if x.device.index != self.device:
                    raise ValueError(f"tensor on {x.device}, engine on cuda:{self.device}")
                x = x.contiguous()
                out = torch.empty(self.out_shape(B, H, W), dtype=torch.float32, device=x.device)
                stream = torch.cuda.current_stream(x.device).cuda_stream
                _capi.check(self._lib.pfnl_forward(self._h, C.c_void_p(x.data_ptr()), 1,
                                                   C.c_void_p(out.data_ptr()), 1, B, H, W,
                                                   C.c_void_p(stream)))
                return out
            return torch.from_numpy(self.forward(x.detach().numpy()))
        x = np.asarray(x)
        B, T, H, W = self._check_input(x.shape, x.dtype == np.float32)
        x = np.ascontiguousarray(x)
        out = self._host_output(self.out_shape(B, H, W))
        _capi.check(self._lib.pfnl_forward(self._h, x.ctypes.data_as(C.c_void_p), 0,
                                           out.ctypes.data_as(C.c_void_p), 0, B, H, W, None))
        return out

    @staticmethod
    def _host_output(shape) -> np.ndarray:
        nbytes = int(np.prod(shape)) * 4
        if nbytes >= (512 << 10) and os.environ.get("PFNL_HOST_OUTPUT", "pinned") != "pageable":
            arr = _pinned_pool.array(shape, nbytes)
            if arr is not None:
                return arr
        return np.empty(shape, np.float32)

    @staticmethod
    def host_output_mode() -> str:
        return "pageable" if os.environ.get("PFNL_HOST_OUTPUT", "pinned") == "pageable" else "pinned (pfnl_host_alloc pool)"

    def forward_device(self, in_ptr: int, out_ptr: int, B: int, H: int, W: int, stream: int = 0) -> None:
        self._check_input((B, self.geom.num_frames, H, W, 3), True)
        _capi.check(self._lib.pfnl_forward(self._h, C.c_void_p(in_ptr), 1, C.c_void_p(out_ptr), 1, B, H, W,
                                           C.c_void_p(stream) if stream else None))

    def forward_strip(self, x, out, row0: int, nrows: int) -> None:
        import torch
        B, T, H, W = self._check_input(x.shape, x.dtype == torch.float32)
        if not (x.is_cuda and out.is_cuda and out.dtype == torch.float32 and tuple(out.shape) == self.out_shape(B, H, W)
                and x.is_contiguous() and out.is_contiguous()):
            raise ValueError("forward_strip needs contiguous float32 cuda tensors, out of the full output shape")
        stream = torch.cuda.current_stream(x.device).cuda_stream
        _capi.check(self._lib.pfnl_forward_strip(self._h, C.c_void_p(x.data_ptr()), C.c_void_p(out.data_ptr()), B, H, W,
                                                 int(row0), int(nrows), C.c_void_p(stream) if stream else None))

    def open_stream(self, H: int, W: int, batch: int = 1):
        from .stream import VideoStream
        return VideoStream(self, H, W, batch)

    def sync(self) -> None:
        _capi.check(self._lib.pfnl_sync(self._h))

    def range_flagged(self) -> bool:
        f = C.c_int(0)
        _capi.check(self._lib.pfnl_range_flag(self._h, C.byref(f)))
        return bool(f.value)

    def range_reruns(self) -> int:
        n = C.c_longlong(0)
        _capi.check(self._lib.pfnl_range_reruns(self._h, C.byref(n)))
        return n.value

    def workspace_bytes(self, B: int, H: int, W: int) -> int:
        n = C.c_size_t(0)
        _capi.check(self._lib.pfnl_workspace_bytes(self._h, B, H, W, C.byref(n)))
        return n.value

    def plan(self, B: int, H: int, W: int) -> Dict[str, object]:
        buf = C.create_string_buffer(512)
        _capi.check(self._lib.pfnl_plan(self._h, B, H, W, buf, 512))
        toks = buf.value.decode().split()
        d: Dict[str, object] = {"structure": toks[0]}
        for t in toks[1:]:
            k, v = t.split("=", 1)
            d[k] = int(v) if v.lstrip("-").isdigit() else v
        return d

    def get_option(self, key: str) -> str:
        buf = C.create_string_buffer(64)
        _capi.check(self._lib.pfnl_get_option(self._h, key.encode(), buf, 64))
        return buf.value.decode()

    def profile(self, enable) -> None:
        _capi.check(self._lib.pfnl_profile_enable(self._h, int(enable)))

    def profile_reset(self) -> None:
        _capi.check(self._lib.pfnl_profile_reset(self._h))

    def profile_read(self) -> Dict[str, Dict[str, float]]:
        n = len(_capi.K_NAMES)
        ms = (C.c_double * n)()
        cnt = (C.c_int64 * n)()
        _capi.check(self._lib.pfnl_profile_read(self._h, ms, cnt))
        return {k: {"ms": ms[i], "launches": int(cnt[i])} for i, k in enumerate(_capi.K_NAMES)}

    def tap(self, name: str, B: int, H: int, W: int) -> np.ndarray:
        T = self.geom.num_frames
        shape = {"nl_out": (B, H, W, 3 * T), "trunk": (B, T, H, W, 64), "merge1": (B, H, W, 48)}[name]
        out = np.empty(shape, np.float32)
        _capi.check(self._lib.pfnl_debug_tap(self._h, name.encode(), out.ctypes.data_as(C.c_void_p), out.size))
        return out
```

Before: 957.6.

## Fuse non-local split-key merge into conv0 input load and overlap attention prologue

When the non-local attention uses several key splits, the separate merge kernel is skipped. conv0's MFMA kernel instead reads the partial numerators and max/denominator values and combines them with the residual and bias while loading its input tile. This removes one launch and a full write and read of Xo, at the cost of redundant merge arithmetic in conv0's halo pixels. A lazy merge is kept for debug reads of nl_out. Separately, the attention kernel's prologue now waits only for the first tile slot instead of draining all prefetches, so loads can overlap.

```diff
diff --git a/pfnl_amd/csrc/capi.hip b/pfnl_amd/csrc/capi.hip
--- a/pfnl_amd/csrc/capi.hip
+++ b/pfnl_amd/csrc/capi.hip
@@ -193,6 +193,8 @@
     size_t off16s_m1 = 0;
     int m1_algo = 0;
     int conv_algo = 5;
+    bool nl_merge_fuse = true;
+    int xo_pending_ks = 0;
     int nl_algo = 2;
     DevBuf wdev16s;
     bool s16_m16 = true;
@@ -384,6 +386,7 @@
     int nltype = 1;
     int nl_family = 0;
     bool nl_fused_pack = false;
+    int nl_merge_ks = 0;
     bool bmid = false, fuse10 = false;
     int algo = 0, conv1x1_algo = 0;
     bool sf = false;
@@ -479,6 +482,7 @@
                  : h->bf16 ? 2
                  : (!pl.strict && (h->nl_algo == 1 || (h->nl_algo == 2 && N >= 1024))) ? 1 : 3;
     pl.nl_fused_pack = (pl.nl_family == 1 || pl.nl_family == 2) && nl_f16_fits_one_launch(B, N);
+    if (pl.nl_fused_pack && h->nl_merge_fuse && H == Hfull && conv0_merges_nl_partials() && nl_f16_key_splits(B, N) > 1) pl.nl_merge_ks = nl_f16_key_splits(B, N);
 
     const size_t frame_floats = (size_t)B * T * H * W * 64;
     pl.p10_floats = pl.small_c10 ? frame_floats : 0;
@@ -552,7 +556,7 @@
     return 0;
 }
 
-int nonlocal_block(const Fwd& f, const float* in, int Hfull, int q0, int q1) {
+int nonlocal_block(const Fwd& f, const float* in, int Hfull, int q0, int q1, bool defer_merge) {
     pfnl_handle* const h = f.h;
     const TrunkPlan& pl = f.pl;
     const int B = f.B, T = f.T, W = f.W, N = (Hfull / 2) * (W / 2), C = 12 * T, CP = nl_padded_ch(C), nlt = pl.nltype;
@@ -588,7 +592,7 @@
         HIPCHK(launch_nl_attn_general(h->X.p, Kx, Nk, h->Xo.p, wd + h->off_nl_w, wd + h->off_nl_b, h->nlp.p, B, N, C, s, Qp, q0, q1, nlt == 2));
     } else if (pl.nl_family == 1 || pl.nl_family == 2) {
         HIPCHK(launch_nl_attn_f16(h->X.p, h->Xo.p, wd + h->off_nl_w, wd + h->off_nl_b, h->nlp.p, reinterpret_cast<uint16_t*>(h->nl16.p), B, N, C, s,
-                                  q0, q1, pl.nl_family == 1, pl.nl_fused_pack));
+                                  q0, q1, pl.nl_family == 1, pl.nl_fused_pack, defer_merge));
     } else {
         HIPCHK(launch_nl_attn(h->X.p, h->Xo.p, wd + h->off_nl_w, wd + h->off_nl_b, h->nlp.p, B, N, C, s, nullptr, q0, q1));
     }
@@ -843,13 +847,19 @@
     const Fwd f{h, pl, s, B, T, B * T, H, W, h->wdev.p, reinterpret_cast<const uint16_t*>(h->wdev16.p), reinterpret_cast<const uint16_t*>(h->wdev16s.p)};
     const float* const wd = h->wdev.p;
 
-    if (int e = nonlocal_block(f, in, Hfull, q0, q1)) return e;
+    const int Nq = (Hfull / 2) * (W / 2);
+    const int merge_ks = (!strip && q0 == 0 && (q1 < 0 || q1 == Nq)) ? pl.nl_merge_ks : 0;
+    if (int e = nonlocal_block(f, in, Hfull, q0, q1, merge_ks > 1)) return e;
+    h->xo_pending_ks = merge_ks;
     {
         ProfScope ps(h, s, PFNL_K_CONV0);
+        const NlPartials parts{h->nlp.p, h->nlp.p + (size_t)B * merge_ks * Nq * nl_padded_ch(12 * T), wd + h->off_nl_b, merge_ks};
+        const NlPartials* const nl = merge_ks > 1 ? &parts : nullptr;
+        const float* const xo = nl ? h->X.p : h->Xo.p;
         if (pl.bf16)
-            HIPCHK(launch_conv0_bf16(h->Xo.p, wd + h->off_conv0_w, wd + h->off_conv0_b, reinterpret_cast<uint16_t*>(h->inp0.p), B, T, Hfull, W, s, strip));
+            HIPCHK(launch_conv0_bf16(xo, wd + h->off_conv0_w, wd + h->off_conv0_b, reinterpret_cast<uint16_t*>(h->inp0.p), B, T, Hfull, W, s, strip, nl));
         else
-            HIPCHK(launch_conv0(h->Xo.p, wd + h->off_conv0_w, wd + h->off_conv0_b, h->inp0.p, B, T, Hfull, W, s, strip, pl.strict));
+            HIPCHK(launch_conv0(xo, wd + h->off_conv0_w, wd + h->off_conv0_b, h->inp0.p, B, T, Hfull, W, s, strip, pl.strict, nl));
     }
     for (int i = 0; i < c.num_block; ++i) {
         if (h->prof_mode == 2) {
@@ -922,6 +932,7 @@
      {{"auto", -1}, {"0", 0}, {"embedded_gaussian", 0}, {"1", 1}, {"gaussian", 1}, {"2", 2}, {"dot_product", 2}},
      "nl_type: auto | 0 | 1 | 2 (nltype 3, 'concat', builds no graph in the reference either: utils.py:23)"},
     {"small_c10", &pfnl_handle::small_c10, {{"on", 1}, {"off", 0}}, "small_c10 must be on or off"},
+    {"nl_merge", &pfnl_handle::nl_merge_fuse, {{"fused", 1}, {"separate", 0}}, "nl_merge must be fused or separate"},
     {"nonlocal", &pfnl_handle::nl_algo, {{"f32", 0}, {"split16", 1}, {"auto", 2}}, "nonlocal must be auto, f32 or split16"},
     {"conv1x1", &pfnl_handle::conv1x1_algo, {{"stream", 1}, {"tiled", 0}, {"split16", 2}}, "conv1x1 must be split16, stream or tiled"},
 };
@@ -1338,18 +1349,18 @@
     static const char* const nln[] = {"general_f32", "split16", "f16", "f32"};
     static const char* const a3[] = {"direct", "winograd_tile", "?", "winograd", "split16"};
     static const char* const a1[] = {"tiled", "stream", "split16"};
-    char tmp[384];
+    char tmp[448];
     if (pl.bf16)
-        std::snprintf(tmp, sizeof tmp, "%s launches_per_block=%d c1x1=%d precision=bf16 tiles=%d chains=%d whole_chains=%d split_parts=%d part_frames=%d nl=%s nl_pack_fused=%d mfma=%d merge1=%s",
+        std::snprintf(tmp, sizeof tmp, "%s launches_per_block=%d c1x1=%d precision=bf16 tiles=%d chains=%d whole_chains=%d split_parts=%d part_frames=%d nl=%s nl_pack_fused=%d nl_merge_in_conv0=%d mfma=%d merge1=%s",
                       pl.name, pl.launches_per_block, pl.c1x1_launches, pl.tiles8x32, pl.chains, pl.split_s ? pl.n_full : pl.chains, pl.split_s, pl.split_q,
-                      nln[pl.nl_family], pl.nl_fused_pack ? 1 : 0, pl.mfma, kMerge1Names[pl.merge1]);
+                      nln[pl.nl_family], pl.nl_fused_pack ? 1 : 0, pl.nl_merge_ks, pl.mfma, kMerge1Names[pl.merge1]);
     else
         std::snprintf(tmp, sizeof tmp, "%s launches_per_block=%d c1x1=%d precision=fp32 conv3x3=%s conv1x1=%s c10_fused=%d chain=%d sf0=%d strict=%d tiles=%d chains=%d "
-                      "whole_chains=%d split_parts=%d part_frames=%d nl=%s nl_pack_fused=%d mfma=%d c1_mfma=%d merge1=%s",
+                      "whole_chains=%d split_parts=%d part_frames=%d nl=%s nl_pack_fused=%d nl_merge_in_conv0=%d mfma=%d c1_mfma=%d merge1=%s",
                       pl.name, pl.launches_per_block, pl.c1x1_launches, pl.small ? "small" : a3[pl.algo < 0 || pl.algo > 4 ? 2 : pl.algo],
                       a1[pl.conv1x1_algo < 0 || pl.conv1x1_algo > 2 ? 0 : pl.conv1x1_algo], pl.c10_fused ? 1 : 0, pl.chain ? 1 : 0, pl.sf0 ? 1 : 0,
                       pl.strict ? 1 : 0, pl.tiles8x32, pl.chains, pl.split_s ? pl.n_full : pl.chains, pl.split_s, pl.split_q, nln[pl.nl_family],
-                      pl.nl_fused_pack ? 1 : 0, pl.mfma, pl.c1_mfma, kMerge1Names[pl.merge1]);
+                      pl.nl_fused_pack ? 1 : 0, pl.nl_merge_ks, pl.mfma, pl.c1_mfma, kMerge1Names[pl.merge1]);
     if (std::strlen(tmp) + 1 > buflen) return fail(PFNL_ERR_INVALID, "buffer too small");
     std::strcpy(buf, tmp);
     return 0;
@@ -1772,6 +1783,11 @@
     if (n == "nl_out") {
         need = (size_t)B * H * W * 3 * T;
         if (h->scratch.ensure(need)) return fail(PFNL_ERR_NOMEM, "scratch allocation failed");
+        if (h->xo_pending_ks > 1) {
+            const int N = (H / 2) * (W / 2), C = 12 * T, ks = h->xo_pending_ks;
+            HIPCHK(pfnl::launch_nl_merge(h->X.p, h->nlp.p, h->nlp.p + (size_t)B * ks * N * pfnl::nl_padded_ch(C), h->wdev.p + h->off_nl_b, h->Xo.p, B, N, C, ks, h->stream));
+            h->xo_pending_ks = 0;
+        }
         HIPCHK(pfnl::launch_nl_unpack(h->Xo.p, h->scratch.p, B, T, H, W, h->stream));
         HIPCHK(hipStreamSynchronize(h->stream));
         src = h->scratch.p;
diff --git a/pfnl_amd/csrc/common.h b/pfnl_amd/csrc/common.h
--- a/pfnl_amd/csrc/common.h
+++ b/pfnl_amd/csrc/common.h
@@ -120,8 +120,16 @@
 struct StripGeom {
     int yoff, Hs, core0, core1;
 };
+struct NlPartials {
+    const float* Zp;
+    const float* ML;
+    const float* bp;
+    int ks;
+};
+bool conv0_merges_nl_partials();
 hipError_t launch_conv0(const float* Xo, const float* w75x64, const float* bias, float* out, int B,
-                        int T, int H, int W, hipStream_t s, const StripGeom* strip = nullptr, bool force_f32 = false);
+                        int T, int H, int W, hipStream_t s, const StripGeom* strip = nullptr, bool force_f32 = false,
+                        const NlPartials* nl = nullptr);
 hipError_t launch_tail(const float* merge, const float* x, const float* w2, const float* b2,
                        float* out, int B, int T, int H, int W, int scale, int merge_cstride, hipStream_t s,
                        const StripGeom* strip = nullptr, unsigned* nonfinite = nullptr);
diff --git a/pfnl_amd/csrc/conv_bf16.h b/pfnl_amd/csrc/conv_bf16.h
--- a/pfnl_amd/csrc/conv_bf16.h
+++ b/pfnl_amd/csrc/conv_bf16.h
@@ -38,6 +38,6 @@
 void conv1x1_bf16_pack_weights(const float* hwio, int T, uint16_t* dst);
 struct StripGeom;
 hipError_t launch_conv0_bf16(const float* Xo, const float* w75x64, const float* bias, uint16_t* out, int B, int T, int H,
-                             int W, hipStream_t s, const StripGeom* strip = nullptr);
+                             int W, hipStream_t s, const StripGeom* strip = nullptr, const NlPartials* nl = nullptr);
 
 }
diff --git a/pfnl_amd/csrc/conv_split16.h b/pfnl_amd/csrc/conv_split16.h
--- a/pfnl_amd/csrc/conv_split16.h
+++ b/pfnl_amd/csrc/conv_split16.h
@@ -49,7 +49,9 @@
 size_t nl_f16_scratch_halfs(int B, int N);
 hipError_t launch_nl_attn_f16(const float* X, float* Xo, const float* Wp, const float* bp, float* partial, uint16_t* scratch16,
                               int B, int N, int C, hipStream_t s, int q0 = 0, int q1 = -1, bool split = true,
-                              bool prepacked = false);
+                              bool prepacked = false,
+                              bool defer_merge = false);
+int nl_f16_key_splits(int B, int N);
 bool nl_f16_fits_one_launch(int B, int N);
 hipError_t launch_nl_pack_fused(const float* x, float* X, uint16_t* scratch16, int B, int T, int H, int W, hipStream_t s);
 
diff --git a/pfnl_amd/csrc/misc_kernels.hip b/pfnl_amd/csrc/misc_kernels.hip
--- a/pfnl_amd/csrc/misc_kernels.hip
+++ b/pfnl_amd/csrc/misc_kernels.hip
@@ -94,10 +94,11 @@
 constexpr int C0M_IN_DW = C0M_IH * C0M_IW * 3 + 4;
 constexpr int C0M_W_BYTES = 5 * 2 * 2 * 1024;
 
-template <bool BF16OUT>
+template <bool BF16OUT, int KS>
 __global__ __launch_bounds__(256) void conv0_mfma_kernel(const float* __restrict__ Xo, const float* __restrict__ w,
                                                          const float* __restrict__ bias, float* __restrict__ out, int T, int H,
-                                                         int W, int CP, int yoff, int Hs) {
+                                                         int W, int CP, int yoff, int Hs, const float* __restrict__ Zp,
+                                                         const float* __restrict__ ML, const float* __restrict__ nlb) {
     typedef _Float16 h8 __attribute__((ext_vector_type(8)));
     typedef unsigned u32x4 __attribute__((ext_vector_type(4)));
     __shared__ __attribute__((aligned(16))) unsigned char sw[C0M_W_BYTES];
@@ -115,8 +116,9 @@
         hb = __builtin_bit_cast(unsigned short, hi);
         lb = __builtin_bit_cast(unsigned short, lo);
     };
-    constexpr int C0M_WIT = (5 * 2 * 64 + 255) / 256, C0M_XIT = (C0M_IN_DW + 255) / 256;
-    float wreg[C0M_WIT][8], xreg[C0M_XIT];
+    constexpr int C0M_WIT = (5 * 2 * 64 + 255) / 256, C0M_XIT = (C0M_IN_DW + 255) / 256, C0M_PIT = (C0M_IH * C0M_IW + 255) / 256;
+    float wreg[C0M_WIT][8];
+    [[maybe_unused]] float xreg[C0M_XIT], preg[C0M_PIT][3];
 #pragma unroll
     for (int k = 0; k < C0M_WIT; ++k) {
         const int ent = min(tid + k * 256, 5 * 2 * 64 - 1);
@@ -128,16 +130,60 @@
             wreg[k][e] = kp < 15 ? wv : 0.f;
         }
     }
-#pragma unroll
-    for (int k = 0; k < C0M_XIT; ++k) {
-        const int i = min(tid + k * 256, C0M_IN_DW - 1);
-        const int c = i % 3, pix = i / 3;
-        const int py = pix / C0M_IW, px = pix - py * C0M_IW;
-        const int gy = yoff + y0 + py - 2, gx = x0 + px - 2;
-        const bool in = py < C0M_IH && gy >= 0 && gy < H && gx >= 0 && gx < W;
-        const int cy = in ? gy : 0, cx = in ? gx : 0;
-        const float v = Xb[((size_t)(cy >> 1) * W2 + (cx >> 1)) * CP + ((cy & 1) * 2 + (cx & 1)) * C3 + 3 * t + c];
-        xreg[k] = in ? v : 0.f;
+    if constexpr (KS == 0) {
+#pragma unroll
+        for (int k = 0; k < C0M_XIT; ++k) {
+            const int i = min(tid + k * 256, C0M_IN_DW - 1);
+            const int c = i % 3, pix = i / 3;
+            const int py = pix / C0M_IW, px = pix - py * C0M_IW;
+            const int gy = yoff + y0 + py - 2, gx = x0 + px - 2;
+            const bool in = py < C0M_IH && gy >= 0 && gy < H && gx >= 0 && gx < W;
+            const int cy = in ? gy : 0, cx = in ? gx : 0;
+            const float v = Xb[((size_t)(cy >> 1) * W2 + (cx >> 1)) * CP + ((cy & 1) * 2 + (cx & 1)) * C3 + 3 * t + c];
+            xreg[k] = in ? v : 0.f;
+        }
+    } else {
+        const size_t N = (size_t)(H / 2) * W2;
+#pragma unroll
+        for (int k = 0; k < C0M_PIT; ++k) {
+            const int pix = min(tid + k * 256, C0M_IH * C0M_IW - 1);
+            const int py = pix / C0M_IW, px = pix - py * C0M_IW;
+            const int gy = yoff + y0 + py - 2, gx = x0 + px - 2;
+            const bool in = gy >= 0 && gy < H && gx >= 0 && gx < W;
+            const int cy = in ? gy : 0, cx = in ? gx : 0;
+            const size_t qn = (size_t)(cy >> 1) * W2 + (cx >> 1);
+            const int co = ((cy & 1) * 2 + (cx & 1)) * C3 + 3 * t;
+            float ml0[KS], ml1[KS], z[KS][3], xv[3], bv[3];
+#pragma unroll
+            for (int p = 0; p < KS; ++p) {
+                const size_t row = ((size_t)b * KS + p) * N + qn;
+                ml0[p] = ML[row * 2];
+                ml1[p] = ML[row * 2 + 1];
+#pragma unroll
+                for (int c = 0; c < 3; ++c) z[p][c] = Zp[row * CP + co + c];
+            }
+#pragma unroll
+            for (int c = 0; c < 3; ++c) {
+                xv[c] = Xb[qn * CP + co + c];
+                bv[c] = nlb[co + c];
+            }
+            float m = -INFINITY;
+#pragma unroll
+            for (int p = 0; p < KS; ++p) m = fmaxf(m, ml0[p]);
+            float num[3] = {0.f, 0.f, 0.f}, den = 0.f;
+#pragma unroll
+            for (int p = 0; p < KS; ++p) {
+                const float wgt = exp2f(ml0[p] - m);
+#pragma unroll
+                for (int c = 0; c < 3; ++c) num[c] = fmaf(wgt, z[p][c], num[c]);
+                den = fmaf(wgt, ml1[p], den);
+            }
+#pragma unroll
+            for (int c = 0; c < 3; ++c) {
+                const float v = xv[c] + num[c] / den + bv[c];
+                preg[k][c] = in ? v : 0.f;
+            }
+        }
     }
 #pragma unroll
     for (int k = 0; k < C0M_WIT; ++k) {
@@ -156,13 +202,28 @@
         *reinterpret_cast<u32x4*>(sw + ((ky * 2 + 0) * 2 + g) * 1024 + l * 16) = hq;
         *reinterpret_cast<u32x4*>(sw + ((ky * 2 + 1) * 2 + g) * 1024 + l * 16) = lq;
     }
-#pragma unroll
-    for (int k = 0; k < C0M_XIT; ++k) {
-        const int i = tid + k * 256;
-        if (i >= C0M_IN_DW) break;
-        unsigned short hb, lb;
-        split1(xreg[k], hb, lb);
-        s_in[i] = hb | ((unsigned)lb << 16);
+    if constexpr (KS == 0) {
+#pragma unroll
+        for (int k = 0; k < C0M_XIT; ++k) {
+            const int i = tid + k * 256;
+            if (i >= C0M_IN_DW) break;
+            unsigned short hb, lb;
+            split1(xreg[k], hb, lb);
+            s_in[i] = hb | ((unsigned)lb << 16);
+        }
+    } else {
+#pragma unroll
+        for (int k = 0; k < C0M_PIT; ++k) {
+            const int pix = tid + k * 256;
+            if (pix >= C0M_IH * C0M_IW) break;
+#pragma unroll
+            for (int c = 0; c < 3; ++c) {
+                unsigned short hb, lb;
+                split1(preg[k][c], hb, lb);
+                s_in[pix * 3 + c] = hb | ((unsigned)lb << 16);
+            }
+        }
+        if (tid < C0M_IN_DW - C0M_IH * C0M_IW * 3) s_in[C0M_IH * C0M_IW * 3 + tid] = 0u;
     }
     __syncthreads();
 
@@ -233,14 +294,36 @@
     return v != 0;
 }
 
+bool conv0_merges_nl_partials() { return !conv0_use_valu(); }
+
+template <bool BF16OUT>
+static hipError_t conv0_mfma_launch(const float* Xo, const float* w75x64, const float* bias, float* out, int B, int T, int H, int W, hipStream_t s,
+                                    int yoff, int Hs, const NlPartials* nl) {
+    const dim3 grid((W + C0M_TW - 1) / C0M_TW, (Hs + C0M_TH - 1) / C0M_TH, B * T);
+    const int CP = nl_padded_ch(12 * T);
+    const int ks = nl ? nl->ks : 0;
+#define C0M_LAUNCH(KS_) hipLaunchKernelGGL((conv0_mfma_kernel<BF16OUT, KS_>), grid, dim3(256), 0, s, Xo, w75x64, bias, out, T, H, W, CP, yoff, Hs, \
+                                           nl ? nl->Zp : nullptr, nl ? nl->ML : nullptr, nl ? nl->bp : nullptr)
+    switch (ks) {
+        case 0: C0M_LAUNCH(0); break;
+        case 2: C0M_LAUNCH(2); break;
+        case 3: C0M_LAUNCH(3); break;
+        case 4: C0M_LAUNCH(4); break;
+        case 5: C0M_LAUNCH(5); break;
+        case 6: C0M_LAUNCH(6); break;
+        case 7: C0M_LAUNCH(7); break;
+        case 8: C0M_LAUNCH(8); break;
+        default: return hipErrorInvalidValue;
+    }
+#undef C0M_LAUNCH
+    return hipGetLastError();
+}
+
 hipError_t launch_conv0(const float* Xo, const float* w75x64, const float* bias, float* out, int B,
-                        int T, int H, int W, hipStream_t s, const StripGeom* strip, bool force_f32) {
+                        int T, int H, int W, hipStream_t s, const StripGeom* strip, bool force_f32, const NlPartials* nl) {
     const int yoff = strip ? strip->yoff : 0, Hs = strip ? strip->Hs : H;
-    if (!conv0_use_valu() && !force_f32) {
-        dim3 grid((W + C0M_TW - 1) / C0M_TW, (Hs + C0M_TH - 1) / C0M_TH, B * T);
-        hipLaunchKernelGGL(conv0_mfma_kernel<false>, grid, dim3(256), 0, s, Xo, w75x64, bias, out, T, H, W, nl_padded_ch(12 * T), yoff, Hs);
-        return hipGetLastError();
-    }
+    if (!conv0_use_valu() && !force_f32) return conv0_mfma_launch<false>(Xo, w75x64, bias, out, B, T, H, W, s, yoff, Hs, nl);
+    if (nl) return hipErrorInvalidValue;
     dim3 grid((W + C0_T - 1) / C0_T, (Hs + C0_T - 1) / C0_T, B * T);
     hipLaunchKernelGGL(conv0_kernel<false>, grid, dim3(256), 0, s, Xo, w75x64, bias, out, T, H, W,
                        nl_padded_ch(12 * T), yoff, Hs);
@@ -248,14 +331,10 @@
 }
 
 hipError_t launch_conv0_bf16(const float* Xo, const float* w75x64, const float* bias, uint16_t* out, int B, int T, int H,
-                             int W, hipStream_t s, const StripGeom* strip) {
+                             int W, hipStream_t s, const StripGeom* strip, const NlPartials* nl) {
     const int yoff = strip ? strip->yoff : 0, Hs = strip ? strip->Hs : H;
-    if (!conv0_use_valu()) {
-        dim3 grid((W + C0M_TW - 1) / C0M_TW, (Hs + C0M_TH - 1) / C0M_TH, B * T);
-        hipLaunchKernelGGL(conv0_mfma_kernel<true>, grid, dim3(256), 0, s, Xo, w75x64, bias, reinterpret_cast<float*>(out), T, H, W,
-                           nl_padded_ch(12 * T), yoff, Hs);
-        return hipGetLastError();
-    }
+    if (!conv0_use_valu()) return conv0_mfma_launch<true>(Xo, w75x64, bias, reinterpret_cast<float*>(out), B, T, H, W, s, yoff, Hs, nl);
+    if (nl) return hipErrorInvalidValue;
     dim3 grid((W + C0_T - 1) / C0_T, (Hs + C0_T - 1) / C0_T, B * T);
     hipLaunchKernelGGL(conv0_kernel<true>, grid, dim3(256), 0, s, Xo, w75x64, bias, reinterpret_cast<float*>(out), T, H, W,
                        nl_padded_ch(12 * T), yoff, Hs);
diff --git a/pfnl_amd/csrc/nonlocal_f16.hip b/pfnl_amd/csrc/nonlocal_f16.hip
--- a/pfnl_amd/csrc/nonlocal_f16.hip
+++ b/pfnl_amd/csrc/nonlocal_f16.hip
@@ -183,13 +183,19 @@
     const int ksp = gridDim.z, sp = blockIdx.z;
     const int kt0 = (int)((long long)ntiles * sp / ksp), kt1 = (int)((long long)ntiles * (sp + 1) / ksp);
 #pragma unroll
-    for (int j = 0; j < G::NSLOT - 1; ++j)
+    for (int k = 0; k < G::PW; ++k) tile_piece(k, kt0, 0, kt0 < kt1);
+#pragma unroll
+    for (int k = 0; k < G::PW; ++k) tile_piece(k, 0, G::NSLOT - 1, false);
+#pragma unroll
+    for (int j = 1; j < G::NSLOT - 1; ++j)
 #pragma unroll
         for (int k = 0; k < G::PW; ++k) tile_piece(k, kt0 + j, j, kt0 + j < kt1);
-#pragma unroll
-    for (int k = 0; k < G::PW; ++k) tile_piece(k, 0, G::NSLOT - 1, false);
-    asm volatile("s_waitcnt vmcnt(0)" ::: "memory");
-    __syncthreads();
+    if (G::PIECES % 8 == 0 || wave + 8 * (G::PW - 1) < G::PIECES) {
+        asm volatile("s_waitcnt vmcnt(%0)" ::"n"((G::NSLOT - 2) * G::PW) : "memory");
+    } else {
+        asm volatile("s_waitcnt vmcnt(%0)" ::"n"((G::NSLOT - 2) * (G::PW - 1)) : "memory");
+    }
+    NF_BARRIER();
 
     bf16x8 pt[2][2];
     [[maybe_unused]] bf16x8 pl[2][2];
@@ -529,7 +535,8 @@
 }
 
 static hipError_t nl_attn_f16_run(const float* X, float* Xo, const float* Wp, const float* bp, float* partial, uint16_t* scratch16,
-                                  int B, int N, int C, hipStream_t s, int q0, int q1, bool split, int ks_cap, bool prepacked = false);
+                                  int B, int N, int C, hipStream_t s, int q0, int q1, bool split, int ks_cap, bool prepacked = false,
+                                  bool defer_merge = false);
 
 bool nl_f16_fits_one_launch(int B, int N) { return 2 * nl_f16_scratch_halfs(1, N) * (size_t)B <= nl_f16_chunk_limit(); }
 
@@ -546,12 +553,29 @@
     return hipGetLastError();
 }
 
+static int nl_f16_splits_of(int B, int nq, int ks_max) {
+    const long long qb = (long long)((nq + NF_QB - 1) / NF_QB) * B;
+    int ks = 1;
+    double best = 1e30;
+    for (int k = 1; k <= ks_max; ++k) {
+        const double t = (double)((qb * k + 255) / 256) / k;
+        if (t < best - 1e-9) {
+            best = t;
+            ks = k;
+        }
+    }
+    return ks;
+}
+
+int nl_f16_key_splits(int B, int N) { return nl_f16_splits_of(B, N, nl_key_splits(B, N)); }
+
 hipError_t launch_nl_attn_f16(const float* X, float* Xo, const float* Wp, const float* bp, float* partial, uint16_t* scratch16,
-                               int B, int N, int C, hipStream_t s, int q0, int q1, bool split, bool prepacked) {
+                               int B, int N, int C, hipStream_t s, int q0, int q1, bool split, bool prepacked, bool defer_merge) {
     if (B < 1 || N < 1) return hipErrorInvalidValue;
+    if (defer_merge && !(prepacked && q0 == 0 && (q1 < 0 || q1 == N) && nl_f16_key_splits(B, N) > 1)) return hipErrorInvalidValue;
     if (prepacked) {
         if (!nl_f16_fits_one_launch(B, N)) return hipErrorInvalidValue;
-        return nl_attn_f16_run(X, Xo, Wp, bp, partial, scratch16, B, N, C, s, q0, q1, split, nl_key_splits(B, N), true);
+        return nl_attn_f16_run(X, Xo, Wp, bp, partial, scratch16, B, N, C, s, q0, q1, split, nl_key_splits(B, N), true, defer_merge);
     }
     const size_t per_clip = 2 * nl_f16_scratch_halfs(1, N);
     const int ks_cap = nl_key_splits(B, N);
@@ -566,7 +590,7 @@
 }
 
 static hipError_t nl_attn_f16_run(const float* X, float* Xo, const float* Wp, const float* bp, float* partial, uint16_t* scratch16,
-                                  int B, int N, int C, hipStream_t s, int q0, int q1, bool split, int ks_cap, bool prepacked) {
+                                  int B, int N, int C, hipStream_t s, int q0, int q1, bool split, int ks_cap, bool prepacked, bool defer_merge) {
     if (C != 84 && C != 60 && C != 36) return hipErrorInvalidValue;
     if (q1 < 0) q1 = N;
     if (q0 < 0 || q0 >= q1 || q1 > N) return hipErrorInvalidValue;
@@ -581,19 +605,7 @@
         hipError_t e = hipGetLastError();
         if (e != hipSuccess) return e;
     }
-    const int ks_max = std::min(nl_key_splits(B, N), ks_cap);
-    int ks = 1;
-    {
-        const long long qb = (long long)((q1 - q0 + NF_QB - 1) / NF_QB) * B;
-        double best = 1e30;
-        for (int k = 1; k <= ks_max; ++k) {
-            const double t = (double)((qb * k + 255) / 256) / k;
-            if (t < best - 1e-9) {
-                best = t;
-                ks = k;
-            }
-        }
-    }
+    const int ks = nl_f16_splits_of(B, q1 - q0, std::min(nl_key_splits(B, N), ks_cap));
     if (ks > 1 && !partial) return hipErrorInvalidValue;
     float* Zp = partial;
     float* ML = partial ? partial + (size_t)B * ks * N * CP : nullptr;
@@ -626,7 +638,7 @@
     }
 #undef NP_LAUNCH
     hipError_t e = hipGetLastError();
-    if (e != hipSuccess || ks == 1) return e;
+    if (e != hipSuccess || ks == 1 || defer_merge) return e;
     return launch_nl_merge(X, Zp, ML, bp, Xo, B, N, C, ks, s, q0, q1);
 }
 
diff --git a/pfnl_amd/engine.py b/pfnl_amd/engine.py
--- a/pfnl_amd/engine.py
+++ b/pfnl_amd/engine.py
@@ -103,7 +103,7 @@
         _capi.check(self._lib.pfnl_copy_weights(self._h, other._h))
         self._ready = True
 
-    OPTION_KEYS = ("precision", "strict_fp32", "conv3x3", "conv1x1", "conv2", "merge1", "nonlocal", "nl_type", "nl_sub_sample", "small", "small_c10",
+    OPTION_KEYS = ("precision", "strict_fp32", "conv3x3", "conv1x1", "conv2", "merge1", "nonlocal", "nl_merge", "nl_type", "nl_sub_sample", "small", "small_c10",
                    "split16_sf", "split16_chain", "split16_c10", "split16_mid", "split16_sf0", "split16_splitchains", "bf16_conv10", "bf16_mfma", "split16_mfma", "graph")
 
     def clone(self) -> "PFNLEngine":
```

Measured after the change: 957.0. Within noise of the previous version (-0.1%).
